# liuQuan98/EYOC

Measured on AMD Instinct MI355X. Metric: registered pairs/sec (30k-voxel KITTI pairs), higher is better.
Workload: dtype f32 (split16 products: fp32 storage/accumulation, 3 fp16 MFMAs on hi/lo-split operands per product); 1 GPU; 64 synthetic 30 cm KITTI-shaped pairs per step per GPU (mean 29894 voxels/cloud, ResUNetBN2C random-init, 5000-point NN, RANSAC 4000000 hypotheses/pair, planted inlier ratio 0.3, spconv math split16); parallelism=pairs sharded over 1 GPU(s), steps_in_flight=2

## Files before the change

### eyoc_amd/_lib.py

```python
from __future__ import annotations

import ctypes as C
import os
import threading

_HERE = os.path.dirname(os.path.abspath(__file__))
LIB_PATH = os.environ.get("EYOC_HIP_LIB") or os.path.join(_HERE, "lib", "libeyoc_hip.so")

MAX_LEVELS = 4
MAP_S1, MAP_DOWN, MAP_UP = 0, 1, 2


class MapsInfo(C.Structure):
    _fields_ = [("n_levels", C.c_int32), ("rows", C.c_int32 * MAX_LEVELS),
                ("pairs_s1", C.c_int64 * MAX_LEVELS), ("pairs_down", C.c_int64 * MAX_LEVELS),
                ("pairs_up", C.c_int64 * MAX_LEVELS), ("pairs_conv1", C.c_int64)]


class ModelDesc(C.Structure):
    _fields_ = [("in_channels", C.c_int32), ("out_channels", C.c_int32), ("conv1_kernel_size", C.c_int32),
                ("normalize_feature", C.c_int32), ("channels", C.c_int32 * 5), ("tr_channels", C.c_int32 * 5),
                ("bn_eps", C.c_float), ("expanded", C.c_int32)]


class LayerParams(C.Structure):
    _fields_ = [("name", C.c_char_p), ("kernel", C.POINTER(C.c_float)), ("K", C.c_int32), ("cin", C.c_int32),
                ("cout", C.c_int32), ("bias", C.POINTER(C.c_float)), ("bn_weight", C.POINTER(C.c_float)),
                ("bn_bias", C.POINTER(C.c_float)), ("bn_mean", C.POINTER(C.c_float)),
                ("bn_var", C.POINTER(C.c_float))]


class RansacParams(C.Structure):
    _fields_ = [("max_distance", C.c_float), ("edge_similarity", C.c_float), ("max_iteration", C.c_int32),
                ("seed", C.c_uint32)]


class RansacResult(C.Structure):
    _fields_ = [("T", C.c_float * 16), ("inliers", C.c_int32), ("best_hypothesis", C.c_int32),
                ("survivors", C.c_int32), ("inlier_rmse", C.c_float)]


class Sc2pcrParams(C.Structure):
    _fields_ = [("inlier_threshold", C.c_float), ("d_thre", C.c_float), ("ratio", C.c_float),
                ("nms_radius", C.c_float), ("num_iterations", C.c_int32), ("max_points", C.c_int32),
                ("k1", C.c_int32), ("k2", C.c_int32)]


class Sc2pcrLayout(C.Structure):
    _fields_ = ([(k, C.c_int32) for k in ("n", "words", "n_seed", "k1", "k2", "n_part", "col_chunk", "reserved")] +
                [("csr_cap", C.c_int64), ("total", C.c_uint64)] +
                [("off_" + k, C.c_uint64) for k in ("ctl", "v", "y", "score", "seeds", "hard", "tight", "knn", "Ts", "dom", "rank",
                                                    "ptr_h", "col_h", "val_h", "cnt", "blk_dense", "seed_h")])


class IcpParams(C.Structure):
    _fields_ = [("max_distance", C.c_double), ("relative_fitness", C.c_double), ("relative_rmse", C.c_double),
                ("max_iteration", C.c_int32), ("flags", C.c_int32)]


class IcpResult(C.Structure):
    _fields_ = [("T", C.c_double * 16), ("fitness", C.c_double), ("inlier_rmse", C.c_double), ("correspondences", C.c_int32),
                ("iterations", C.c_int32), ("status", C.c_int32), ("reserved", C.c_int32)]


_vp, _i, _sz = C.c_void_p, C.c_int, C.c_size_t
PROTOTYPES = {
    "eyoc_version": (_i, []),
    "eyoc_last_error": (C.c_char_p, []),
    "eyoc_create": (_i, [_i, C.POINTER(_vp)]),
    "eyoc_destroy": (_i, [_vp]),
    "eyoc_maps_workspace_bytes": (_sz, [_i]),
    "eyoc_maps_build": (_i, [_vp, _vp, _i, _vp, _sz, _vp, C.POINTER(_vp)]),
    "eyoc_maps_build_ordered": (_i, [_vp, _vp, _i, _vp, _sz, _vp, _i, C.POINTER(_vp)]),
    "eyoc_maps_free": (_i, [_vp]),
    "eyoc_maps_last_fault_batches": (_i, [_vp, _vp, _vp]),
    "eyoc_maps_internal_order": (_i, [_vp, _i]),
    "eyoc_maps_lazy_tables": (_i, [_vp, _i]),
    "eyoc_maps_fused_levels": (_i, [_vp, _i]),
    "eyoc_spconv_select_down_kernel": (_i, [_vp, _i]),
    "eyoc_maps_order_window_shift": (_i, [_vp, _i]),
    "eyoc_maps_row_order": (_vp, [_vp]),
    "eyoc_maps_copy_row_order": (_i, [_vp, _vp, _vp]),
    "eyoc_maps_rows": (_i, [_vp, _i]),
    "eyoc_maps_coords": (_vp, [_vp, _i]),
    "eyoc_maps_table": (_vp, [_vp, _i, _i]),
    "eyoc_maps_copy_coords": (_i, [_vp, _i, _vp, _vp]),
    "eyoc_maps_copy_table": (_i, [_vp, _i, _i, _vp, _vp]),
    "eyoc_maps_copy_up_order": (_i, [_vp, _i, _vp, _vp]),
    "eyoc_maps_order_min_rows": (_i, [_vp, _i]),
    "eyoc_maps_info": (_i, [_vp, _vp, _i, _vp, C.POINTER(MapsInfo)]),
    "eyoc_voxelize_workspace_bytes": (_sz, [_i]),
    "eyoc_voxelize": (_i, [_vp, _vp, _i, _i, C.c_float, _i, _vp, _vp, C.POINTER(C.c_int), _vp, _sz, _vp]),
    "eyoc_voxelize_batched_workspace_bytes": (_sz, [_i, _i]),
    "eyoc_voxelize_batched": (_i, [_vp, _vp, _i, C.POINTER(C.c_int64), _i, _i, C.c_float, _i, _vp, _vp, _vp,
                                   C.POINTER(C.c_int64), _vp, _sz, _vp]),
    "eyoc_voxelize_batched_isolating_workspace_bytes": (_sz, [_i, _i]),
    "eyoc_voxelize_batched_isolating": (_i, [_vp, _vp, _i, C.POINTER(C.c_int64), _i, _i, C.c_float, _i, _vp, _vp, _vp,
                                             C.POINTER(C.c_int64), _vp, _sz, _vp, _vp]),
    "eyoc_batch_drop_workspace_bytes": (_sz, [_i]),
    "eyoc_batch_drop": (_i, [_vp, _vp, _vp, _i, _i, _vp, _vp, _vp, _vp, C.POINTER(C.c_int), _vp, _vp, _sz, _vp]),
    "eyoc_remap_rows": (_i, [_vp, _vp, _i, _vp, _i, _vp, _vp]),
    "eyoc_gather_rows": (_i, [_vp, _vp, _i, _i, _vp, _i, _vp, C.c_float, _vp, _vp]),
    "eyoc_dotmax": (_i, [_vp, _vp, _vp, _i, C.POINTER(C.c_int32), C.POINTER(C.c_int32), _i, _vp, _vp, _vp]),
    "eyoc_knn2": (_i, [_vp, _vp, _vp, _i, C.POINTER(C.c_int32), C.POINTER(C.c_int32), _i, _vp, _vp, _vp, _vp]),
    "eyoc_lowe_topk": (_i, [_vp, _vp, _vp, _i, _i, _vp, _vp, _vp]),
    "eyoc_pair_filter": (_i, [_vp, _i, _vp, _vp, _vp, _vp, _i, _vp, C.c_float, _vp, _vp, _vp]),
    "eyoc_pair_filter_similarity": (_i, [_vp, _vp, _vp, _vp, _vp, _i, _vp, _i, _i, C.c_float, C.c_float, C.c_double, _vp, _vp,
                                         _vp]),
    "eyoc_spconv_packed_floats": (_sz, [_i, _i, _i]),
    "eyoc_spconv_pack_weights": (_i, [_vp, _vp, _i, _i, _i, _vp]),
    "eyoc_spconv_select_kernel": (_i, [_vp, _i]),
    "eyoc_spconv_pack_weights_transposed": (_i, [_vp, _i, _i, _i, _i, _vp]),
    "eyoc_spconv_grad_weight_workspace_bytes": (_sz, [_i, _i, _i, _i]),
    "eyoc_spconv_grad_weight": (_i, [_vp, _vp, _i, _i, _vp, _i, _i, _vp, _i, _i, _vp, _vp, _sz, _vp]),
    "eyoc_spconv_pack_weights_split16": (_i, [_vp, _vp, _i, _i, _i, _vp, _vp]),
    "eyoc_spconv_ex": (_i, [_vp, _vp, _i, _i, _i, _vp, _i, _i, _vp, _i, _vp, _vp, _i, _i, _vp, _i, _i, _i, _vp, _vp]),
    "eyoc_spconv_select_split16_kernel": (_i, [_vp, _i]),
    "eyoc_spconv_select_st_kernel": (_i, [_vp, _i]),
    "eyoc_spconv_st_split_below": (_i, [_vp, _i]),
    "eyoc_spconv_st_group_rows": (_i, [_vp, _i]),
    "eyoc_spconv_st_ksplit": (_i, [_vp, _i]),
    "eyoc_spconv_local_rulebook_bytes": (_sz, [_i]),
    "eyoc_spconv_build_local_rulebook": (_i, [_vp, _vp, _i, _i, _vp, _vp, _vp]),
    "eyoc_spconv_staged": (_i, [_vp, _vp, _vp, _i, _i, _vp, _i, _i, _vp, _i, _vp, _vp, _i, _i, _vp, _i, _i, _vp, _vp]),
    "eyoc_split16_encode": (_i, [_vp, _vp, _i, _i, _i, _vp, _i, _vp]),
    "eyoc_split16_decode": (_i, [_vp, _vp, _i, _i, _i, _vp, _i, _vp]),
    "eyoc_model_set_math": (_i, [_vp, _i]),
    "eyoc_model_last_math": (_i, [_vp]),
    "eyoc_model_range_check": (_i, [_vp, _vp, C.POINTER(C.c_float)]),
    "eyoc_model_range_snapshot": (_i, [_vp, _vp, _vp]),
    "eyoc_model_set_progress_event": (_i, [_vp, _i, _vp]),
    "eyoc_model_set_probe": (_i, [_vp, _i]),
    "eyoc_spconv": (_i, [_vp, _vp, _i, _i, _vp, _i, _i, _vp, _i, _vp, _vp, _i, _i, _vp, _i, _vp]),
    "eyoc_spconv_sum": (_i, [_vp, _vp, _i, _i, _vp, _i, _i, _vp, _i, _vp, _i, _vp]),
    "eyoc_model_blob_floats": (_sz, [C.POINTER(ModelDesc)]),
    "eyoc_model_pack_host": (_i, [C.POINTER(ModelDesc), C.POINTER(LayerParams), _i, _vp, _sz]),
    "eyoc_model_create": (_i, [_vp, C.POINTER(ModelDesc), C.POINTER(LayerParams), _i, _vp, _sz, C.POINTER(_vp)]),
    "eyoc_model_destroy": (_i, [_vp]),
    "eyoc_model_fuse_tail": (_i, [_vp, _i]),
    "eyoc_model_workspace_bytes": (_sz, [_vp, _vp]),
    "eyoc_model_forward": (_i, [_vp, _vp, _vp, _vp, _vp, _vp, _sz, _vp]),
    "eyoc_model_num_layers": (_i, [_vp]),
    "eyoc_model_layer_work": (_i, [_vp, _vp, _vp, _vp, C.POINTER(C.c_char_p), C.POINTER(C.c_int64),
                                   C.POINTER(C.c_double), C.POINTER(C.c_double), C.POINTER(C.c_double)]),
    "eyoc_model_set_timing": (_i, [_vp, _i]),
    "eyoc_model_layer_ms": (_i, [_vp, C.POINTER(C.c_float)]),
    "eyoc_model_timing_slot": (_i, [_vp, _i]),
    "eyoc_bn_workspace_bytes": (_sz, [_i, _i]),
    "eyoc_bn_train_forward": (_i, [_vp, _vp, _i, _i, _i, _vp, _vp, C.c_float, _i, _vp, _i, _vp, _vp, _sz, _vp]),
    "eyoc_bn_train_forward_running": (_i, [_vp, _vp, _i, _i, _i, _vp, _vp, C.c_float, _i, _vp, _i, _vp, _vp, _vp, C.c_float, _vp, _sz, _vp]),
    "eyoc_bn_train_backward": (_i, [_vp, _vp, _i, _vp, _i, _vp, _i, _i, _i, _vp, _vp, C.c_float, _vp, _i, _vp, _vp, _vp, _sz, _vp]),
    "eyoc_maps_gather_window": (_i, [_vp, _vp, _i, _vp, _i, _vp, _vp]),
    "eyoc_maps_gather_window_internal": (_i, [_vp, _vp, _i, _vp, _i, _vp, _vp]),
    "eyoc_knn_prefilter": (_i, [_vp, _i]),
    "eyoc_spconv_select_up_kernel": (_i, [_vp, _i]),
    "eyoc_spconv_upc_min_rows": (_i, [_vp, _i]),
    "eyoc_spconv_upc_tile_rows": (_i, [_i, _i]),
    "eyoc_spconv_upc_bytes": (_sz, [_i]),
    "eyoc_spconv_upc_build": (_i, [_vp, _vp, _i, _vp, _vp, _vp]),
    "eyoc_spconv_upc": (_i, [_vp, _vp, _vp, _i, _i, _vp, _i, _i, _vp, _i, _vp, _i, _vp, _i, _i, _vp, _vp]),
    "eyoc_spconv_select_conv1_kernel": (_i, [_vp, _i]),
    "eyoc_knn1": (_i, [_vp, _vp, _vp, _i, C.POINTER(C.c_int32), C.POINTER(C.c_int32), _i, _i, _vp, _vp, _vp]),
    "eyoc_pdist": (_i, [_vp, _vp, _i, _vp, _i, _i, _i, _vp, _vp]),
    "eyoc_kabsch_batched": (_i, [_vp, _vp, _vp, _vp, _i, _i, _vp, _vp]),
    "eyoc_irls_quad": (_i, [_vp, _vp, _vp, _vp, _i, _i, _vp, _vp]),
    "eyoc_ransac": (_i, [_vp, _vp, _vp, _vp, _i, C.POINTER(RansacParams), _vp, _vp]),
    "eyoc_maps_select_orders": (_i, [_vp, _i, _i]),
    "eyoc_ransac_select_pruning": (_i, [_vp, _i]),
    "eyoc_registration_accept_degenerate": (_i, [_vp, _i]),
    "eyoc_ransac_transform_store": (_i, [_vp, _i]),
    "eyoc_ransac_workspace_bytes": (_sz, [_vp, _i, _i, _i, _sz]),
    "eyoc_ransac_batched_ws": (_i, [_vp, _vp, _vp, _vp, C.POINTER(C.c_int32), C.POINTER(C.c_int32), _i,
                                    C.POINTER(RansacParams), _vp, _vp, _sz, _vp]),
    "eyoc_ransac_batched": (_i, [_vp, _vp, _vp, _vp, C.POINTER(C.c_int32), C.POINTER(C.c_int32), _i,
                                 C.POINTER(RansacParams), _vp, _vp]),
    "eyoc_sc2pcr_workspace_bytes": (_sz, [_i, C.POINTER(Sc2pcrParams)]),
    "eyoc_sc2pcr": (_i, [_vp, _vp, _vp, _i, C.POINTER(Sc2pcrParams), _vp, _vp, _vp, _sz, _vp]),
    "eyoc_sc2pcr_batched_workspace_bytes": (_sz, [_i, C.POINTER(Sc2pcrParams)]),
    "eyoc_sc2pcr_batched_workspace_bytes_n": (_sz, [_i, _i, C.POINTER(Sc2pcrParams)]),
    "eyoc_sc2pcr_set_shortlist_cap": (_i, [_vp, _i]),
    "eyoc_sc2pcr_set_dense_threshold": (_i, [_vp, _i]),
    "eyoc_sc2pcr_select_kernels": (_i, [_vp, _i]),
    "eyoc_sc2pcr_workspace_layout": (_i, [_i, C.POINTER(Sc2pcrParams), C.POINTER(Sc2pcrLayout)]),
    "eyoc_sc2pcr_batched": (_i, [_vp, _vp, _vp, C.POINTER(C.c_int32), _i, C.POINTER(Sc2pcrParams), _vp, _vp, _i, _vp, _sz,
                                 _vp]),
    "eyoc_icp_workspace_bytes": (_sz, [_i, _i, _i]),
    "eyoc_icp_batched": (_i, [_vp, _vp, _vp, C.POINTER(C.c_int32), C.POINTER(C.c_int32), _i, _vp, C.POINTER(IcpParams), _vp, _vp,
                              _vp, _sz, _vp]),
    "eyoc_icp_correspondences": (_i, [_vp, _vp, _vp, C.POINTER(C.c_int32), C.POINTER(C.c_int32), _i, _vp, C.c_double, _vp, _vp,
                                      _vp, _vp, _sz, _vp]),
}


ERR_INVALID, ERR_HIP, ERR_WORKSPACE, ERR_DUPLICATE, ERR_RANGE = -1, -2, -3, -4, -5
# ... 136 lines not shown
```

### eyoc_amd/csrc/common.h

```cpp
#pragma once
#include <hip/hip_runtime.h>

#include <cstdarg>
#include <cstdint>
#include <cstdio>
#include <cstring>
#include <string>
#include <vector>

#include "../../include/eyoc_hip.h"

namespace eyoc {

void set_error(const char* fmt, ...);

#define EYOC_CHECK_HIP(expr)                                                               \
  do {                                                                                     \
    hipError_t _e = (expr);                                                                \
    if (_e != hipSuccess) {                                                                \
      eyoc::set_error("%s failed: %s (%s:%d)", #expr, hipGetErrorString(_e), __FILE__,    \
                      __LINE__);                                                           \
      return EYOC_ERR_HIP;                                                                 \
    }                                                                                      \
  } while (0)
// ... 87 lines not shown
  unsigned long long* keys;
  int* vals;
  unsigned int mask;
};

__host__ __device__ inline unsigned long long pack_key(int b, int x, int y, int z) {
  return ((unsigned long long)(unsigned)b << 54) |
         ((unsigned long long)((unsigned)(x + COORD_BIAS) & 0x3FFFFu) << 36) |
         ((unsigned long long)((unsigned)(y + COORD_BIAS) & 0x3FFFFu) << 18) |
         ((unsigned long long)((unsigned)(z + COORD_BIAS) & 0x3FFFFu));
}

__host__ __device__ inline unsigned int hash_key(unsigned long long k) {
  k ^= k >> 33;
  k *= 0xff51afd7ed558ccdull;
  k ^= k >> 33;
  k *= 0xc4ceb9fe1a85ec53ull;
  k ^= k >> 33;
  return (unsigned int)k;
}

__device__ inline int hash_lookup(const HashTable& t, unsigned long long key) {
  unsigned int s = hash_key(key) & t.mask;
  for (unsigned int probes = 0; probes <= t.mask; ++probes) {
    unsigned long long k = t.keys[s];
    if (k == key) return t.vals[s];
    if (k == KEY_EMPTY) return -1;
    s = (s + 1) & t.mask;
  }
  return -1;
}

}

struct eyoc_maps {
  int n_levels = 0;
  int rows[EYOC_MAX_LEVELS] = {0, 0, 0, 0};
  int32_t* coords[EYOC_MAX_LEVELS] = {nullptr, nullptr, nullptr, nullptr};
  eyoc::HashTable table[EYOC_MAX_LEVELS];
  int32_t* nbr_s1[EYOC_MAX_LEVELS] = {nullptr, nullptr, nullptr, nullptr};
  int32_t* nbr_down[EYOC_MAX_LEVELS] = {nullptr, nullptr, nullptr, nullptr};
  int32_t* nbr_up[EYOC_MAX_LEVELS] = {nullptr, nullptr, nullptr, nullptr};
  int32_t* parent[EYOC_MAX_LEVELS] = {nullptr, nullptr, nullptr, nullptr};
  int32_t* children[EYOC_MAX_LEVELS] = {nullptr, nullptr, nullptr, nullptr};
  int32_t* perm_up[EYOC_MAX_LEVELS] = {nullptr, nullptr, nullptr, nullptr};
  int32_t* perm_s1[EYOC_MAX_LEVELS] = {nullptr, nullptr, nullptr, nullptr};
  int32_t* perm_down[EYOC_MAX_LEVELS] = {nullptr, nullptr, nullptr, nullptr};
  int32_t* row_perm = nullptr;
  unsigned char* local_s1[EYOC_MAX_LEVELS] = {nullptr, nullptr, nullptr, nullptr};
  unsigned char* local_up[EYOC_MAX_LEVELS] = {nullptr, nullptr, nullptr, nullptr};
  unsigned char* local_s1w[EYOC_MAX_LEVELS] = {nullptr, nullptr, nullptr, nullptr};
  unsigned char* local_down[EYOC_MAX_LEVELS] = {nullptr, nullptr, nullptr, nullptr};
  unsigned char* local_upc[EYOC_MAX_LEVELS] = {nullptr, nullptr, nullptr, nullptr};
  bool table0_built = false;
  bool s1_ready[EYOC_MAX_LEVELS] = {true, true, true, true};
  bool up_ready[EYOC_MAX_LEVELS] = {true, true, true, true};
  int32_t* up8[EYOC_MAX_LEVELS] = {nullptr, nullptr, nullptr, nullptr};
  hipEvent_t s1_ev[EYOC_MAX_LEVELS] = {nullptr, nullptr, nullptr, nullptr};
  hipEvent_t up_ev[EYOC_MAX_LEVELS] = {nullptr, nullptr, nullptr, nullptr};
  hipEvent_t table0_ev = nullptr;
  eyoc_maps() = default;
  eyoc_maps(const eyoc_maps&) = delete;
  eyoc_maps& operator=(const eyoc_maps&) = delete;
  ~eyoc_maps();
};

namespace eyoc {
int maps_build_table0(eyoc_maps* maps, hipStream_t st);
int maps_ensure_table(eyoc_maps* maps, int kind, int level, hipStream_t st);
size_t sort_rows64_tmp_bytes(int n);
int sort_rows_by_key64(void* tmp, size_t tmp_bytes, const unsigned long long* keys_in, unsigned long long* keys_out, const int* vals_in,
                       int* vals_out, int n, int bits, hipStream_t st);
size_t sort_rows_tmp_bytes(int n, int bits);
int sort_rows_by_key(void* tmp, size_t tmp_bytes, const unsigned int* keys_in, unsigned int* keys_out, const int* vals_in,
                     int* vals_out, int n, int bits, hipStream_t st);
}
```

### eyoc_amd/csrc/coordmap.hip

```cpp
#include <cstdlib>

#include "spconv.h"
#include "derive.h"
#include "scan.h"

using namespace eyoc;

namespace {

__device__ inline void coarse_coord(const int32_t* c, int ts2, int& b, int& x, int& y, int& z) {
  const int m = ~(ts2 - 1);
  b = c[0]; x = c[1] & m; y = c[2] & m; z = c[3] & m;
}

__global__ void k_insert(const int32_t* __restrict__ coords, int n, int ts2, HashTable t, int* __restrict__ slot_out,
                         int* __restrict__ err, unsigned int* __restrict__ range_mask = nullptr) {
  int i = blockIdx.x * blockDim.x + threadIdx.x;
  if (i >= n) return;
  int b, x, y, z;
  coarse_coord(coords + 4 * (size_t)i, ts2, b, x, y, z);
  constexpr int LIM = COORD_BIAS - 16;
  if (b < 0 || b >= 1024 || x < -LIM || x >= LIM || y < -LIM || y >= LIM || z < -LIM || z >= LIM) {
    if (err) atomicAdd(&err[0], 1);
    if (range_mask && b >= 0 && b < 1024) atomicOr(&range_mask[b >> 5], 1u << (b & 31));
// ... 556 lines not shown
  for (; i < n; i += stride) c += t[i] >= 0;
#pragma unroll
  for (int d = 32; d >= 1; d >>= 1) c += __shfl_down(c, d, 64);
  if ((threadIdx.x & 63) == 0 && c) atomicAdd(out, (unsigned long long)c);
}

__global__ void k_count_region(const int32_t* __restrict__ coords, int n, HashTable t, int ks,
                               unsigned long long* __restrict__ out) {
  int o = blockIdx.x * blockDim.x + threadIdx.x;
  unsigned int c = 0;
  if (o < n) {
    const int4 p = reinterpret_cast<const int4*>(coords)[o];
    const int r = ks / 2;
    for (int dz = -r; dz <= r; ++dz)
      for (int dy = -r; dy <= r; ++dy)
        for (int dx = -r; dx <= r; ++dx) c += hash_lookup(t, pack_key(p.x, p.y + dx, p.z + dy, p.w + dz)) >= 0;
  }
#pragma unroll
  for (int d = 32; d >= 1; d >>= 1) c += __shfl_down(c, d, 64);
  if ((threadIdx.x & 63) == 0 && c) atomicAdd(out, (unsigned long long)c);
}

constexpr int UP_KEY_BITS = KEY_PATTERN_BITS + KEY_WINDOW_BITS;
constexpr int ZORDER_MIN_ROWS = 8192;

unsigned int table_capacity(int n) {
  unsigned int cap = 1024;
  while (cap < 2u * (unsigned)n) cap <<= 1;
  return cap;
}

const int32_t* table_ptr(const eyoc_maps* maps, int kind, int level) {
  if (!maps || level < 0 || level >= maps->n_levels) return nullptr;
  switch (kind) {
    case EYOC_MAP_S1: return maps->nbr_s1[level];
    case EYOC_MAP_DOWN: return level + 1 < maps->n_levels ? maps->nbr_down[level] : nullptr;
    case EYOC_MAP_UP: return level + 1 < maps->n_levels ? maps->nbr_up[level] : nullptr;
    default: return nullptr;
  }
}

hipEvent_t* fill_event(eyoc_maps* m, int kind, int level) {
  if (!m || level < 0 || level + 1 >= m->n_levels) return nullptr;
  if (kind == EYOC_MAP_S1) return &m->s1_ev[level];
  if (kind == EYOC_MAP_UP) return &m->up_ev[level];
  return nullptr;
}

void keep_fault_masks(eyoc_ctx* ctx, const int* h, int code) {
  if (code == EYOC_ERR_DUPLICATE) memcpy(ctx->fault_dup, h, 32 * sizeof(uint32_t));
  if (code == EYOC_ERR_RANGE) memcpy(ctx->fault_range, h + 32, 32 * sizeof(uint32_t));
}

}

extern "C" {

size_t eyoc_maps_workspace_bytes(int n_rows) {
  if (n_rows < 0) return 0;
  const size_t n = (size_t)n_rows;
  const size_t cap = table_capacity(n_rows);
  size_t b = 0;
  b += EYOC_MAX_LEVELS * (align_up(cap * 8) + align_up(cap * 4));
  b += EYOC_MAX_LEVELS * align_up(n * 16);
  b += 10 * align_up(n * 27 * 4);
  b += 3 * align_up(n * 8 * 4);
  b += 3 * align_up(n * 4) + align_up((n / SCAN_TILE + 2) * 4);
  b += 3 * (align_up(n * 4) + align_up(n * 32));
  b += 4 * align_up(4 * n * 4) + align_up(sort_rows_tmp_bytes(4 * n_rows, UP_KEY_BITS + 4));
  b += align_up(n * 8) * 2 + align_up(n * 4) * 2 + align_up(sort_rows64_tmp_bytes(n_rows));
  b += 2 * align_up(local_rulebook_bytes(n_rows)) + EYOC_MAX_LEVELS * (align_up(local_rulebook_bytes(1)) + 256);
  b += 2 * align_up(local_rulebook_up_bytes(n_rows)) + EYOC_MAX_LEVELS * (align_up(local_rulebook_up_bytes(1)) + 256);
  b += 2 * (align_up(upc_kept_bytes(n_rows)) + align_up(upc_scratch_bytes(n_rows))) + EYOC_MAX_LEVELS * (align_up(upc_kept_bytes(1)) + align_up(upc_scratch_bytes(1)) + 512);
  b += 4 * (align_up(local_rulebook128_bytes(n_rows)) + 256);
  b += 4096;
  return b + 96 * 256;
}

int eyoc_maps_build(eyoc_ctx* ctx, const int32_t* coords_dev, int n, void* ws, size_t ws_bytes, void* stream,
                    eyoc_maps** out) {
  return eyoc_maps_build_ordered(ctx, coords_dev, n, ws, ws_bytes, stream, 0, out);
}

int eyoc_maps_build_ordered(eyoc_ctx* ctx, const int32_t* coords_dev, int n, void* ws, size_t ws_bytes, void* stream,
                            int order, eyoc_maps** out) {
  if (ctx) {
    memset(ctx->fault_dup, 0, sizeof(ctx->fault_dup));
    memset(ctx->fault_range, 0, sizeof(ctx->fault_range));
  }
  EYOC_REQUIRE(ctx && out && ws, EYOC_ERR_INVALID, "eyoc_maps_build: NULL argument");
  EYOC_REQUIRE(order >= -1 && order <= 1, EYOC_ERR_INVALID, "eyoc_maps_build_ordered: order %d", order);
  EYOC_REQUIRE(n > 0 && coords_dev, EYOC_ERR_INVALID, "eyoc_maps_build: empty coordinate set (n=%d)", n);
  EYOC_REQUIRE(((uintptr_t)ws & 255) == 0, EYOC_ERR_INVALID, "eyoc_maps_build: workspace must be 256-byte aligned");
  EYOC_REQUIRE(ws_bytes >= eyoc_maps_workspace_bytes(n), EYOC_ERR_WORKSPACE,
               "eyoc_maps_build: workspace %zu < required %zu bytes", ws_bytes, eyoc_maps_workspace_bytes(n));
  hipStream_t st = (hipStream_t)stream;
  Carver cv(ws, ws_bytes);
  eyoc_maps* m = new eyoc_maps();
  m->n_levels = EYOC_MAX_LEVELS;
  int* counters = cv.take<int>(128);
  unsigned int* fault_masks = (unsigned int*)(counters + 64);
  int* slot = cv.take<int>(n);
  int* flag = cv.take<int>(n);
  int* partial = cv.take<int>(n / SCAN_TILE + 2);
  int* host = (int*)ctx->pinned;
#define FAIL_HIP(expr)                                                                       \
  do {                                                                                       \
    hipError_t _e = (expr);                                                                  \
    if (_e != hipSuccess) {                                                                  \
      set_error("%s failed: %s (%s:%d)", #expr, hipGetErrorString(_e), __FILE__, __LINE__);  \
      delete m;                                                                              \
      return EYOC_ERR_HIP;                                                                   \
    }                                                                                        \
  } while (0)

  FAIL_HIP(hipMemsetAsync(counters, 0, 128 * sizeof(int), st));
  m->rows[0] = n;
  m->coords[0] = cv.take<int32_t>((size_t)n * 4);
  const eyoc_ctx::Knobs& kn = ctx->knobs;
  const int order_mode = kn.maps_internal_order >= 0 ? kn.maps_internal_order : order;
  const bool zorder = order_mode > 0 || (order_mode < 0 && n >= ZORDER_MIN_ROWS);
  int pre_rows[EYOC_MAX_LEVELS] = {n, 0, 0, 0};
  if (zorder) {
    unsigned long long* zk_in = cv.take<unsigned long long>(n);
    unsigned long long* zk_out = cv.take<unsigned long long>(n);
    int* zr_in = cv.take<int>(n);
    m->row_perm = cv.take<int32_t>(n);
    const size_t zb = sort_rows64_tmp_bytes(n);
    void* ztmp = cv.take<char>(zb);
    int kbits = ctx->zorder_kbits, bbits = ctx->zorder_bbits;
    for (int attempt = 0; attempt < 2; ++attempt) {
      if (attempt) FAIL_HIP(hipMemsetAsync(counters + 16, 0, (EYOC_MAX_LEVELS + 4) * sizeof(int), st));
      hipLaunchKernelGGL(k_morton_key, dim3(cdiv(n, 256)), dim3(256), 0, st, coords_dev, n, kbits, zk_in, zr_in);
      if (int rc = sort_rows_by_key64(ztmp, zb, zk_in, zk_out, zr_in, m->row_perm, n, 3 * (kbits + 1) + bbits, st)) { delete m; return rc; }
      hipLaunchKernelGGL(k_gather_coords, dim3(cdiv(n, 256)), dim3(256), 0, st, coords_dev, m->row_perm, n, m->coords[0]);
      hipLaunchKernelGGL(k_count_levels, dim3(cdiv(n, 256) < 1024 ? cdiv(n, 256) : 1024), dim3(256), 0, st, m->coords[0], n, kbits, bbits,
                         counters + 16, fault_masks);
      FAIL_HIP(hipMemcpyAsync(host + 16, counters + 16, (128 - 16) * sizeof(int), hipMemcpyDeviceToHost, st));
      FAIL_HIP(hipStreamSynchronize(st));
      if (host[16] == 0) break;
      kbits = 17; bbits = 10;
    }
    {
      int kb = 1, bb = 1;
      while (kb < 17 && (1 << kb) <= host[16 + EYOC_MAX_LEVELS + 2]) ++kb;
      while (bb < 10 && (1 << bb) <= host[16 + EYOC_MAX_LEVELS + 3]) ++bb;
      ctx->zorder_kbits = kb + 1 < 17 ? kb + 1 : 17;
      ctx->zorder_bbits = bb + 1 < 10 ? bb + 1 : 10;
    }
    if (host[16 + EYOC_MAX_LEVELS] != 0) {
      set_error("eyoc_maps_build: %d coordinate rows outside the supported key range (|c| < 2^17 - 16, 0 <= batch < 1024)",
                host[16 + EYOC_MAX_LEVELS]);
      keep_fault_masks(ctx, host + 64, EYOC_ERR_RANGE);
      delete m;
      return EYOC_ERR_RANGE;
    }
    if (host[16 + EYOC_MAX_LEVELS + 1] != 0) {
      set_error("eyoc_maps_build: %d duplicate coordinate rows (a sparse tensor needs unique coordinates)", host[16 + EYOC_MAX_LEVELS + 1]);
      keep_fault_masks(ctx, host + 64, EYOC_ERR_DUPLICATE);
      delete m;
      return EYOC_ERR_DUPLICATE;
    }
    for (int l = 1; l < EYOC_MAX_LEVELS; ++l) pre_rows[l] = host[16 + l];
  } else {
    FAIL_HIP(hipMemcpyAsync(m->coords[0], coords_dev, (size_t)n * 16, hipMemcpyDeviceToDevice, st));
  }
  {
    const unsigned int cap = table_capacity(n);
    m->table[0].keys = cv.take<unsigned long long>(cap);
    m->table[0].vals = cv.take<int>(cap);
    m->table[0].mask = cap - 1;
    m->table0_built = false;
  }
  unsigned int top_cap = 0;
// ... 7 lines not shown
    FAIL_HIP(hipMemsetAsync(m->children[0], 0xFF, (size_t)((char*)(tt.keys + top_cap) - (char*)m->children[0]), st));
    FAIL_HIP(hipMemsetAsync(tt.vals, 0x7F, (size_t)top_cap * 4, st));
  }
  const bool fused_levels = zorder && kn.maps_fused_levels;
  if (fused_levels) {
    LevelOut lo;
    for (int l = 1; l < EYOC_MAX_LEVELS; ++l) {
      m->rows[l] = pre_rows[l];
      m->coords[l] = cv.take<int32_t>((size_t)m->rows[l] * 4);
      m->parent[l - 1] = cv.take<int32_t>((size_t)m->rows[l - 1]);
      lo.coords[l - 1] = m->coords[l]; lo.parent[l - 1] = m->parent[l - 1]; lo.children[l - 1] = m->children[l - 1];
    }
    const int tiles = cdiv(n, LV_TILE);
    int* part = flag;
    hipLaunchKernelGGL(k_levels_count, dim3(tiles), dim3(LV_BLOCK), 0, st, m->coords[0], n, part, counters);
    hipLaunchKernelGGL(k_levels_fill, dim3(tiles), dim3(LV_BLOCK), 0, st, m->coords[0], n, part, lo, counters + 3);
    const int lt = EYOC_MAX_LEVELS - 1;
    hipLaunchKernelGGL(k_insert, dim3(cdiv(m->rows[lt], 256)), dim3(256), 0, st, m->coords[lt], m->rows[lt], 1 << lt, m->table[lt], (int*)nullptr, counters);
  }
  for (int l = 1; l < EYOC_MAX_LEVELS && !fused_levels; ++l) {
    const int n_src = m->rows[l - 1];
    const int32_t* src = m->coords[l - 1];
    const int ts2 = 1 << l;
    const int nb = cdiv(n_src, SCAN_TILE);
    const bool sorted_level = zorder;
    HashTable& t = m->table[l];
    if (sorted_level) {
      hipLaunchKernelGGL(k_flag_sorted, dim3(cdiv(n_src, 256)), dim3(256), 0, st, src, n_src, ts2, flag,
                         l == 1 ? counters : (int*)nullptr, l == 1 ? counters + 1 : (int*)nullptr);
    } else {
      const unsigned int cap = table_capacity(n_src);
      t.keys = cv.take<unsigned long long>(cap);
      t.vals = cv.take<int>(cap);
      t.mask = cap - 1;
      FAIL_HIP(hipMemsetAsync(t.keys, 0xFF, (size_t)cap * 8, st));
      FAIL_HIP(hipMemsetAsync(t.vals, 0x7F, (size_t)cap * 4, st));
      hipLaunchKernelGGL(k_insert, dim3(cdiv(n_src, 256)), dim3(256), 0, st, src, n_src, ts2, t, slot, counters,
                         l == 1 ? fault_masks + 32 : (unsigned int*)nullptr);
      hipLaunchKernelGGL(k_flag, dim3(cdiv(n_src, 256)), dim3(256), 0, st, slot, t.vals, n_src, flag, (int*)nullptr);
    }
    hipLaunchKernelGGL(k_scan_partials, dim3(nb), dim3(SCAN_BLOCK), 0, st, flag, n_src, partial);
    hipLaunchKernelGGL(k_scan_top, dim3(1), dim3(SCAN_BLOCK), 0, st, partial, nb, counters + 2 + l);
    if (zorder) {
      m->rows[l] = pre_rows[l];
    } else {
    if (l == 1) {
      FAIL_HIP(hipMemcpyAsync(host + 128, counters, 128 * sizeof(int), hipMemcpyDeviceToHost, st));
      FAIL_HIP(hipStreamSynchronize(st));
      host[0] = host[128 + 2 + l]; host[1] = host[128]; host[2] = host[128 + 1];
    } else {
      FAIL_HIP(hipMemcpyAsync(host, counters + 2 + l, sizeof(int), hipMemcpyDeviceToHost, st));
      FAIL_HIP(hipStreamSynchronize(st));
    }
    if (l == 1 && host[1] != 0) {
      set_error("eyoc_maps_build: %d coordinate rows outside the supported key range (|c| < 2^17 - 16, 0 <= batch < 1024)", host[1]);
      keep_fault_masks(ctx, host + 128 + 64, EYOC_ERR_RANGE);
      delete m;
      return EYOC_ERR_RANGE;
    }
    if (l == 1 && sorted_level && host[2] != 0) {
      set_error("eyoc_maps_build: %d duplicate coordinate rows (a sparse tensor needs unique coordinates)", host[2]);
      keep_fault_masks(ctx, host + 128 + 64, EYOC_ERR_DUPLICATE);
      delete m;
      return EYOC_ERR_DUPLICATE;
    }
    m->rows[l] = host[0];
    }
    m->coords[l] = cv.take<int32_t>((size_t)m->rows[l] * 4);
    m->parent[l - 1] = cv.take<int32_t>((size_t)n_src);
    if (!zorder) {
      m->children[l - 1] = cv.take<int32_t>((size_t)m->rows[l] * 8);
      FAIL_HIP(hipMemsetAsync(m->children[l - 1], 0xFF, (size_t)m->rows[l] * 32, st));
    }
    if (sorted_level) {
      hipLaunchKernelGGL(k_compact_sorted, dim3(nb), dim3(SCAN_BLOCK), 0, st, flag, partial, src, n_src, ts2, l - 1,
                         m->coords[l], m->parent[l - 1], m->children[l - 1]);
      if (l + 1 == EYOC_MAX_LEVELS) {
        hipLaunchKernelGGL(k_insert, dim3(cdiv(m->rows[l], 256)), dim3(256), 0, st, m->coords[l], m->rows[l], ts2, t, (int*)nullptr, counters);
      }
      continue;
    }
    hipLaunchKernelGGL(k_compact<false>, dim3(nb), dim3(SCAN_BLOCK), 0, st, flag, partial, slot, src, n_src, ts2,
                       m->coords[l], t.vals, (int32_t*)nullptr);
    hipLaunchKernelGGL(k_children, dim3(cdiv(n_src, 256)), dim3(256), 0, st, slot, t.vals, src, n_src, l - 1,
                       m->parent[l - 1], m->children[l - 1], l == 1 ? counters + 1 : (int*)nullptr,
                       l == 1 ? fault_masks : (unsigned int*)nullptr);
    if (l == 1) {
      FAIL_HIP(hipMemcpyAsync(host + 128, counters, 128 * sizeof(int), hipMemcpyDeviceToHost, st));
      FAIL_HIP(hipStreamSynchronize(st));
      host[0] = host[128 + 1];
      if (host[0] != 0) {
        set_error("eyoc_maps_build: %d duplicate coordinate rows (a sparse tensor needs unique coordinates)", host[0]);
        keep_fault_masks(ctx, host + 128 + 64, EYOC_ERR_DUPLICATE);
        delete m;
        return EYOC_ERR_DUPLICATE;
      }
    }
  }
  const bool use_upc = kn.up_kernel == 2 && n >= kn.upc_min_rows;
  const bool use_up = kn.up_kernel == 1 || (kn.up_kernel == 2 && !use_upc);
  const bool lazy = zorder && use_upc && kn.maps_lazy_tables != 0;
  for (int l = 0; l < EYOC_MAX_LEVELS; ++l) {
    m->nbr_s1[l] = cv.take<int32_t>((size_t)27 * m->rows[l]);
    if (l + 1 < EYOC_MAX_LEVELS) {
      m->nbr_down[l] = cv.take<int32_t>((size_t)27 * m->rows[l + 1]);
      m->nbr_up[l] = cv.take<int32_t>((size_t)27 * m->rows[l]);
// ... 27 lines not shown
  unsigned int* key_in = cv.take<unsigned int>(total);
  unsigned int* key_out = cv.take<unsigned int>(total);
  int* row_in = cv.take<int>(total);
  int32_t* perm_all = cv.take<int32_t>(total);
  const size_t sort_bytes = sort_rows_tmp_bytes((int)total, TAG_SHIFT + TAG_BITS);
  void* sort_tmp = cv.take<char>(sort_bytes);
  for (int l = EYOC_MAX_LEVELS - 2; l >= 0; --l) {
    const int nl = m->rows[l], nc = m->rows[l + 1];
    const int su = seg_up[l];
    if (lazy) {
      if (l > 0)
        hipLaunchKernelGGL((k_derive_fine<true, 2>), dim3(cdiv(nl, 256)), dim3(256), 0, st, m->coords[l], nl, l, m->parent[l], m->children[l],
                           m->nbr_s1[l + 1], nc, m->nbr_s1[l], m->up8[l], (unsigned int*)nullptr, (int*)nullptr, 0u, wshift);
    } else {
      hipLaunchKernelGGL((k_derive_fine<true, 1>), dim3(cdiv(nl, 256)), dim3(256), 0, st, m->coords[l], nl, l, m->parent[l],
                         m->children[l], m->nbr_s1[l + 1], nc, m->nbr_s1[l], m->nbr_up[l],
                         su >= 0 ? key_in + seg_base[su] : (unsigned int*)nullptr, su >= 0 ? row_in + seg_base[su] : (int*)nullptr,
                         (unsigned int)(su >= 0 ? su : 0) << TAG_SHIFT, wshift);
    }
    hipLaunchKernelGGL(k_derive_down, dim3(cdiv(nc, 256)), dim3(256), 0, st, nc, m->children[l], m->nbr_s1[l + 1],
                       m->nbr_down[l]);
  }
  for (int l = 0; l + 1 < EYOC_MAX_LEVELS; ++l) {
    const int sd = seg_dn[l];
    if (sd < 0) continue;
    hipLaunchKernelGGL(k_children_key, dim3(cdiv(m->rows[l + 1], 256)), dim3(256), 0, st, m->children[l], m->rows[l + 1],
                       key_in + seg_base[sd], row_in + seg_base[sd], (unsigned int)sd << TAG_SHIFT, wshift);
  }
  for (int l = 0; l < EYOC_MAX_LEVELS; ++l) {
    const int ss = seg_s1[l];
    if (ss < 0) continue;
    const int bits = l == 0 ? 2 : 4;
    hipLaunchKernelGGL(k_pattern_key, dim3(cdiv(m->rows[l], 256)), dim3(256), 0, st, m->nbr_s1[l], m->rows[l], bits,
                       key_in + seg_base[ss], row_in + seg_base[ss], (unsigned int)ss << TAG_SHIFT, wshift);
  }
  if (total > 0) {
    if (int rc = sort_rows_by_key(sort_tmp, sort_bytes, key_in, key_out, row_in, perm_all, (int)total, TAG_SHIFT + TAG_BITS, st)) {
      delete m;
      return rc;
    }
    for (int l = 0; l < EYOC_MAX_LEVELS; ++l) {
      if (seg_up[l] >= 0) m->perm_up[l] = perm_all + seg_base[seg_up[l]];
      if (seg_s1[l] >= 0) m->perm_s1[l] = perm_all + seg_base[seg_s1[l]];
      if (seg_dn[l] >= 0) m->perm_down[l] = perm_all + seg_base[seg_dn[l]];
    }
  }
  if (zorder) {
    for (int l = 0; l < EYOC_MAX_LEVELS; ++l) {
      m->local_s1[l] = cv.take<unsigned char>(local_rulebook_bytes(m->rows[l]));
      if (lazy && l == 0) {
        DeriveSrc src;
        src.coords = m->coords[0]; src.parent = m->parent[0]; src.children = m->children[0]; src.s1c = m->nbr_s1[1];
        src.nc = m->rows[1]; src.sh = 0; src.up8 = m->up8[0];
        if (int rc = build_local_rulebook_derived(src, m->rows[0], m->local_s1[0], counters + 8, st, kn.st_group)) { delete m; return rc; }
      } else if (int rc = build_local_rulebook(m->nbr_s1[l], 27, m->rows[l], m->local_s1[l], counters + 8, st, kn.st_group)) { delete m; return rc; }
      if (l + 1 < EYOC_MAX_LEVELS && use_up) {
        m->local_up[l] = cv.take<unsigned char>(local_rulebook_up_bytes(m->rows[l]));
        if (int rc = build_local_rulebook_up(m->nbr_up[l], 27, m->rows[l], m->local_up[l], counters + 9, st)) { delete m; return rc; }
      }
      if (l + 1 < EYOC_MAX_LEVELS && use_upc) {
        m->local_upc[l] = cv.take<unsigned char>(upc_kept_bytes(m->rows[l]));
        unsigned char* scratch = cv.take<unsigned char>(upc_scratch_bytes(m->rows[l]));
        if (m->local_upc[l]) {
          if (int rc = build_upc(lazy ? m->up8[l] : m->nbr_up[l], m->coords[l], 1 << l, m->rows[l], m->local_upc[l], scratch, st, lazy)) { delete m; return rc; }
        } else if (int rc = maps_ensure_table(m, EYOC_MAP_UP, l, st)) { delete m; return rc; }
      }
    }
    const bool use_down = kn.down_kernel == 1 && n >= kn.upc_min_rows;
    for (int l = EYOC_MAX_LEVELS - 1; l < EYOC_MAX_LEVELS && use_down && kn.s1_wide; ++l) {
      m->local_s1w[l] = cv.take<unsigned char>(local_rulebook128_bytes(m->rows[l]));
      if (m->local_s1w[l])
        if (int rc = build_local_rulebook128(m->nbr_s1[l], 27, m->rows[l], m->local_s1w[l], counters + 13, st, kn.st_group)) { delete m; return rc; }
    }
    for (int l = 0; l + 1 < EYOC_MAX_LEVELS && use_down; ++l) {
      m->local_down[l] = cv.take<unsigned char>(local_rulebook128_bytes(m->rows[l + 1]));
      if (m->local_down[l])
        if (int rc = build_local_rulebook128(m->nbr_down[l], 27, m->rows[l + 1], m->local_down[l], counters + 10 + l, st, kn.st_group)) { delete m; return rc; }
    }
    for (int l = 0; l < EYOC_MAX_LEVELS; ++l) {
      host[16 + l] = 0;
      if (m->local_upc[l]) FAIL_HIP(hipMemcpyAsync(host + 16 + l, upc_overflow_ptr(m->local_upc[l]), sizeof(int), hipMemcpyDeviceToHost, st));
    }
    FAIL_HIP(hipMemcpyAsync(host, counters + 8, 8 * sizeof(int), hipMemcpyDeviceToHost, st));
    FAIL_HIP(hipMemcpyAsync(host + 32, counters, 8 * sizeof(int), hipMemcpyDeviceToHost, st));
    FAIL_HIP(hipStreamSynchronize(st));
    if (host[32] != 0) {
      set_error("eyoc_maps_build: %d coordinate rows outside the supported key range (|c| < 2^17 - 16, 0 <= batch < 1024)", host[32]);
      keep_fault_masks(ctx, host + 64, EYOC_ERR_RANGE);
      delete m;
      return EYOC_ERR_RANGE;
    }
    if (host[33] != 0) {
      set_error("eyoc_maps_build: %d duplicate coordinate rows (a sparse tensor needs unique coordinates)", host[33]);
      keep_fault_masks(ctx, host + 64, EYOC_ERR_DUPLICATE);
      delete m;
      return EYOC_ERR_DUPLICATE;
    }
    for (int l = 1; l < EYOC_MAX_LEVELS; ++l)
      if (host[32 + 2 + l] != m->rows[l]) {
        set_error("eyoc_maps_build: internal error - level %d has %d rows by its scan, %d by the up-front count", l, host[32 + 2 + l], m->rows[l]);
        delete m;
        return EYOC_ERR_INVALID;
      }
    if (host[0] != 0) {
      for (int l = 0; l < EYOC_MAX_LEVELS; ++l) m->local_s1[l] = nullptr;
      if (int rc = maps_ensure_table(m, EYOC_MAP_S1, 0, st)) { delete m; return rc; }
    }
    if (host[1] != 0)
      for (int l = 0; l < EYOC_MAX_LEVELS; ++l) m->local_up[l] = nullptr;
    for (int l = 0; l + 1 < EYOC_MAX_LEVELS; ++l)
      if (host[2 + l] != 0) m->local_down[l] = nullptr;
    if (host[5] != 0)
      for (int l = 0; l < EYOC_MAX_LEVELS; ++l) m->local_s1w[l] = nullptr;
    for (int l = 0; l < EYOC_MAX_LEVELS; ++l)
      if (host[16 + l] != 0) {
        m->local_upc[l] = nullptr;
        if (int rc = maps_ensure_table(m, EYOC_MAP_UP, l, st)) { delete m; return rc; }
      }
  }
  FAIL_HIP(hipGetLastError());
#undef FAIL_HIP
  if (!cv.ok()) {
    set_error("eyoc_maps_build: internal workspace accounting error (%zu > %zu)", cv.off, cv.cap);
    delete m;
    return EYOC_ERR_WORKSPACE;
  }
  *out = m;
  return EYOC_OK;
}

size_t eyoc_voxelize_workspace_bytes(int n_points) {
  if (n_points < 0) return 0;
  const size_t n = (size_t)n_points, cap = table_capacity(n_points);
  return align_up(cap * 8) + align_up(cap * 4) + align_up(n * 16) + 3 * align_up(n * 4) +
         align_up((n / SCAN_TILE + 2) * 4) + 4096 + 16 * 256;
}

size_t eyoc_voxelize_batched_workspace_bytes(int n_points_total, int n_clouds) {
  if (n_points_total < 0 || n_clouds < 1) return 0;
  return eyoc_voxelize_workspace_bytes(n_points_total) + align_up((size_t)(n_clouds + 1) * 8) + align_up((size_t)(n_clouds + 1) * 4);
}

size_t eyoc_voxelize_batched_isolating_workspace_bytes(int n_points_total, int n_clouds) {
  if (n_points_total < 0 || n_clouds < 1) return 0;
  return eyoc_voxelize_batched_workspace_bytes(n_points_total, n_clouds) + align_up((size_t)n_clouds * 8 + 8);
}

}

namespace {

int voxelize_run(eyoc_ctx* ctx, const char* who, const float* xyz_dev, int n, int stride, const int64_t* pt_off_host,
                 int n_clouds, float voxel_size, int batch_base, int32_t* sel_dev, int32_t* coords_dev, float* xyz_out_dev,
                 int64_t* vox_off_host, void* ws, size_t ws_bytes, hipStream_t st, int32_t* faults_host = nullptr) {
  Carver cv(ws, ws_bytes);
  const bool iso = faults_host != nullptr;
  const int fo = 64 + ((n_clouds + 2) & ~1);
  int* counters = cv.take<int>(iso ? fo + 2 * n_clouds : 64 + n_clouds + 1);
  int* faults = counters + fo;
  int64_t* pt_off = cv.take<int64_t>(n_clouds + 1);
  int32_t* raw = cv.take<int32_t>((size_t)n * 4);
  int* slot = cv.take<int>(n);
  int* flag = cv.take<int>(n);
  int* partial = cv.take<int>(n / SCAN_TILE + 2);
  HashTable t;
  const unsigned int cap = table_capacity(n);
  t.keys = cv.take<unsigned long long>(cap);
  t.vals = cv.take<int>(cap);
  t.mask = cap - 1;
  EYOC_REQUIRE(cv.ok(), EYOC_ERR_WORKSPACE, "%s: internal workspace accounting error (%zu > %zu)", who, cv.off, cv.cap);
  const size_t up_bytes = n_clouds > 1 ? align_up((size_t)(n_clouds + 1) * 8) : 0;
  const int back = iso ? fo + 2 * n_clouds : n_clouds > 1 ? 64 + n_clouds + 1 : 4;
  EYOC_REQUIRE(up_bytes + (size_t)back * 4 <= ctx->pinned_bytes, EYOC_ERR_INVALID, "%s: %d clouds exceed the pinned staging", who,
               n_clouds);
  int64_t* up = (int64_t*)ctx->pinned;
  int* host = (int*)((char*)ctx->pinned + up_bytes);
  if (n_clouds > 1) {
    memcpy(up, pt_off_host, (size_t)(n_clouds + 1) * 8);
    EYOC_CHECK_HIP(hipMemcpyAsync(pt_off, up, (size_t)(n_clouds + 1) * 8, hipMemcpyHostToDevice, st));
  }
  EYOC_CHECK_HIP(hipMemsetAsync(counters, 0, 64 * sizeof(int), st));
  if (iso) EYOC_CHECK_HIP(hipMemsetAsync(faults, 0, (size_t)n_clouds * 2 * sizeof(int), st));
// ... 346 lines not shown
```

### eyoc_amd/csrc/model.hip

```cpp
#include <algorithm>
#include <cmath>
#include <cstdlib>

#include "spconv.h"

using namespace eyoc;

namespace {

enum MapSel { M_CONV1, M_S1, M_DOWN, M_UP, M_IDENT, M_AFFINE };

struct LayerPlan {
  std::string name;
  std::string norm;
  int K, cin, cout;
  MapSel map;
  int level;
  int out_level;
  int in_buf, in_col, out_buf, out_col, res_buf;
  int relu, l2norm, has_bias;
  size_t w_off = 0, b_off = 0;
  size_t w16_off = 0, s_off = 0;
};

// ... 333 lines not shown
  if (m->math == 0) return 0;
  for (const LayerPlan& p : m->layers)
    if (p.map == M_S1 && p.cin >= 128 && p.cout >= 64 && p.cout <= 256 &&
        (long long)cdiv(maps->rows[p.level], ST_TILE) * (p.cout / 32) <= KS_MAX_SLOTS)
      return KS_PART_BYTES;
  return 0;
}

size_t eyoc_model_workspace_bytes(const eyoc_model* m, const eyoc_maps* maps) {
  if (!m || !maps) return 0;
  size_t b = 0;
  for (int i = B_X1; i < B_OUT; ++i) b += align_up((size_t)maps->rows[m->bufs[i].level] * m->bufs[i].width * sizeof(float));
  b += align_up(ks_part_bytes(m, maps));
  return b + 256;
}

int eyoc_model_num_layers(const eyoc_model* m) { return m ? (int)m->layers.size() : 0; }

int eyoc_model_set_math(eyoc_model* m, int mode) {
  EYOC_REQUIRE(m && mode >= -1 && mode <= 1, EYOC_ERR_INVALID, "eyoc_model_set_math: mode %d not in {-1, 0, 1}", mode);
  const int prev = m->math;
  m->math = mode;
  return prev + 1 ? prev + 2 : 1;
}

int eyoc_model_last_math(const eyoc_model* m) { return m ? m->last_math : -1; }

int eyoc_model_set_timing(eyoc_model* m, int on) {
  EYOC_REQUIRE(m, EYOC_ERR_INVALID, "eyoc_model_set_timing: NULL model");
  m->timing = on ? 1 : 0;
  m->events_valid[0] = m->events_valid[1] = 0;
  if (on && m->events.empty()) {
    m->events.resize(2 * (m->layers.size() + 1));
    for (auto& e : m->events) EYOC_CHECK_HIP(hipEventCreate(&e));
  }
  return EYOC_OK;
}

int eyoc_model_timing_slot(eyoc_model* m, int slot) {
  EYOC_REQUIRE(m && (slot == 0 || slot == 1), EYOC_ERR_INVALID, "eyoc_model_timing_slot: slot %d", slot);
  m->slot = slot;
  return EYOC_OK;
}

int eyoc_model_layer_ms(eyoc_model* m, float* ms) {
  EYOC_REQUIRE(m && ms, EYOC_ERR_INVALID, "eyoc_model_layer_ms: NULL argument");
  EYOC_REQUIRE(m->timing && m->events_valid[m->slot], EYOC_ERR_INVALID, "eyoc_model_layer_ms: no timed forward recorded in slot %d", m->slot);
  const hipEvent_t* ev = m->events.data() + (size_t)m->slot * (m->layers.size() + 1);
  EYOC_CHECK_HIP(hipEventSynchronize(ev[m->layers.size()]));
  for (size_t i = 0; i < m->layers.size(); ++i) EYOC_CHECK_HIP(hipEventElapsedTime(&ms[i], ev[i], ev[i + 1]));
  return EYOC_OK;
}

int eyoc_model_forward(eyoc_ctx* ctx, const eyoc_model* mc, const eyoc_maps* maps, const float* feats_dev, float* out_dev,
                       void* ws, size_t ws_bytes, void* stream) {
  EYOC_REQUIRE(ctx && mc && maps && feats_dev && out_dev && ws, EYOC_ERR_INVALID, "eyoc_model_forward: NULL argument");
  EYOC_REQUIRE(ws_bytes >= eyoc_model_workspace_bytes(mc, maps), EYOC_ERR_WORKSPACE,
               "eyoc_model_forward: workspace %zu < required %zu bytes", ws_bytes, eyoc_model_workspace_bytes(mc, maps));
  EYOC_REQUIRE(((uintptr_t)ws & 255) == 0, EYOC_ERR_INVALID, "eyoc_model_forward: workspace must be 256-byte aligned");
  eyoc_model* m = const_cast<eyoc_model*>(mc);
  hipStream_t st = (hipStream_t)stream;
  float* buf[B_COUNT];
  Carver cv(ws, ws_bytes);
  buf[B_IN] = const_cast<float*>(feats_dev);
  buf[B_OUT] = out_dev;
  for (int i = B_X1; i < B_OUT; ++i) buf[i] = cv.take<float>((size_t)maps->rows[m->bufs[i].level] * m->bufs[i].width);
  const size_t ks_bytes = ks_part_bytes(m, maps);
  float* ks_part = ks_bytes ? cv.take<float>(ks_bytes / 4) : nullptr;
  const int want = m->math;
  const bool split_ok = ctx->knobs.spconv_kernel != 0 && !(m->desc.normalize_feature && m->desc.out_channels > 64) &&
                        m->desc.channels[1] % 32 == 0;
  const bool split = split_ok && (want == 1 || (want < 0 && maps->rows[0] >= 8192));
  EYOC_REQUIRE(want != 1 || split, EYOC_ERR_INVALID,
               "eyoc_model_forward: split16 arithmetic is not available for this model / kernel selection");
  m->last_math = split ? 1 : 0;
  EYOC_CHECK_HIP(hipMemsetAsync(m->range, 0, 4, st));
  EYOC_CHECK_HIP(hipMemsetAsync(m->range + 4, 0, 8, st));
  hipEvent_t* ev = m->timing ? m->events.data() + (size_t)m->slot * (m->layers.size() + 1) : nullptr;
  if (m->timing) EYOC_CHECK_HIP(hipEventRecord(ev[0], st));
  bool progress_recorded = m->progress_event == nullptr;
  for (size_t li = 0; li < m->layers.size(); ++li) {
    const LayerPlan& p = m->layers[li];
    const int n_out = maps->rows[p.out_level];
    int rc;
    if (!progress_recorded && (int)li >= m->progress_layer) {
      EYOC_CHECK_HIP(hipEventRecord(m->progress_event, st));
      progress_recorded = true;
    }
    if (p.map == M_AFFINE) {
      rc = launch_affine(buf[p.in_buf] + p.in_col, m->bufs[p.in_buf].width, n_out, p.cout, m->blob + p.w_off, m->blob + p.b_off,
                         buf[p.out_buf] + p.out_col, m->bufs[p.out_buf].width, split, split ? m->range : nullptr, st);
    } else if (p.map == M_CONV1) {
      Conv1Args a;
      a.coords = maps->coords[0]; a.n = n_out; a.table = maps->table[0]; a.ks = m->desc.conv1_kernel_size;
      a.in = buf[p.in_buf]; a.cin = p.cin; a.w = m->blob + p.w_off; a.bias = m->blob + p.b_off; a.cout = p.cout;
      a.out = buf[p.out_buf] + p.out_col; a.ld_out = m->bufs[p.out_buf].width;
      a.out_split = split ? 1 : 0;
      a.ctx = ctx;
      a.range = split ? m->range : nullptr;
      a.wscale = m->blob + p.s_off;
      a.in_perm = maps->row_perm;
      if (a.in_perm) {
        int best = -1;
        size_t best_sz = 0;
        for (int i = B_X1; i < B_OUT; ++i) {
          const size_t sz = (size_t)maps->rows[m->bufs[i].level] * m->bufs[i].width;
          if (i != p.out_buf && sz > best_sz) { best = i; best_sz = sz; }
        }
// ... 11 lines not shown
    } else if (split && ctx->knobs.fuse_tail != 0 && li + 2 == m->layers.size() && p.map == M_IDENT && p.K == 1 && p.res_buf < 0 &&
               m->layers[li + 1].map == M_IDENT && m->layers[li + 1].K == 1 && m->layers[li + 1].in_buf == p.out_buf &&
               m->layers[li + 1].res_buf < 0 && !m->layers[li + 1].relu && m->layers[li + 1].out_buf == B_OUT && p.out_col == 0 &&
               tail_fusable(p.cin, p.cout, m->layers[li + 1].cout)) {
      const LayerPlan& q = m->layers[li + 1];
      rc = launch_tail_fused(buf[p.in_buf] + p.in_col, m->bufs[p.in_buf].width, n_out, m->blob + p.w16_off, m->blob + p.s_off,
                             m->blob + p.b_off, p.relu, m->blob + q.w16_off, m->blob + q.s_off, m->blob + q.b_off, q.l2norm,
                             buf[q.out_buf] + q.out_col, m->bufs[q.out_buf].width, maps->row_perm, m->range, st);
      if (rc) return rc;
      if (m->timing) {
        EYOC_CHECK_HIP(hipEventRecord(ev[li + 1], st));
        EYOC_CHECK_HIP(hipEventRecord(ev[li + 2], st));
      }
      ++li;
      continue;
    } else {
      SpconvArgs a;
      a.nbr = p.map == M_S1 ? maps->nbr_s1[p.level] : p.map == M_DOWN ? maps->nbr_down[p.level]
              : p.map == M_UP ? maps->nbr_up[p.level] : nullptr;
      a.K = p.K; a.n_out = n_out;
      a.n_in = maps->rows[m->bufs[p.in_buf].level];
      a.in = buf[p.in_buf] + p.in_col; a.ld_in = m->bufs[p.in_buf].width; a.cin = p.cin;
      a.w = m->blob + p.w_off; a.cout = p.cout; a.bias = m->blob + p.b_off;
      a.res = p.res_buf >= 0 ? buf[p.res_buf] : nullptr; a.ld_res = p.res_buf >= 0 ? m->bufs[p.res_buf].width : 0;
      a.relu = p.relu; a.l2norm = p.l2norm;
      a.out = buf[p.out_buf] + p.out_col; a.ld_out = m->bufs[p.out_buf].width;
      a.ctx = ctx;
      if (split) {
        a.math = 1;
        a.w = m->blob + p.w16_off;
        a.out_scale = m->blob + p.s_off;
        a.out_split = p.out_buf != B_OUT;
        a.range = m->range;
        if (p.map == M_S1 && p.cin >= 32 && p.cin % 32 == 0) { a.local = maps->local_s1[p.level]; a.ks_part = ks_part; }
        if (p.map == M_S1 && p.cin % 32 == 0 && p.cout % 128 == 0 && ctx->knobs.s1_wide) a.local128 = maps->local_s1w[p.level];
        if (p.map == M_DOWN && p.cin % 32 == 0 && p.cout % 64 == 0) a.local_down = maps->local_down[p.level];
        if (p.map == M_UP && p.cin % 32 == 0 && p.cout % 64 == 0) a.local_up = maps->local_up[p.level];
        if (p.map == M_UP && p.cin % 32 == 0 && p.cout % 64 == 0) a.local_upc = maps->local_upc[p.level];
      }
      if (p.out_buf == B_OUT) a.out_perm = maps->row_perm;
      if ((p.map == M_S1 || p.map == M_UP) && spconv_record_path(a) == 0)
        if ((rc = maps_ensure_table(const_cast<eyoc_maps*>(maps), p.map == M_S1 ? EYOC_MAP_S1 : EYOC_MAP_UP, p.level, st))) return rc;
      a.perm = p.map == M_UP ? maps->perm_up[p.level] : p.map == M_S1 ? maps->perm_s1[p.level]
               : p.map == M_DOWN ? maps->perm_down[p.level] : nullptr;
      if (split && ctx->knobs.fuse_tail == 2 && li + 3 == m->layers.size() && p.map == M_S1 && p.cout == 64) {
        const LayerPlan &q1 = m->layers[li + 1], &q2 = m->layers[li + 2];
        if (q1.map == M_IDENT && q1.K == 1 && q1.res_buf < 0 && q2.map == M_IDENT && q2.K == 1 && q2.in_buf == q1.out_buf && q2.res_buf < 0 &&
            !q2.relu && q2.out_buf == B_OUT && q1.out_col == 0 && tail_fusable(q1.cin, q1.cout, q2.cout) && q1.in_buf == p.out_buf &&
            q1.in_col == p.out_col && q1.cin == p.cout + 32 && spconv_record_path(a) == 1 && spconv_st_can_fuse_tail(a)) {
          a.tail.skip = buf[q1.in_buf] + q1.in_col + p.cout; a.tail.ld_skip = m->bufs[q1.in_buf].width;
          a.tail.w1 = m->blob + q1.w16_off; a.tail.s1 = m->blob + q1.s_off; a.tail.b1 = m->blob + q1.b_off; a.tail.relu1 = q1.relu;
          a.tail.w2 = m->blob + q2.w16_off; a.tail.s2 = m->blob + q2.s_off; a.tail.b2 = m->blob + q2.b_off; a.tail.l2norm = q2.l2norm;
          a.tail.out = buf[q2.out_buf] + q2.out_col; a.tail.ld_out = m->bufs[q2.out_buf].width; a.tail.out_perm = maps->row_perm;
          rc = launch_spconv(a, st);
          if (rc) return rc;
          if (m->timing)
            for (int e = 1; e <= 3; ++e) EYOC_CHECK_HIP(hipEventRecord(ev[li + e], st));
          li += 2;
          continue;
        }
      }
      rc = launch_spconv(a, st);
    }
    if (rc) return rc;
    if (m->timing) EYOC_CHECK_HIP(hipEventRecord(ev[li + 1], st));
  }
  if (!progress_recorded) EYOC_CHECK_HIP(hipEventRecord(m->progress_event, st));
  if (m->timing) m->events_valid[m->slot] = 1;
  return EYOC_OK;
}

int eyoc_model_set_progress_event(eyoc_model* m, int layer, void* hip_event) {
  EYOC_REQUIRE(m, EYOC_ERR_INVALID, "eyoc_model_set_progress_event: NULL model");
  const int n = (int)m->layers.size();
  if (layer < 0) layer += n;
  EYOC_REQUIRE(!hip_event || (layer >= 0 && layer <= n), EYOC_ERR_INVALID, "eyoc_model_set_progress_event: layer %d of %d", layer, n);
  m->progress_event = (hipEvent_t)hip_event;
  m->progress_layer = layer;
  return EYOC_OK;
}

int eyoc_model_layer_work(eyoc_ctx* ctx, const eyoc_model* m, const eyoc_maps* maps, void* stream, const char** names,
                          int64_t* pairs, double* flops, double* gather_bytes, double* compulsory_bytes) {
  EYOC_REQUIRE(ctx && m && maps, EYOC_ERR_INVALID, "eyoc_model_layer_work: NULL argument");
  eyoc_maps_info_t info;
  int rc = eyoc_maps_info(ctx, maps, m->desc.conv1_kernel_size, stream, &info);
  if (rc) return rc;
  for (size_t li = 0; li < m->layers.size(); ++li) {
    const LayerPlan& p = m->layers[li];
    const double n_out = maps->rows[p.out_level];
    double n_in = n_out, pr = 0;
    switch (p.map) {
      case M_CONV1: pr = (double)info.pairs_conv1; break;
      case M_S1: pr = (double)info.pairs_s1[p.level]; break;
      case M_DOWN: pr = (double)info.pairs_down[p.level]; n_in = maps->rows[p.level]; break;
      case M_UP: pr = (double)info.pairs_up[p.level]; n_in = maps->rows[p.level + 1]; break;
      case M_IDENT: pr = n_out; break;
      case M_AFFINE: break;
    }
    if (p.map == M_AFFINE) {
      if (names) names[li] = p.name.c_str();
      if (pairs) pairs[li] = 0;
      if (flops) flops[li] = 2.0 * n_out * p.cout;
      if (gather_bytes) gather_bytes[li] = 8.0 * n_out * p.cout;
      if (compulsory_bytes) compulsory_bytes[li] = 8.0 * n_out * p.cout;
      continue;
    }
    const double wbytes = 4.0 * p.K * p.cin * p.cout;
    if (names) names[li] = p.name.c_str();
    if (pairs) pairs[li] = (int64_t)pr;
    if (flops) flops[li] = 2.0 * pr * p.cin * p.cout;
    if (gather_bytes) gather_bytes[li] = pr * (4.0 * p.cin + 8.0) + 4.0 * n_out * p.cout + wbytes;
    if (compulsory_bytes) compulsory_bytes[li] = 4.0 * (n_in * p.cin + n_out * p.cout) + 8.0 * pr + wbytes;
  }
  return EYOC_OK;
}

}
```

### eyoc_amd/csrc/spconv.h

```cpp
#pragma once
#include "common.h"

namespace eyoc {

inline int spconv_ct(int cout) { return cout >= 128 ? 128 : cout; }
inline int spconv_cc(int cin, int ) { return cin % 64 == 0 ? 64 : 32; }

struct TailFuse {
  const float* skip = nullptr;
  int ld_skip = 0;
  const float *w1 = nullptr, *s1 = nullptr, *b1 = nullptr, *w2 = nullptr, *s2 = nullptr, *b2 = nullptr;
  int relu1 = 0, l2norm = 0;
  float* out = nullptr;
  int ld_out = 0;
  const int32_t* out_perm = nullptr;
};

struct SpconvArgs {
  const int32_t* nbr;
  int K, n_out;
  int n_in = 0;
  const float* in;
  int ld_in, cin;
  const float* w;
  int cout;
  const float* bias;
  const float* res;
  int ld_res;
  int relu;
  int l2norm;
  float* out;
  int ld_out;
  int math = 0;
  int out_split = 0;
  const int32_t* out_perm = nullptr;
  const unsigned char* local = nullptr;
  const unsigned char* local128 = nullptr;
  const unsigned char* local_down = nullptr;
  const unsigned char* local_up = nullptr;
  const unsigned char* local_upc = nullptr;
  const float* out_scale = nullptr;
  const int32_t* perm = nullptr;
  int small_rows = 0;
  unsigned int* range = nullptr;
  eyoc_ctx* ctx = nullptr;
  float* ks_part = nullptr;
  int allow_offset_split = 0, offset_split = 1;
  float* offset_part = nullptr;
  int cg_local = 0;
  TailFuse tail;
};
constexpr int KS_MAX_SLOTS = 1024;
constexpr size_t KS_PART_BYTES = (size_t)KS_MAX_SLOTS * 256 * 32 * 4;

typedef _Float16 half8_t __attribute__((ext_vector_type(8)));
typedef _Float16 half4_t __attribute__((ext_vector_type(4)));

__device__ inline void split16_encode4(const float4 v, uint2& hi, uint2& lo) {
  half4_t h, l;
  h[0] = (_Float16)v.x; h[1] = (_Float16)v.y; h[2] = (_Float16)v.z; h[3] = (_Float16)v.w;
  l[0] = (_Float16)(v.x - (float)h[0]); l[1] = (_Float16)(v.y - (float)h[1]);
  l[2] = (_Float16)(v.z - (float)h[2]); l[3] = (_Float16)(v.w - (float)h[3]);
  hi = __builtin_bit_cast(uint2, h);
  lo = __builtin_bit_cast(uint2, l);
}
__device__ inline float4 split16_decode4(const uint2 hi, const uint2 lo) {
  const half4_t h = __builtin_bit_cast(half4_t, hi), l = __builtin_bit_cast(half4_t, lo);
  return make_float4((float)h[0] + (float)l[0], (float)h[1] + (float)l[1], (float)h[2] + (float)l[2], (float)h[3] + (float)l[3]);
}
__host__ __device__ inline int split16_off4(int c) { return (c >> 5) * 128 + (c & 31) * 2; }
constexpr int SPLIT16_LO = 64;
__device__ inline void split16_store4(float* row, int c, const float4 v) {
  uint2 hi, lo;
  split16_encode4(v, hi, lo);
  char* p = reinterpret_cast<char*>(row) + split16_off4(c);
  *reinterpret_cast<uint2*>(p) = hi;
  *reinterpret_cast<uint2*>(p + SPLIT16_LO) = lo;
}
__device__ inline float4 split16_load4(const float* row, int c) {
  const char* p = reinterpret_cast<const char*>(row) + split16_off4(c);
  return split16_decode4(*reinterpret_cast<const uint2*>(p), *reinterpret_cast<const uint2*>(p + SPLIT16_LO));
}

constexpr float SPLIT16_LIMIT = 6.0e4f;
__device__ inline float split16_merge(float a, float b) {
  const unsigned int x = __float_as_uint(a) & 0x7FFFFFFFu, y = __float_as_uint(b) & 0x7FFFFFFFu;
  return __uint_as_float(x > y ? x : y);
}
__device__ inline bool split16_over(float mx) { return (__float_as_uint(mx) & 0x7FFFFFFFu) >= __float_as_uint(SPLIT16_LIMIT); }
__device__ inline void split16_track(float& mx, const float4 v) {
  mx = split16_merge(split16_merge(split16_merge(mx, v.x), split16_merge(v.y, v.z)), v.w);
}
__device__ inline void split16_report(unsigned int* range, float mx) {
  if (!range) return;
  if (split16_over(mx)) { atomicOr(range, 1u); atomicOr(range + 3, 1u); }
  if (__builtin_nontemporal_load(range + 2)) atomicMax(range + 1, __float_as_uint(mx) & 0x7FFFFFFFu);
}
__device__ inline bool split16_poisoned(const unsigned int* range) { return range && __builtin_nontemporal_load(range) != 0u; }

__device__ __forceinline__ void lds_barrier() { asm volatile("s_waitcnt lgkmcnt(0)\n\ts_barrier" ::: "memory"); }

template <int HS>
__device__ inline int canonical_slot_id(const int* hk, const unsigned short* hpos, int s) {
  const int kv = hk[s];
  int start = s, len = 1;
  while (len < HS && hk[(start - 1) & (HS - 1)] >= 0) { start = (start - 1) & (HS - 1); ++len; }
  int rank = 0;
  for (int q = start; q != s; q = (q + 1) & (HS - 1)) rank += hk[q] < kv;
  for (int q = (s + 1) & (HS - 1); hk[q] >= 0 && q != start; q = (q + 1) & (HS - 1)) rank += hk[q] < kv;
  return hpos[(start + rank) & (HS - 1)];
}

int launch_spconv(const SpconvArgs& a, hipStream_t st);
int launch_permute_rows(const float* in, const int32_t* perm, int n, int c, float* out, hipStream_t st);
int launch_spconv_st(const SpconvArgs& a, const unsigned char* local_dev, hipStream_t st);
int launch_spconv_up(const SpconvArgs& a, const unsigned char* local_dev, hipStream_t st);
size_t local_rulebook_up_bytes(int n_out);
bool spconv_st_can_fuse_tail(const SpconvArgs& a);
int spconv_record_path(const SpconvArgs& a);
int build_local_rulebook_up(const int32_t* nbr_dev, int K, int n_out, unsigned char* out_dev, int* overflow_dev, hipStream_t st);
size_t upc_kept_bytes(int n_out);
size_t upc_scratch_bytes(int n_out);
int build_upc(const int32_t* nbr_dev, const int32_t* coords_dev, int stride, int n_out, unsigned char* ws, unsigned char* scratch, hipStream_t st, bool compact = false);
const int* upc_overflow_ptr(const unsigned char* ws);
int upc_set_tile_rows(int odd_axes, int rows);
int launch_spconv_upc(const SpconvArgs& a, const unsigned char* ws, hipStream_t st);
int st_variants();
size_t local_rulebook_bytes(int n_out);
int build_local_rulebook(const int32_t* nbr_dev, int K, int n_out, unsigned char* out_dev, int* overflow_dev, hipStream_t st, int group = 1);
struct DeriveSrc {
  const int32_t* coords = nullptr;
  const int32_t* parent = nullptr;
  const int32_t* children = nullptr;
  const int32_t* s1c = nullptr;
  int nc = 0, sh = 0;
  int32_t* up8 = nullptr;
};
size_t local_rulebook128_bytes(int n_out);
int build_local_rulebook128(const int32_t* nbr_dev, int K, int n_out, unsigned char* out_dev, int* overflow_dev, hipStream_t st, int group = 1);
int launch_spconv_st128(const SpconvArgs& a, const unsigned char* local_dev, hipStream_t st);
int build_local_rulebook_derived(const DeriveSrc& src, int n_out, unsigned char* out_dev, int* overflow_dev, hipStream_t st, int group = 1);
int launch_spconv_rs(const SpconvArgs& a, hipStream_t st);
bool tail_fusable(int cin1, int cmid, int cout);
int launch_tail_fused(const float* in, int ld_in, int n, const float* w1, const float* s1, const float* b1, int relu1, const float* w2,
                      const float* s2, const float* b2, int l2norm, float* out, int ld_out, const int32_t* out_perm, unsigned int* range,
                      hipStream_t st);
bool spconv_rs_fits(const SpconvArgs& a);
int launch_spconv_wave(const SpconvArgs& a, hipStream_t st);

struct Conv1Args {
  const int32_t* coords;
  int n;
  HashTable table;
  int ks;
  const float* in;
  int cin;
  const float* w;
  const float* bias;
  int cout;
  const float* wscale = nullptr;
  float* out;
  int ld_out;
  int out_split = 0;
  unsigned int* range = nullptr;
  const int32_t* in_perm = nullptr;
  const int32_t* parent;
  const int32_t* children;
  const int32_t* s1c;
  int nc;
  const unsigned char* local1 = nullptr;
  const eyoc_ctx* ctx = nullptr;
};
constexpr int ST_TILE = 256, ST_UMAX = 639, ST_UCAP = 1280, ST_NPASS = 2, ST_LOC_OFF = 16 + ST_UCAP * 4, ST_INV_OFF = 33152, ST_LR_BYTES = 33408;
int launch_conv1(const Conv1Args& a, hipStream_t st);
bool conv1_walks_octree(const Conv1Args& a);

}
```

### eyoc_amd/csrc/spconv_st.hip

```cpp
#include <atomic>
#include <cstdlib>

#include "spconv.h"
#include "derive.h"

using namespace eyoc;

namespace {

typedef float f32x4 __attribute__((ext_vector_type(4)));
typedef unsigned int u32x4 __attribute__((ext_vector_type(4)));

constexpr int NW = 4;
constexpr int TILE = NW * 64;
constexpr int XROWS = 640;
constexpr int UMAX = XROWS - 1;
constexpr int NPASS = 2;
constexpr int UCAP = 1280;
constexpr int X_BYTES = XROWS * 128;
constexpr int LO_REGION = XROWS * 64;
constexpr int NIT = XROWS / (16 * NW);
__host__ __device__ constexpr int slot_addr(int l) { return l * 64 + ((l >> 2) & 3) * 16; }

constexpr int MASK_OFF = 16 + UCAP * 4 + NPASS * 27 * 64 * 8;
constexpr int MASK_PASS_BYTES = 56;
constexpr int RM_OFF = MASK_OFF + NPASS * MASK_PASS_BYTES;
constexpr int INV_OFF = RM_OFF + TILE;
constexpr int LR_BYTES = INV_OFF + TILE;
static_assert(INV_OFF == ST_INV_OFF, "spconv.h mirrors this layout");
static_assert(TILE == ST_TILE && UMAX == ST_UMAX && UCAP == ST_UCAP && NPASS == ST_NPASS && LR_BYTES == ST_LR_BYTES, "spconv.h mirrors this layout");
static_assert(LR_BYTES % 128 == 0, "records start on cache lines");
#ifndef EYOC_LR_HSLOTS_LOG2
#define EYOC_LR_HSLOTS_LOG2 11
#endif
constexpr int HSLOTS_LOG2 = EYOC_LR_HSLOTS_LOG2, HSLOTS_T = 1 << HSLOTS_LOG2;

template <bool DERIVE, int NWB>
__global__ __launch_bounds__(NWB * 64) void k_local_rulebook(const int32_t* __restrict__ nbr, int K, int n_out, unsigned char* __restrict__ out,
                                                             int* __restrict__ overflow, int group, DeriveSrc d) {
  constexpr int TR = NWB * 64;
  constexpr int HS = HSLOTS_T, HSHIFT = 32 - HSLOTS_LOG2;
  __shared__ int hk[HS];
  __shared__ unsigned short hid[HS];
  __shared__ unsigned short srow[27][TR];
  __shared__ __attribute__((aligned(16))) unsigned long long key[TR];
  __shared__ int wave_cnt[NWB];
  __shared__ int too_many;
  const int lane = threadIdx.x & 63, wave = threadIdx.x >> 6;
  const int tile = blockIdx.x;
  const int row = tile * TR + (int)threadIdx.x;
  for (int i = threadIdx.x; i < HS; i += TR) hk[i] = -1;
  if (threadIdx.x == 0) too_many = 0;
  __syncthreads();
  unsigned short slot[27];
  int idxs[27];
  if constexpr (DERIVE) {
#pragma unroll
    for (int k = 0; k < 27; ++k) idxs[k] = -1;
    if (row < n_out) {
      const int4 c = reinterpret_cast<const int4*>(d.coords)[row];
      const int b[3] = {(c.y >> d.sh) & 1, (c.z >> d.sh) & 1, (c.w >> d.sh) & 1};
      int blk[8];
      derive_blocks(b, d.parent[row], d.s1c, d.nc, blk);
      derive_window(b, blk, d.children, idxs);
      if (d.up8) {
        int bl[8];
        derive_up_blocks(b, blk, bl);
        const int cls = b[0] | (b[1] << 1) | (b[2] << 2);
#pragma unroll
        for (int m = 0; m < 8; ++m) d.up8[(size_t)m * n_out + row] = (m & ~cls) == 0 ? bl[m] : -1;
      }
    }
  } else {
#pragma unroll
    for (int k = 0; k < 27; ++k) idxs[k] = (k < K && row < n_out) ? nbr[(size_t)k * n_out + row] : -1;
  }
#pragma unroll
  for (int k = 0; k < 27; ++k) {
    const int idx = idxs[k];
    unsigned int s = 0xFFFFu;
    if (idx >= 0) {
      s = ((unsigned)idx * 2654435761u) >> HSHIFT;
      int probes = 0;
      while (true) {
        const int prev = atomicCAS(&hk[s], -1, idx);
        if (prev == -1 || prev == idx) break;
        s = (s + 1) & (HS - 1);
        if (++probes >= HS) { too_many = 1; s = 0xFFFFu; break; }
      }
    }
    slot[k] = (unsigned short)s;
  }
  {
    unsigned int mask = 0;
#pragma unroll
    for (int k = 0; k < 27; ++k) {
      srow[k][threadIdx.x] = slot[k];
      if (slot[k] != 0xFFFFu) mask |= 1u << k;
    }
    const unsigned int zp = (mask >> 18) & 0x1FFu, zm = mask & 0x1FFu, z0 = (mask >> 9) & 0x1FFu;
    const unsigned int yp = mask & 0x70381C0u ? 1u : 0u;
    const unsigned int ym = mask & 0x01C0E07u ? 1u : 0u;
    const unsigned int xp = mask & 0x4924924u ? 1u : 0u;
    const unsigned int xm = mask & 0x1249249u ? 1u : 0u;
    unsigned int cb = (zp ? 32u : 0u) | (zm ? 16u : 0u) | (yp << 3) | (ym << 2) | (xp << 1) | xm;
    cb ^= cb >> 1; cb ^= cb >> 2; cb ^= cb >> 4;
    const unsigned long long coarse = cb;
    const unsigned long long pattern = ((unsigned long long)zp << 18) | ((unsigned long long)zm << 9) | z0;
    key[threadIdx.x] = group ? (coarse << 35) | (pattern << 8) | threadIdx.x : (unsigned long long)threadIdx.x;
  }
  __syncthreads();
  if (too_many) {
    if (threadIdx.x == 0) {
      reinterpret_cast<int*>(out + (size_t)tile * LR_BYTES)[0] = -1;
      atomicAdd(overflow, 1);
    }
    return;
  }
  constexpr int PER_WAVE = HS / NWB;
  int cnt = 0;
  for (int i0 = 0; i0 < PER_WAVE; i0 += 64) cnt += __popcll(__ballot(hk[wave * PER_WAVE + i0 + lane] >= 0));
  if (lane == 0) wave_cnt[wave] = cnt;
  __syncthreads();
  int base = 0, total = 0;
  for (int w = 0; w < NWB; ++w) { if (w < wave) base += wave_cnt[w]; total += wave_cnt[w]; }
  unsigned char* lr = out + (size_t)tile * LR_BYTES;
  int* U = reinterpret_cast<int*>(lr + 16);
  if (total <= UMAX) {
    for (int i0 = 0; i0 < PER_WAVE; i0 += 64) {
      const int s = wave * PER_WAVE + i0 + lane;
      const int key = hk[s];
      const unsigned long long m = __ballot(key >= 0);
      const int id = base + __popcll(m & ((1ull << lane) - 1ull));
      if (key >= 0) {
        hid[s] = (unsigned short)id;
        U[id] = key;
      }
      base += __popcll(m);
    }
  } else {
    for (int i0 = 0; i0 < PER_WAVE; i0 += 64) {
      const int s = wave * PER_WAVE + i0 + lane;
      const unsigned long long m = __ballot(hk[s] >= 0);
      if (hk[s] >= 0) hid[s] = (unsigned short)(base + __popcll(m & ((1ull << lane) - 1ull)));
      base += __popcll(m);
    }
    __syncthreads();
    unsigned short ids[PER_WAVE / 64];
#pragma unroll
    for (int q = 0; q < PER_WAVE / 64; ++q) {
      const int s = wave * PER_WAVE + q * 64 + lane;
      ids[q] = hk[s] >= 0 ? (unsigned short)canonical_slot_id<HS>(hk, hid, s) : (unsigned short)0;
    }
    __syncthreads();
#pragma unroll
    for (int q = 0; q < PER_WAVE / 64; ++q) {
      const int s = wave * PER_WAVE + q * 64 + lane;
      const int key = hk[s];
      if (key >= 0) {
        hid[s] = ids[q];
        if (ids[q] < NPASS * UMAX) U[ids[q]] = key;
      }
    }
  }
  if (threadIdx.x == 0) {
    reinterpret_cast<int*>(lr)[0] = total <= NPASS * UMAX ? total : -1;
    if (total > NPASS * UMAX) atomicAdd(overflow, 1);
  }
  __syncthreads();
  if (group) {
    const unsigned long long mine = key[threadIdx.x];
    int rank = 0;
    const ulonglong2* kp = reinterpret_cast<const ulonglong2*>(key);
#pragma unroll 8
    for (int i = 0; i < TR / 2; ++i) {
      const ulonglong2 kk = kp[i];
      rank += (kk.x < mine) + (kk.y < mine);
    }
    __syncthreads();
    key[rank] = mine;
    __syncthreads();
  }
  unsigned short* loc = reinterpret_cast<unsigned short*>(lr + 16 + UCAP * 4);
  unsigned char* msk = lr + MASK_OFF;
  __shared__ unsigned char nib[NPASS][27][4];
  const int r = (int)threadIdx.x, w = r >> 6, c = (r >> 4) & 3, j = r & 15;
  const int src = (int)(key[group ? (c * NWB + ((c & 1) ? NWB - 1 - w : w)) * 16 + j : r] & 255u);
  lr[RM_OFF + (w * 16 + j) * 4 + c] = (unsigned char)src;
  lr[INV_OFF + src] = (unsigned char)r;
#pragma unroll
  for (int k = 0; k < 27; ++k) {
    const unsigned int hs = srow[k][src];
    const int id = hs != 0xFFFFu ? (int)hid[hs] : -1;
#pragma unroll
    for (int p = 0; p < NPASS; ++p) {
      if (p > 0 && total <= p * UMAX) continue;
      const int l = (id >= p * UMAX && id < (p + 1) * UMAX) ? id - p * UMAX : UMAX;
      loc[(((size_t)(p * 27 + k) * 64) + w * 16 + j) * 4 + c] = (unsigned short)slot_addr(l);
      const unsigned long long b = __ballot(l != UMAX);
      if (lane == 0)
        nib[p][k][w] = (unsigned char)(((b & 0xFFFFull) != 0) | (((b >> 16) & 0xFFFFull) != 0) << 1 | (((b >> 32) & 0xFFFFull) != 0) << 2 |
                                       (((b >> 48) & 0xFFFFull) != 0) << 3);
    }
  }
  __syncthreads();
  if (threadIdx.x < NPASS * 28) {
    const int p = (int)threadIdx.x / 28, k = (int)threadIdx.x % 28;
    unsigned short m = 0;
    if (k < 27 && !(p > 0 && total <= p * UMAX)) {
      m = (unsigned short)(nib[p][k][0] | nib[p][k][1] << 4);
      if (NWB == 4) m |= (unsigned short)(nib[p][k][2] << 8 | nib[p][k][3] << 12);
    }
    reinterpret_cast<unsigned short*>(msk)[p * 28 + k] = m;
  }
}

template <int NTW, int CC, int NH>
__global__ __launch_bounds__(NW * 64, 2) void spconv_st_kernel(SpconvArgs a, const unsigned char* __restrict__ local, int n_tiles) {
  constexpr int CTW = NTW * 16, NC = 4;
  constexpr int CTG = CTW * NH;
  constexpr int WD = (NTW * NH <= 2) ? 2 : 1;
  extern __shared__ __attribute__((aligned(16))) unsigned char xs[];
  const int lane = threadIdx.x & 63;
  const int wave = __builtin_amdgcn_readfirstlane((int)(threadIdx.x >> 6));
  const int g = lane >> 4, j = lane & 15;
  const int n_cg = a.cout / CTG;
  const int xcd = (int)blockIdx.x & 7, per = 8 / n_cg;
  const int cg = xcd % n_cg, tile = ((int)blockIdx.x >> 3) * per + xcd / n_cg;
  if (tile >= n_tiles) return;
  const int w0 = NH == 1 ? wave : 2 * (wave >> 1);
  const int ct0 = cg * CTG + (NH == 2 ? (wave & 1) * CTW : 0);
  const int CT = a.cout >= 128 ? 128 : a.cout;
  const int n_slices = a.cout / CT, slice = ct0 / CT, nt0 = (ct0 - slice * CT) / 16;
  constexpr int JQ = CC / 16;
  const int ncc = a.cin / CC;
  const int nqb = a.cin / 32;
  constexpr int K = 27;

  const unsigned char* lr = local + (size_t)tile * LR_BYTES;
  const int n_u = __builtin_amdgcn_readfirstlane(reinterpret_cast<const int*>(lr)[0]);
// ... 153 lines not shown
      if (a.out_split) split16_store4(a.out + (size_t)o * a.ld_out, ch, v);
      else *reinterpret_cast<float4*>(a.out + (size_t)o * a.ld_out + ch) = v;
    }
  }
  if (a.out_split) split16_report(a.range, mx);
}


#ifdef EYOC_ST_TRACE
constexpr int TRACE_WGS = 16384, TRACE_N = 16;
__device__ unsigned long long g_st_trace[TRACE_WGS * TRACE_N];
#define ST_STAMP(i) do { if (threadIdx.x == 0 && blockIdx.x < TRACE_WGS) g_st_trace[blockIdx.x * TRACE_N + (i)] = __builtin_amdgcn_s_memrealtime(); } while (0)
#else
#define ST_STAMP(i) do {} while (0)
#endif
typedef float f32x16 __attribute__((ext_vector_type(16)));
typedef unsigned int u32x8 __attribute__((ext_vector_type(8)));

#include "spconv_st_loop.inc"
#if defined(EYOC_ST_ABLATIONS) || defined(EYOC_ST_TRACE)
#include "spconv_st_loop_abl.inc"
#endif

template <int CC, int NH, int SKIP, int NWV = NW, int TR = TILE, int TAILF = 0>
__global__ __launch_bounds__(NWV * 64, NWV / 2) void spconv_st_asm_kernel(SpconvArgs a, const unsigned char* __restrict__ local, int n_tiles, int ksplit, int phase) {
  constexpr int NTW = 2, CTW = NTW * 16, NC = 4;
  constexpr bool T128 = TR == 128;
  static_assert(TAILF == 0 || (NH == 2 && TR == TILE && NWV == NW && SKIP == 1), "the fused tail rides on the 256-row NH = 2 kernel");
  constexpr int CTG = T128 ? (NH == 2 ? 4 * CTW : 2 * CTW) : CTW * NH * (NWV / NW);
  constexpr int NITV = XROWS / (16 * NWV);
  static_assert(NWV == NW || (NWV == 2 * NW && NH == 1), "8 waves: 64 rows x 32 channels each");
  static_assert(TR == TILE || (T128 && NWV == NW), "128-row tiles: four waves");
  __shared__ __attribute__((aligned(128))) unsigned char xs[X_BYTES + (SKIP >= 15 && SKIP <= 17 ? 8192 : 0)];
  const int lane = threadIdx.x & 63;
  const int wave = __builtin_amdgcn_readfirstlane((int)(threadIdx.x >> 6));
  const int g = lane >> 4, j = lane & 15;
  const int n_cg = a.cout / CTG;
  const int xcd = (int)blockIdx.x & 7, per = 8 / n_cg;
  const int cg = a.cg_local ? ((int)blockIdx.x >> 3) % n_cg : xcd % n_cg;
  const int tile = a.cg_local ? (((int)blockIdx.x >> 3) / n_cg) * 8 + xcd : ((int)blockIdx.x >> 3) * per + xcd / n_cg;
  if (tile >= n_tiles) return;
  const int w0 = T128 ? (NH == 2 ? 0 : (wave >> 1)) : NH == 1 ? (wave & 3) : 2 * (wave >> 1);
  const int ct0 = cg * CTG + (T128 && NH == 2 ? wave * CTW : T128 || NH == 2 ? (wave & 1) * CTW : (wave >> 2) * CTW);
  const int CT = a.cout >= 128 ? 128 : a.cout;
  const int n_slices = a.cout / CT, slice = ct0 / CT, nt0 = (ct0 - slice * CT) / 16;
  constexpr int JQ = CC / 16;
  const int ncc = a.cin / CC;
  const int nqb = a.cin / 32;
  constexpr int K = 27;

  ST_STAMP(0);
  const unsigned char* lr = local + (size_t)tile * LR_BYTES;
  const int* __restrict__ U = reinterpret_cast<const int*>(lr + 16);
  if (threadIdx.x < 8)
    *reinterpret_cast<float4*>(xs + (threadIdx.x >> 2) * LO_REGION + UMAX * 64 + (threadIdx.x & 3) * 16) = make_float4(0.f, 0.f, 0.f, 0.f);

  const unsigned long long wbits = (unsigned long long)(size_t)a.w;
  u32x4 wr;
  wr[0] = (unsigned)__builtin_amdgcn_readfirstlane((int)(unsigned)wbits);
  wr[1] = (unsigned)__builtin_amdgcn_readfirstlane((int)((unsigned)(wbits >> 32) & 0xFFFFu));
  wr[2] = (unsigned)__builtin_amdgcn_readfirstlane(K * a.cin * a.cout * 4);
  wr[3] = 0x00020000u;
  const int tile4 = CC * CT / 4;
  const unsigned int kstride = (unsigned)(n_slices * ncc * tile4 * 16);
  const unsigned int w1off = JQ * 1024;
  if ((unsigned)(size_t)(__attribute__((address_space(3))) unsigned char*)xs != 0u) __builtin_trap();

  f32x16 A0, A1, A2, A3;
#pragma unroll
  for (int i = 0; i < 16; ++i) { A0[i] = 0.f; A1[i] = 0.f; A2[i] = 0.f; A3[i] = 0.f; }

  int n_up = 0;
  int Ureg[NITV];
  auto load_rows = [&](int pass) {
#pragma unroll
    for (int it = 0; it < NITV; ++it) Ureg[it] = U[pass * UMAX + (it * NWV + wave) * 16 + (lane >> 2)];
  };
  auto stage = [&](int pass, int qb) {
    if constexpr (SKIP == 6) return;
#pragma unroll
    for (int it = 0; it < NITV; ++it) {
      const int l0 = (it * NWV + wave) * 16;
      if (l0 < n_up) {
        const int l = l0 + (lane >> 2);
        const float* src = a.in + (size_t)Ureg[it] * a.ld_in + qb * 32 + (((lane & 3) ^ ((l >> 2) & 3)) << 2);
        if (l < n_up) {
          __builtin_amdgcn_global_load_lds(src, (__attribute__((address_space(3))) void*)(xs + l0 * 64), 16, 0, 0);
          __builtin_amdgcn_global_load_lds(src + 16, (__attribute__((address_space(3))) void*)(xs + LO_REGION + l0 * 64), 16, 0, 0);
        }
      }
    }
  };

  if (!phase) load_rows(0);
  int warm = 0;
  if (!phase && threadIdx.x < 27 * 64 * 8 / 128) warm = *reinterpret_cast<const int*>(lr + 16 + UCAP * 4 + threadIdx.x * 128);
  const int n_u = __builtin_amdgcn_readfirstlane(reinterpret_cast<const int*>(lr)[0]);
  const int n_pass = n_u > UMAX ? 2 : 1;
  const int ks = __builtin_amdgcn_readfirstlane((int)blockIdx.y);
  const int i0 = ks * (n_pass * nqb) / ksplit, i1 = phase ? 0 : (ks + 1) * (n_pass * nqb) / ksplit;
  bool first = true;
  for (int pass = 0; pass < n_pass; ++pass) {
    const int q_lo = max(i0 - pass * nqb, 0), q_hi = min(i1 - pass * nqb, nqb);
    if (q_lo >= q_hi) continue;
    n_up = min(n_u - pass * UMAX, UMAX);
    if (pass > 0) load_rows(pass);
    const unsigned int* mp = reinterpret_cast<const unsigned int*>(lr + MASK_OFF + pass * MASK_PASS_BYTES);
    u32x8 M0, M1;
#pragma unroll
    for (int i = 0; i < 8; ++i) {
      M0[i] = (unsigned)__builtin_amdgcn_readfirstlane((int)mp[i]) >> (w0 * 4);
      M1[i] = i < 6 ? (unsigned)__builtin_amdgcn_readfirstlane((int)mp[8 + i]) >> (w0 * 4) : 0u;
    }
    const unsigned char* lb = lr + 16 + UCAP * 4 + ((size_t)pass * 27 * 64 + w0 * 16) * 8;
#ifdef EYOC_ST_QBREV
    for (int qbr = q_lo; qbr < q_hi; ++qbr) {
      const int qb = q_hi - 1 - (qbr - q_lo);
#else
    for (int qb = q_lo; qb < q_hi; ++qb) {
#endif
      if (!first) __syncthreads();
#ifdef EYOC_ST_DELAY_PRE
      if (first) { asm volatile("s_waitcnt vmcnt(0)" ::: "memory"); for (int z_ = 0; z_ < EYOC_ST_DELAY_PRE; ++z_) __builtin_amdgcn_s_sleep(127); }
#endif
      first = false;
      stage(pass, qb);
      const int cc = (qb * 32) / CC, qp = ((qb * 32) % CC) / 32;
      const unsigned int ws0 = (unsigned)__builtin_amdgcn_readfirstlane(((slice * ncc + cc) * tile4 + (nt0 * JQ + 2 * qp) * 64) * 16);
      unsigned int so;
#ifdef EYOC_ST_DELAY
      if (pass == 0 && qb == q_lo) { asm volatile("s_waitcnt vmcnt(0)" ::: "memory"); for (int z_ = 0; z_ < EYOC_ST_DELAY; ++z_) __builtin_amdgcn_s_sleep(127); }
#endif
#ifdef EYOC_ST_TRACE
      unsigned long long tb = 0, tb1 = 0, tb2 = 0;
      const int blk_i = pass * nqb + qb;
      if (blk_i < 2) ST_STAMP(2 + 3 * blk_i);
      if (blk_i == 0) ST_STAMP(1);
#endif
#define EYOC_ST_OPERANDS                                                                                                            \
  [wr] "s"(wr), [ws0] "s"(ws0), [ks] "s"(kstride), [lb] "s"(lb), [w1] "s"(w1off), "{s[36:43]}"(M0), "{s[44:51]}"(M1)
#define EYOC_ST_ASM_NH2(TEXT)                                                                                                       \
  asm volatile(TEXT : "+{v[64:79]}"(A0), "+{v[80:95]}"(A1), "+{v[96:111]}"(A2), "+{v[112:127]}"(A3), [so] "=&s"(so)                   \
               : EYOC_ST_OPERANDS : "memory", "scc", EYOC_ST_LOOP_CLOBBERS)
#ifdef EYOC_ST_TRACE
      if constexpr (NH == 2 && SKIP == 1) {
        asm volatile(EYOC_ST_LOOP_NH2_TRACE : "+{v[64:79]}"(A0), "+{v[80:95]}"(A1), "+{v[96:111]}"(A2), "+{v[112:127]}"(A3), [so] "=&s"(so), [tb] "=&s"(tb), [tb1] "=&s"(tb1), [tb2] "=&s"(tb2)
                     : EYOC_ST_OPERANDS : "memory", "scc", EYOC_ST_LOOP_CLOBBERS);
        if (blk_i < 2) {
          if (threadIdx.x == 0 && blockIdx.x < TRACE_WGS) {
            g_st_trace[blockIdx.x * TRACE_N + 3 + 3 * blk_i] = tb;
            g_st_trace[blockIdx.x * TRACE_N + 10 + 2 * blk_i] = tb1;
            g_st_trace[blockIdx.x * TRACE_N + 11 + 2 * blk_i] = tb2;
          }
          ST_STAMP(4 + 3 * blk_i);
        }
      } else
#endif
      if constexpr (NH == 2 && (SKIP == 1 || SKIP == 6 || SKIP == 7 || SKIP == 15)) EYOC_ST_ASM_NH2(EYOC_ST_LOOP_NH2);
      else if constexpr (NH == 2 && SKIP == 0) EYOC_ST_ASM_NH2(EYOC_ST_LOOP_NH2_NOSKIP);
#ifdef EYOC_ST_ABLATIONS
      else if constexpr (NH == 2 && SKIP == 2) EYOC_ST_ASM_NH2(EYOC_ST_LOOP_NH2_LAZY);
      else if constexpr (NH == 2 && SKIP == 3) EYOC_ST_ASM_NH2(EYOC_ST_LOOP_NH2_NOW);
      else if constexpr (NH == 2 && SKIP == 4) EYOC_ST_ASM_NH2(EYOC_ST_LOOP_NH2_NOX);
      else if constexpr (NH == 2 && SKIP == 5) EYOC_ST_ASM_NH2(EYOC_ST_LOOP_NH2_NOV);
      else if constexpr (NH == 2 && SKIP == 8) EYOC_ST_ASM_NH2(EYOC_ST_LOOP_NH2_NOM);
// ... 34 lines not shown
                     : EYOC_ST_OPERANDS : "memory", "scc", EYOC_ST_LOOP_CLOBBERS);
#undef EYOC_ST_ASM_NH2
#undef EYOC_ST_OPERANDS
    }
  }

  asm volatile("" :: "v"(warm));
  if constexpr (NH == 1 && NWV == NW && !T128) {
    if (ksplit > 1) {
      constexpr int NR4 = 8;
      float4* P = reinterpret_cast<float4*>(a.ks_part) + (size_t)((tile * n_cg + cg) * ksplit) * NR4 * 256;
      if (phase == 0) {
        float4* mine = P + (size_t)ks * NR4 * 256 + threadIdx.x;
#pragma unroll
        for (int r = 0; r < NR4; ++r) {
          const f32x16& A = r < 4 ? A0 : A1;
          mine[r * 256] = make_float4(A[(r & 3) * 4], A[(r & 3) * 4 + 1], A[(r & 3) * 4 + 2], A[(r & 3) * 4 + 3]);
        }
        return;
      }
#pragma unroll
      for (int i = 0; i < 16; ++i) { A0[i] = 0.f; A1[i] = 0.f; }
      for (int k = 0; k < ksplit; ++k) {
        const float4* src = P + (size_t)k * NR4 * 256 + threadIdx.x;
#pragma unroll
        for (int r = 0; r < NR4; ++r) {
          const float4 v = src[r * 256];
          f32x16& A = r < 4 ? A0 : A1;
          A[(r & 3) * 4] += v.x; A[(r & 3) * 4 + 1] += v.y; A[(r & 3) * 4 + 2] += v.z; A[(r & 3) * 4 + 3] += v.w;
        }
      }
    }
  }
  const float os = a.out_scale ? *a.out_scale : 1.0f;
  const int ch = ct0 + 8 * g;
  float4 b4[NTW];
#pragma unroll
  for (int t = 0; t < NTW; ++t)
    b4[t] = a.bias ? *reinterpret_cast<const float4*>(a.bias + ch + 4 * t) : make_float4(0.f, 0.f, 0.f, 0.f);
  float mx = 0.f;
  constexpr int NG = NH * NC;
  int orow[NG];
#pragma unroll
  for (int h = 0; h < NH; ++h) {
    const unsigned int rm = *reinterpret_cast<const unsigned int*>(lr + RM_OFF + ((w0 + h) * 16 + j) * 4);
#pragma unroll
    for (int c = 0; c < NC; ++c) orow[h * NC + c] = tile * TR + (int)((rm >> (8 * c)) & 255u);
  }
  uint4 rh[NG], rl[NG];
  if (a.res) {
#pragma unroll
    for (int hc = 0; hc < NG; ++hc) {
      const int o = orow[hc];
      if (o < a.n_out) {
        const char* rp = reinterpret_cast<const char*>(a.res + (size_t)o * a.ld_res) + split16_off4(ch);
        rh[hc] = *reinterpret_cast<const uint4*>(rp);
        rl[hc] = *reinterpret_cast<const uint4*>(rp + SPLIT16_LO);
      }
    }
  }
  float4 v[NG][NTW];
#pragma unroll
  for (int hc = 0; hc < NG; ++hc) {
    const int o = orow[hc];
#pragma unroll
    for (int t = 0; t < NTW; ++t) {
      const int ai = (hc * NTW + t) * 4;
      const f32x16& A = ai < 16 ? A0 : ai < 32 ? A1 : ai < 48 ? A2 : A3;
      v[hc][t] = make_float4(A[ai % 16 + 0] * os + b4[t].x, A[ai % 16 + 1] * os + b4[t].y, A[ai % 16 + 2] * os + b4[t].z,
                             A[ai % 16 + 3] * os + b4[t].w);
    }
    if (a.res && o < a.n_out) {
      const float4 q0 = split16_decode4(make_uint2(rh[hc].x, rh[hc].y), make_uint2(rl[hc].x, rl[hc].y));
      const float4 q1 = split16_decode4(make_uint2(rh[hc].z, rh[hc].w), make_uint2(rl[hc].z, rl[hc].w));
      v[hc][0].x += q0.x; v[hc][0].y += q0.y; v[hc][0].z += q0.z; v[hc][0].w += q0.w;
      v[hc][1].x += q1.x; v[hc][1].y += q1.y; v[hc][1].z += q1.z; v[hc][1].w += q1.w;
    }
#pragma unroll
    for (int t = 0; t < NTW; ++t) {
      if (a.relu) { v[hc][t].x = fmaxf(v[hc][t].x, 0.f); v[hc][t].y = fmaxf(v[hc][t].y, 0.f); v[hc][t].z = fmaxf(v[hc][t].z, 0.f); v[hc][t].w = fmaxf(v[hc][t].w, 0.f); }
      if (o < a.n_out) split16_track(mx, v[hc][t]);
    }
  }
  if constexpr (TAILF != 0) {
    const TailFuse& tf = a.tail;
    const bool odd = (wave & 1) != 0;
    uint4 Xh[NG], Xl[NG];
#pragma unroll
    for (int hc = 0; hc < NG; ++hc) {
      uint2 h0, l0, h1, l1;
      split16_encode4(v[hc][0], h0, l0);
      split16_encode4(v[hc][1], h1, l1);
      Xh[hc] = make_uint4(h0.x, h0.y, h1.x, h1.y);
      Xl[hc] = make_uint4(l0.x, l0.y, l1.x, l1.y);
    }
    auto sel4 = [](bool c, const uint4 x, const uint4 y) { return make_uint4(c ? x.x : y.x, c ? x.y : y.y, c ? x.z : y.z, c ? x.w : y.w); };
    constexpr int NK = NG / 2;
    int myrow[NK];
    uint4 Oh[NK], Ol[NK], Sh[NK], Sl[NK];
#pragma unroll
    for (int k = 0; k < NK; ++k) {
      myrow[k] = odd ? orow[NK + k] : orow[k];
      Oh[k] = sel4(odd, Xh[NK + k], Xh[k]);
      Ol[k] = sel4(odd, Xl[NK + k], Xl[k]);
      const int o = myrow[k] < a.n_out ? myrow[k] : a.n_out - 1;
      const char* sp = reinterpret_cast<const char*>(tf.skip + (size_t)o * tf.ld_skip) + g * 16;
      Sh[k] = *reinterpret_cast<const uint4*>(sp);
      Sl[k] = *reinterpret_cast<const uint4*>(sp + SPLIT16_LO);
    }
    auto load_w1 = [&](int cc, half8_t (&W)[4][2]) {
#pragma unroll
      for (int nt = 0; nt < 4; ++nt)
#pragma unroll
        for (int p = 0; p < 2; ++p)
          W[nt][p] = *reinterpret_cast<const half8_t*>(reinterpret_cast<const char*>(tf.w1) + ((cc * 4 + nt) * 2 + p) * 1024 + lane * 16);
    };
    half8_t Wc[2][4][2];
    load_w1(0, Wc[0]);
    half8_t W2[2][2][2];
    auto load_w2 = [&]() {
#pragma unroll
      for (int nt = 0; nt < 2; ++nt)
#pragma unroll
        for (int kb = 0; kb < 2; ++kb)
#pragma unroll
          for (int p = 0; p < 2; ++p) {
            const char* f = reinterpret_cast<const char*>(tf.w2) + (nt * 4 + 2 * kb + p) * 1024 + (((g >> 1) * 16 + j) * 16) + 8 * (g & 1);
            const uint2 lo = *reinterpret_cast<const uint2*>(f), hi = *reinterpret_cast<const uint2*>(f + 512);
            W2[nt][kb][p] = __builtin_bit_cast(half8_t, make_uint4(lo.x, lo.y, hi.x, hi.y));
          }
    };
    const float os1 = *tf.s1, os2 = *tf.s2;
    float4 b1[4], b2[2];
#pragma unroll
    for (int t = 0; t < 4; ++t) b1[t] = *reinterpret_cast<const float4*>(tf.b1 + 16 * t + 4 * g);
#pragma unroll
    for (int t = 0; t < 2; ++t) b2[t] = *reinterpret_cast<const float4*>(tf.b2 + 16 * t + 4 * g);
    lds_barrier();
    unsigned char* xw = xs + (size_t)(wave * NK) * 2048 + lane * 16;
#pragma unroll
    for (int k = 0; k < NK; ++k) {
      *reinterpret_cast<uint4*>(xw + k * 2048) = sel4(odd, Xh[k], Xh[NK + k]);
      *reinterpret_cast<uint4*>(xw + k * 2048 + 1024) = sel4(odd, Xl[k], Xl[NK + k]);
    }
    lds_barrier();
    const unsigned char* xr = xs + (size_t)((wave ^ 1) * NK) * 2048 + lane * 16;
    uint4 Ph[NK], Pl[NK];
#pragma unroll
    for (int k = 0; k < NK; ++k) {
      Ph[k] = *reinterpret_cast<const uint4*>(xr + k * 2048);
      Pl[k] = *reinterpret_cast<const uint4*>(xr + k * 2048 + 1024);
    }
    f32x4 acc1[NK][4];
#pragma unroll
    for (int k = 0; k < NK; ++k)
#pragma unroll
      for (int t = 0; t < 4; ++t) acc1[k][t] = f32x4{0.f, 0.f, 0.f, 0.f};
#pragma unroll
    for (int cc = 0; cc < 3; ++cc) {
      if (cc < 2) load_w1(cc + 1, Wc[(cc + 1) & 1]);
      else load_w2();
#pragma unroll
      for (int k = 0; k < NK; ++k) {
        const bool mine = cc == (odd ? 1 : 0);
        const uint4 xh = cc == 2 ? Sh[k] : sel4(mine, Oh[k], Ph[k]), xl = cc == 2 ? Sl[k] : sel4(mine, Ol[k], Pl[k]);
        const half8_t X0 = __builtin_bit_cast(half8_t, xh), X1 = __builtin_bit_cast(half8_t, xl);
#pragma unroll
        for (int term = 0; term < 3; ++term)
#pragma unroll
          for (int t = 0; t < 4; ++t)
            acc1[k][t] = __builtin_amdgcn_mfma_f32_16x16x32_f16(Wc[cc & 1][t][term == 2 ? 1 : 0], term == 1 ? X1 : X0, acc1[k][t], 0, 0, 0);
      }
    }
    const bool poisoned = split16_poisoned(a.range) || split16_over(mx);
    const float qnan = __builtin_nanf("");
    float mx2 = 0.f;
#pragma unroll
    for (int k = 0; k < NK; ++k) {
      half8_t Y[2][2];
      float cmx = 0.f;
#pragma unroll
      for (int t = 0; t < 4; ++t) {
        float4 u = make_float4(acc1[k][t][0] * os1 + b1[t].x, acc1[k][t][1] * os1 + b1[t].y, acc1[k][t][2] * os1 + b1[t].z, acc1[k][t][3] * os1 + b1[t].w);
        if (tf.relu1) { u.x = fmaxf(u.x, 0.f); u.y = fmaxf(u.y, 0.f); u.z = fmaxf(u.z, 0.f); u.w = fmaxf(u.w, 0.f); }
        split16_track(cmx, u);
        uint2 h, l;
        split16_encode4(u, h, l);
        const half4_t h4 = __builtin_bit_cast(half4_t, h), l4 = __builtin_bit_cast(half4_t, l);
#pragma unroll
        for (int r = 0; r < 4; ++r) { Y[t >> 1][0][4 * (t & 1) + r] = h4[r]; Y[t >> 1][1][4 * (t & 1) + r] = l4[r]; }
      }
      f32x4 o2[2];
#pragma unroll
      for (int t = 0; t < 2; ++t) o2[t] = f32x4{0.f, 0.f, 0.f, 0.f};
#pragma unroll
      for (int kb = 0; kb < 2; ++kb)
#pragma unroll
        for (int term = 0; term < 3; ++term)
#pragma unroll
          for (int t = 0; t < 2; ++t)
            o2[t] = __builtin_amdgcn_mfma_f32_16x16x32_f16(W2[t][kb][term == 2 ? 1 : 0], Y[kb][term == 1 ? 1 : 0], o2[t], 0, 0, 0);
      float4 w[2];
      float ss = 0.f;
#pragma unroll
      for (int t = 0; t < 2; ++t) {
        w[t] = make_float4(o2[t][0] * os2 + b2[t].x, o2[t][1] * os2 + b2[t].y, o2[t][2] * os2 + b2[t].z, o2[t][3] * os2 + b2[t].w);
        ss += w[t].x * w[t].x + w[t].y * w[t].y + w[t].z * w[t].z + w[t].w * w[t].w;
      }
      if (tf.l2norm) {
        ss += __shfl_xor(ss, 16, 64);
        ss += __shfl_xor(ss, 32, 64);
        const float inv = 1.0f / sqrtf(ss);
#pragma unroll
        for (int t = 0; t < 2; ++t) { w[t].x *= inv; w[t].y *= inv; w[t].z *= inv; w[t].w *= inv; }
      }
      if (myrow[k] < a.n_out) mx2 = split16_merge(mx2, cmx);
      cmx = split16_merge(cmx, __shfl_xor(cmx, 16, 64));
      cmx = split16_merge(cmx, __shfl_xor(cmx, 32, 64));
      const bool bad = poisoned || split16_over(cmx);
      if (myrow[k] < a.n_out) {
        const size_t oo = tf.out_perm ? (size_t)tf.out_perm[myrow[k]] : (size_t)myrow[k];
#pragma unroll
        for (int t = 0; t < 2; ++t)
          *reinterpret_cast<float4*>(tf.out + oo * tf.ld_out + 16 * t + 4 * g) = bad ? make_float4(qnan, qnan, qnan, qnan) : w[t];
      }
    }
    if (a.range) {
      if (split16_over(mx)) { atomicOr(a.range + 4, 1u); atomicOr(a.range + 3, 1u); }
      if (split16_over(mx2)) { atomicOr(a.range + 5, 1u); atomicOr(a.range + 3, 1u); }
      if (__builtin_nontemporal_load(a.range + 2)) atomicMax(a.range + 1, __float_as_uint(split16_merge(mx, mx2)) & 0x7FFFFFFFu);
    }
    return;
  }
#pragma unroll
  for (int hc = 0; hc < NG; ++hc) {
    const int o = orow[hc];
    if (o >= a.n_out) continue;
    if (SKIP == 7 && os != 12345.f) continue;
    if (a.out_split) {
      uint2 h0, l0, h1, l1;
      split16_encode4(v[hc][0], h0, l0);
      split16_encode4(v[hc][1], h1, l1);
      char* op = reinterpret_cast<char*>(a.out + (size_t)o * a.ld_out) + split16_off4(ch);
      *reinterpret_cast<uint4*>(op) = make_uint4(h0.x, h0.y, h1.x, h1.y);
      *reinterpret_cast<uint4*>(op + SPLIT16_LO) = make_uint4(l0.x, l0.y, l1.x, l1.y);
    } else {
      float* op = a.out + (size_t)o * a.ld_out + ch;
      *reinterpret_cast<float4*>(op) = v[hc][0];
      *reinterpret_cast<float4*>(op + 4) = v[hc][1];
    }
  }
  if (a.out_split) split16_report(a.range, mx);
#ifdef EYOC_ST_TRACE
  asm volatile("s_waitcnt vmcnt(0)" ::: "memory");
  ST_STAMP(8);
  if (threadIdx.x == 0 && blockIdx.x < TRACE_WGS) {
    unsigned int hw;
    asm volatile("s_getreg_b32 %0, hwreg(HW_REG_HW_ID)" : "=s"(hw));
    unsigned int xcc;
    asm volatile("s_getreg_b32 %0, hwreg(HW_REG_XCC_ID)" : "=s"(xcc));
    g_st_trace[blockIdx.x * TRACE_N + 9] = ((unsigned long long)xcc << 32) | hw;
  }
#endif
}

}

#ifdef EYOC_ST_TRACE
extern "C" int eyoc_debug_st_trace(unsigned long long* host, size_t n) {
  if (n > (size_t)TRACE_WGS * TRACE_N) n = (size_t)TRACE_WGS * TRACE_N;
  if (hipMemcpyFromSymbol(host, HIP_SYMBOL(g_st_trace), n * 8) != hipSuccess) return -1;
  unsigned long long* z = (unsigned long long*)calloc(n, 8);
  (void)hipMemcpyToSymbol(HIP_SYMBOL(g_st_trace), z, n * 8);
  free(z);
  return 0;
}
#endif

namespace eyoc {

size_t local_rulebook_bytes(int n_out) { return (size_t)cdiv(n_out, TILE) * LR_BYTES; }

int build_local_rulebook(const int32_t* nbr_dev, int K, int n_out, unsigned char* out_dev, int* overflow_dev, hipStream_t st, int group) {
  if (n_out <= 0) return EYOC_OK;
  hipLaunchKernelGGL((k_local_rulebook<false, 4>), dim3(cdiv(n_out, TILE)), dim3(256), 0, st, nbr_dev, K, n_out, out_dev, overflow_dev, group, DeriveSrc());
  EYOC_CHECK_HIP(hipGetLastError());
  return EYOC_OK;
}

int build_local_rulebook_derived(const DeriveSrc& src, int n_out, unsigned char* out_dev, int* overflow_dev, hipStream_t st, int group) {
  if (n_out <= 0) return EYOC_OK;
  EYOC_REQUIRE(src.coords && src.parent && src.children && src.s1c && src.nc > 0, EYOC_ERR_INVALID, "build_local_rulebook_derived: incomplete octree");
  hipLaunchKernelGGL((k_local_rulebook<true, 4>), dim3(cdiv(n_out, TILE)), dim3(256), 0, st, (const int32_t*)nullptr, 27, n_out, out_dev, overflow_dev, group, src);
  EYOC_CHECK_HIP(hipGetLastError());
  return EYOC_OK;
}

#ifdef EYOC_ST_ABLATIONS
constexpr int ST_VARIANTS = 28;
#else
constexpr int ST_VARIANTS = 7;
#endif
int st_variants() { return ST_VARIANTS; }

bool spconv_st_can_fuse_tail(const SpconvArgs& a) {
  if (a.math != 1 || !a.local || a.l2norm || a.K != 27 || a.cout != 64 || a.cin % 32 != 0 || !a.out_split || a.out_perm) return false;
  const eyoc_ctx::Knobs& kn = knobs_of(a.ctx);
  const int v = kn.st_variant;
  if (!(v == 1 || v == 4 || v == 5 || v == 6)) return false;
  const int n_tiles = cdiv(a.n_out, TILE);
  return !((long long)n_tiles * (a.cout / 64) < kn.st_split_below);
}

__global__ __launch_bounds__(256) void k_tail_poison(unsigned int* __restrict__ range, float* __restrict__ out, int n, int ld, int c) {
  const unsigned int stored = __builtin_nontemporal_load(range + 4), inter = __builtin_nontemporal_load(range + 5);
  if (blockIdx.x == 0 && threadIdx.x == 0 && (stored | inter)) atomicOr(range, 1u);
  if (stored == 0u) return;
  const float qnan = __builtin_nanf("");
  for (long long i = (long long)blockIdx.x * 256 + threadIdx.x; i < (long long)n * c; i += (long long)gridDim.x * 256)
    out[(i / c) * ld + i % c] = qnan;
}

int launch_spconv_st(const SpconvArgs& a_in, const unsigned char* local_dev, hipStream_t st) {
  const SpconvArgs& a = a_in;
  EYOC_REQUIRE(a.math == 1 && local_dev && !a.l2norm && a.K == 27 && !a.perm, EYOC_ERR_INVALID, "spconv_st: unsupported layer");
  const int n_tiles = cdiv(a.n_out, TILE);
  const eyoc_ctx::Knobs& kn = knobs_of(a.ctx);
  const int split_below = kn.st_split_below;
  const int variant0 = kn.st_variant;
  const bool small = variant0 != 0 && a.cout >= 64 && a.cout <= 256 && (long long)n_tiles * (a.cout / 64) < split_below;
  const int ctg = a.cout >= 64 && !small ? 64 : 32;
  const bool wide = spconv_cc(a.cin, a.cout) == 64;
  const int n_cg = a.cout / ctg;
  EYOC_REQUIRE(a.cout % ctg == 0 && n_cg >= 1 && n_cg <= 8 && 8 % n_cg == 0 && a.cin % 32 == 0, EYOC_ERR_INVALID,
               "spconv_st: %d -> %d channels", a.cin, a.cout);
  SpconvArgs a_loc = a_in;
  a_loc.cg_local = (kn.st_cg_local && n_cg > 1 && variant0 != 0 && (size_t)27 * a.cin * a.cout * 4 <= (size_t)2 << 20) ? 1 : 0;
  const SpconvArgs& a2 = a_loc;
  dim3 grid((unsigned)(a_loc.cg_local ? cdiv(n_tiles, 8) * 8 * n_cg : cdiv(n_tiles, 8 / n_cg) * 8)), block(NW * 64);
  const int variant = kn.st_variant;
  int ksplit = 1;
  if (variant == 1 && ctg == 32 && a.ks_part && kn.st_ksplit && a.cin >= 128) {
    const int wgs = (int)grid.x, nqb = a.cin / 32;
    ksplit = KS_MAX_SLOTS / (wgs > 0 ? wgs : 1);
    if (ksplit > nqb) ksplit = nqb;
    if (ksplit < 4 || (long long)n_tiles * n_cg > KS_MAX_SLOTS) ksplit = 1;
// ... 63 lines not shown
  const dim3 grid((unsigned)(cdiv(n_tiles, 8 / n_cg) * 8)), block(NW * 64);
  if (wide_wg) {
    if (spconv_cc(a.cin, a.cout) == 64) hipLaunchKernelGGL((spconv_st_asm_kernel<64, 2, 1, NW, 128>), grid, block, 0, st, a, local_dev, n_tiles, 1, 0);
    else hipLaunchKernelGGL((spconv_st_asm_kernel<32, 2, 1, NW, 128>), grid, block, 0, st, a, local_dev, n_tiles, 1, 0);
    EYOC_CHECK_HIP(hipGetLastError());
    return EYOC_OK;
  }
  const int nh1 = knobs_of(a.ctx).st_variant;
  const bool deep = nh1 != 4;
#ifdef EYOC_ST_ABLATIONS
  const int v_ = knobs_of(a.ctx).st_variant;
#define EYOC_ST128_ABL(SK_)                                                                                                         \
  do {                                                                                                                              \
    if (spconv_cc(a.cin, a.cout) == 64) hipLaunchKernelGGL((spconv_st_asm_kernel<64, 1, SK_, NW, 128>), grid, block, 0, st, a, local_dev, n_tiles, 1, 0); \
    else hipLaunchKernelGGL((spconv_st_asm_kernel<32, 1, SK_, NW, 128>), grid, block, 0, st, a, local_dev, n_tiles, 1, 0);          \
    EYOC_CHECK_HIP(hipGetLastError());                                                                                              \
    return EYOC_OK;                                                                                                                 \
  } while (0)
  if (v_ == 16) EYOC_ST128_ABL(6);
  if (v_ == 17) EYOC_ST128_ABL(7);
  if (v_ == 23) EYOC_ST128_ABL(13);
  if (v_ == 18) EYOC_ST128_ABL(8);
  if (v_ == 19) EYOC_ST128_ABL(9);
  if (v_ == 20) EYOC_ST128_ABL(10);
  if (v_ == 21) EYOC_ST128_ABL(11);
#undef EYOC_ST128_ABL
#endif
  if (nh1 == 5 || nh1 == 6) {
    if (spconv_cc(a.cin, a.cout) == 64) {
      if (nh1 == 5) hipLaunchKernelGGL((spconv_st_asm_kernel<64, 1, 19, NW, 128>), grid, block, 0, st, a, local_dev, n_tiles, 1, 0);
      else hipLaunchKernelGGL((spconv_st_asm_kernel<64, 1, 20, NW, 128>), grid, block, 0, st, a, local_dev, n_tiles, 1, 0);
    } else {
      if (nh1 == 5) hipLaunchKernelGGL((spconv_st_asm_kernel<32, 1, 19, NW, 128>), grid, block, 0, st, a, local_dev, n_tiles, 1, 0);
      else hipLaunchKernelGGL((spconv_st_asm_kernel<32, 1, 20, NW, 128>), grid, block, 0, st, a, local_dev, n_tiles, 1, 0);
    }
    EYOC_CHECK_HIP(hipGetLastError());
    return EYOC_OK;
  }
  if (spconv_cc(a.cin, a.cout) == 64) {
    if (deep) hipLaunchKernelGGL((spconv_st_asm_kernel<64, 1, 18, NW, 128>), grid, block, 0, st, a, local_dev, n_tiles, 1, 0);
    else hipLaunchKernelGGL((spconv_st_asm_kernel<64, 1, 1, NW, 128>), grid, block, 0, st, a, local_dev, n_tiles, 1, 0);
  } else {
    if (deep) hipLaunchKernelGGL((spconv_st_asm_kernel<32, 1, 18, NW, 128>), grid, block, 0, st, a, local_dev, n_tiles, 1, 0);
    else hipLaunchKernelGGL((spconv_st_asm_kernel<32, 1, 1, NW, 128>), grid, block, 0, st, a, local_dev, n_tiles, 1, 0);
  }
  EYOC_CHECK_HIP(hipGetLastError());
  return EYOC_OK;
}

size_t local_rulebook128_bytes(int n_out) { return (size_t)cdiv(n_out, 128) * LR_BYTES; }

int build_local_rulebook128(const int32_t* nbr_dev, int K, int n_out, unsigned char* out_dev, int* overflow_dev, hipStream_t st, int group) {
  if (n_out <= 0) return EYOC_OK;
  hipLaunchKernelGGL((k_local_rulebook<false, 2>), dim3(cdiv(n_out, 128)), dim3(128), 0, st, nbr_dev, K, n_out, out_dev, overflow_dev, group, DeriveSrc());
  EYOC_CHECK_HIP(hipGetLastError());
  return EYOC_OK;
}

}
```

### eyoc_amd/harness.py

```python
from __future__ import annotations

import contextlib
import copy
import json
import logging
from dataclasses import dataclass, field
from typing import NamedTuple

import numpy as np
import torch

from . import _lib, icp
from . import registration as reg
from .eval import gather_rows, knn1_segmented
from .isolate import batch_drop, remap_rows
from .metrics import registration_errors
from .sparse_tensor import CoordinateManager, SparseTensor
from .synthetic import batch_coords, plant_correspondences, subsample_indices
from .voxelize import sparse_quantize_batch


@dataclass
class RegistrationConfig:
    model: str = "ResUNetBN2C"
    model_n_out: int = 32
    conv1_kernel_size: int = 5
    normalize_feature: bool = True
    bn_momentum: float = 0.05
    voxel_size: float = 0.3
    n_points: int = 5000
    use_RANSAC: bool = True
    ransac_max_iteration: int = 4000000
    rte_thresh: float = 2.0
    rre_thresh: float = 5.0
    sc2pcr: dict = field(default_factory=lambda: dict(
        inlier_threshold=0.6, num_node=8000, use_mutual=False, d_thre=0.1, num_iterations=20, ratio=0.2,
        nms_radius=0.6, max_points=8000, k1=30, k2=20))
    fp32_retry_per_step: bool = False
    isolate_failures: bool = False
    icp_refine: bool = False
    icp_max_correspondence_distance: float | None = None
    icp_max_iteration: int = 30


RETRIED_FP32 = 1 << 4
DROPPED_DUPLICATE = 1 << 0
DROPPED_RANGE = 1 << 1
DROPPED_EMPTY = 1 << 2
DROPPED_NONFINITE = 1 << 3
DROPPED = DROPPED_DUPLICATE | DROPPED_RANGE | DROPPED_EMPTY | DROPPED_NONFINITE
MAX_REBUILDS = 2


def pairs_of_clouds(clouds, offsets, P):
    n_clouds = len(offsets) - 1
    if n_clouds != 2 * P:
        raise ValueError(f"{n_clouds} clouds for {P} pairs")
    clouds = np.asarray(list(clouds), np.int64)
    if clouds.size and (clouds.min() < 0 or clouds.max() >= n_clouds):
        raise ValueError(f"cloud {int(clouds.max() if clouds.max() >= n_clouds else clouds.min())} is not one of the batch's {n_clouds}")
    return clouds // 2


def fault_bits(dup, rng, offsets, P):
    bits = np.zeros(P, np.int64)
    np.bitwise_or.at(bits, pairs_of_clouds(dup, offsets, P), DROPPED_DUPLICATE)
    np.bitwise_or.at(bits, pairs_of_clouds(rng, offsets, P), DROPPED_RANGE)
    return bits


def live_segments(dropped, n_points):
    return np.concatenate([[0], np.cumsum(np.where(np.asarray(dropped) == 0, int(n_points), 0))]).astype(np.int64)


def build_with_isolation(batch, build, fault_batches):
    first = None
    for attempt in range(MAX_REBUILDS + 1):
        try:
            return build(batch), batch
        except _lib.EyocError as e:
            if e.code not in (_lib.ERR_DUPLICATE, _lib.ERR_RANGE):
                raise
            first = first or _lib.EyocError(str(e), e.code)
            if attempt == MAX_REBUILDS:
                raise first
            dup, rng = fault_batches()
            bits = fault_bits(dup, rng, batch.offsets, batch.P)
            if not bits[batch.dropped == 0].any():
                raise first
            batch = batch.without_pairs(bits)


# ... 186 lines not shown

    def wait(self):
        self.done.synchronize()
        self.keep = None
        overflow = bool(int(self.words[0]) != 0)
        self.status = np.zeros(self.host.shape[0], np.int64) if self.dropped is None else np.array(self.dropped, np.int64)
        if overflow and self.retry is not None:
            pipe, batch, seed, maps, slot = self.retry
            again = pipe._retry_fp32(batch, seed, maps, slot, pipelined=True)
            self.host.copy_(again.result.cpu())
            if self.icp is not None:
                self.icp.copy_(again.icp.cpu())
            self.status |= RETRIED_FP32
        self.retry = None
        return self.host, overflow


_CALLERS_STREAM = contextlib.nullcontext()


class RegistrationPipeline:
    def __init__(self, model, config: RegistrationConfig | None = None):
        self.model = model
        self.cfg = config or RegistrationConfig()
        self.matcher = None if self.cfg.use_RANSAC else reg.Matcher(**self.cfg.sc2pcr)
        self.timing = False
        self.slot = 0
        self._ev = None
        self.fp32_retries = 0
        self.dropped_pairs = 0
        self.featured = self.matched = self.last_nn_idx = None
        self.registered_batch = None
        self.last_icp = None
        self._icp_dev = None
        self.side_priority = 0
        self._side = self._tail = None
        self._pinned, self._pinned_w, self._stage = {}, {}, {}
        self._range_words = None
        self._ransac_budget = None

    def _mark(self, step, i):
        if step.timers is not None:
            step.timers[i].record()

    def stage_ms(self, slot=None):
        e = self._ev[self.slot if slot is None else slot]
        e[3].synchronize()
        return {"feat": e[0].elapsed_time(e[1]), "match": e[1].elapsed_time(e[2]), "reg": e[2].elapsed_time(e[3])}

    @torch.no_grad()
    def features(self, batch: DeviceBatch, maps=None) -> SparseTensor:
        return self._features(batch, maps)[0]

    def _features(self, batch, maps):
        check, self.model.range_check = self.model.range_check, False
        try:
            if maps is None and not self.cfg.isolate_failures:
                return self.model(SparseTensor(batch.feats, coordinates=batch.coords)), batch
            if maps is None:
                cm, batch = self._build_maps(batch)
            else:
                cm, ready, reduced = maps
                torch.cuda.current_stream().wait_event(ready)
                if self.cfg.isolate_failures and reduced is not batch:
                    batch = reduced
                    batch.record_stream(torch.cuda.current_stream())
            return self.model(SparseTensor(batch.feats, coordinate_manager=cm)), batch
        finally:
            self.model.range_check = check

    def _build_maps(self, batch):
        def build(b):
            cm = CoordinateManager(b.coords)
            cm.maps(-1)
            return cm
        if not self.cfg.isolate_failures:
            return build(batch), batch
        return build_with_isolation(batch, build, lambda: _lib.fault_batches(batch.coords.device))

    @contextlib.contextmanager
    def _accept_degenerate(self, device):
        if not self.cfg.isolate_failures:
            yield
            return
        prev = _lib.knob("eyoc_registration_accept_degenerate", 1, device=device)
        try:
            yield
        finally:
            _lib.knob("eyoc_registration_accept_degenerate", prev, device=device)

    def _step(self, batch, seed, maps, slot, timed, tail=None, read_back=False):
        if timed and self._ev is None:
            self._ev = [[torch.cuda.Event(enable_timing=True) for _ in range(4)] for _ in range(2)]
        step = _Step(slot, self._ev[slot] if timed else None)
        main = torch.cuda.current_stream()
        self._mark(step, 0)
        F, step.batch = self._features(batch, maps)
        step.F = F.F
        self._mark(step, 1)
        if read_back:
            step.words = self._pinned_words(slot)
            if tail is not None:
                self.model.range_snapshot(step.words)
        step.featured = torch.cuda.Event()
        step.featured.record(main)
        if tail is not None:
            tail.wait_event(step.featured)
        with _CALLERS_STREAM if tail is None else torch.cuda.stream(tail):
            if tail is not None and self.cfg.isolate_failures and step.batch.dropped.any():
                step.batch.record_stream(tail)
            step.result = (self._match_and_register if self.cfg.use_RANSAC else self._match_and_register_sc2)(step, seed)
            self._mark(step, 3)
            if read_back:
                step.host = self._pinned_set(slot, step.result)
                step.host.copy_(step.result, non_blocking=True)
                if self.cfg.icp_refine:
                    step.icp_host = self._pinned_set(slot, step.icp)
                    step.icp_host.copy_(step.icp, non_blocking=True)
                if tail is None:
                    self.model.range_snapshot(step.words)
                step.done = torch.cuda.Event()
                step.done.record(main if tail is None else tail)
        return step

    def _publish(self, step, count_dropped=True):
        self.featured, self.matched, self.last_nn_idx, self._icp_dev = step.featured, step.matched, step.nn_idx, step.icp
        if self.cfg.isolate_failures:
            self.registered_batch = step.batch
            if count_dropped:
                self.dropped_pairs += int((step.batch.dropped != 0).sum())
        return step

    @torch.no_grad()
    def _retry_fp32(self, batch, seed, maps, slot, pipelined):
        self.fp32_retries += 1
        if pipelined:
            try:
                self.model.check_range()
            except _lib.EyocError as e:
                if e.code != _lib.ERR_RANGE:
                    raise
        math, self.model.spconv_math = self.model.spconv_math, "fp32"
        try:
            return self._step(batch, seed, maps, slot, self.timing and not pipelined)
        finally:
            self.model.spconv_math = math

    @torch.no_grad()
    def prepare_maps(self, batch: DeviceBatch, after=None) -> MapsHandle:
        if self._side is None:
# ... 184 lines not shown
```

### eyoc_amd/model.py

```python
from __future__ import annotations

import ctypes as C
import itertools
import logging

import numpy as np
import torch
import torch.nn as nn

from . import _lib
from .sparse_tensor import SparseTensor

_TENSOR_VERSION = torch.Tensor._version.__get__
_TENSOR_PTR = torch.Tensor.data_ptr


class _Conv(nn.Module):

    def __init__(self, K, cin, cout, bias=False):
        super().__init__()
        shape = (cin, cout) if K == 1 else (K, cin, cout)
        self.kernel = nn.Parameter(torch.randn(shape) * float(np.sqrt(2.0 / (K * cin))))
        self.bias = nn.Parameter(torch.zeros(1, cout)) if bias else None
        self.K, self.cin, self.cout = K, cin, cout
# ... 140 lines not shown

    def repack(self):
        return self.pack(self._packed_device)

    def pack_host(self) -> torch.Tensor:
        lib = _lib.load()
        blob = torch.zeros(self.blob_floats(), dtype=torch.float32)
        d = self._desc()
        layers, nl, keep = self._layer_params()
        _lib.check(lib.eyoc_model_pack_host(C.byref(d), layers, nl, C.c_void_p(blob.data_ptr()), blob.numel()), "eyoc_model_pack_host")
        del keep
        return blob

    def pack(self, device=None, blob: torch.Tensor | None = None, from_blob=False):
        lib = _lib.load()
        device = torch.device(device) if device is not None else self.final.kernel.device
        if device.type != "cuda":
            raise _lib.EyocError("the model runs on the GPU only: call model.to('cuda') first")
        self._invalidate()
        n = self.blob_floats()
        if blob is None:
            blob = torch.zeros(n + 64, dtype=torch.float32, device=device)
            off = ((-blob.data_ptr()) % 256) // 4
            blob = blob[off:off + n]
        d = self._desc()
        h = C.c_void_p()
        with torch.cuda.device(device):
            if from_blob:
                rc = lib.eyoc_model_create(_lib.ctx(device.index), C.byref(d), None, 0, _lib.ptr(blob), blob.numel(),
                                           C.byref(h))
            else:
                layers, nl, keep = self._layer_params()
                rc = lib.eyoc_model_create(_lib.ctx(device.index), C.byref(d), layers, nl, _lib.ptr(blob),
                                           blob.numel(), C.byref(h))
        _lib.check(rc, "eyoc_model_create")
        self._handle, self._blob, self._packed_device = h, blob, device
        self._packed_version = None if from_blob else self._weights_version()
        if self._timing:
            _lib.check(lib.eyoc_model_set_timing(h, 1), "eyoc_model_set_timing")
        if self._math != -1:
            lib.eyoc_model_set_math(h, self._math)
        if self._probe:
            _lib.check(lib.eyoc_model_set_probe(h, 1), "eyoc_model_set_probe")
        self._apply_progress()
        return blob

    @property
    def weight_blob(self):
        if self._handle is None:
            self.pack()
        return self._blob

    def forward(self, x: SparseTensor) -> SparseTensor:
        if not isinstance(x, SparseTensor):
            raise TypeError("expected an eyoc_amd.SparseTensor")
        if x.F.shape[1] != self.in_channels:
            raise ValueError(f"features have {x.F.shape[1]} channels, model expects {self.in_channels}")
        if self.training:
            from .train import forward_layers
            return forward_layers(self, x)
        dev = x.device
        if self._handle is None or self._packed_device != dev:
            self.pack(dev)
        elif self._packed_version is not None and self._packed_version != self._weights_version():
            self.pack(dev)
        lib = _lib.load()
        cm = x.coordinate_manager
        maps = cm.maps(-1)
        cm._reading()
        out = torch.empty((len(x), self.out_channels), dtype=torch.float32, device=dev)
        with torch.cuda.device(dev):
            ws = _lib.workspace(lib.eyoc_model_workspace_bytes(self._handle, maps), dev)

            def run():
                _lib.check(lib.eyoc_model_forward(_lib.ctx(dev.index), self._handle, maps, _lib.ptr(x.F), _lib.ptr(out),
                                                  _lib.ptr(ws), ws.numel(), _lib.stream_ptr()), "eyoc_model_forward")
            run()
            if self.range_check and lib.eyoc_model_last_math(self._handle) == 1:
                try:
                    self.check_range()
                except _lib.EyocError as e:
                    if e.code != _lib.ERR_RANGE or self._math != -1:
                        raise
                    logging.warning("eyoc_amd: split16 arithmetic overflowed (an activation reached 6e4); re-running "
                                    "this forward with fp32 MFMAs - set model.spconv_math = 'fp32' for this checkpoint")
                    lib.eyoc_model_set_math(self._handle, 0)
                    try:
                        run()
                    finally:
                        lib.eyoc_model_set_math(self._handle, -1)
        return SparseTensor(out, coordinate_map_key=x.coordinate_map_key, coordinate_manager=cm)

    def check_range(self):
        if self._handle is None:
            return None
        mx = C.c_float(-1.0)
        with torch.cuda.device(self._packed_device):
            rc = _lib.load().eyoc_model_range_check(self._handle, _lib.stream_ptr(), C.byref(mx))
        self.last_max_activation = float(mx.value) if mx.value >= 0 else None
        _lib.check(rc, "eyoc_model_range_check")
        return self.last_max_activation

    def progress_event(self, layer: int):
        if layer is None:
            self._progress = None
        else:
            ev = torch.cuda.Event()
            ev.record()
            self._progress = (ev, int(layer))
        self._apply_progress()
        return None if layer is None else self._progress[0]

    def _apply_progress(self):
        pr = getattr(self, "_progress", None)
        if self._handle is not None:
            _lib.check(_lib.load().eyoc_model_set_progress_event(self._handle, 0 if pr is None else pr[1], None if pr is None else C.c_void_p(pr[0].cuda_event)),
                       "eyoc_model_set_progress_event")

    def range_snapshot(self, words: torch.Tensor):
        assert words.is_pinned() and words.dtype == torch.int32 and words.numel() >= 4
        if self._handle is None:
            words.zero_()
            return
        with torch.cuda.device(self._packed_device):
            _lib.check(_lib.load().eyoc_model_range_snapshot(self._handle, words.data_ptr(), _lib.stream_ptr()), "eyoc_model_range_snapshot")

    def probe_activations(self, on=True):
        self._probe = bool(on)
        if self._handle is not None:
            _lib.check(_lib.load().eyoc_model_set_probe(self._handle, 1 if on else 0), "eyoc_model_set_probe")
# ... 117 lines not shown
```

### eyoc_amd/sparse_tensor.py

```python
from __future__ import annotations

import ctypes as C

import torch

from . import _lib


class _DeviceArray:

    def __init__(self, ptr: int, shape, owner):
        self.__cuda_array_interface__ = {"shape": tuple(shape), "typestr": "<i4", "data": (ptr, False), "version": 2}
        self._owner = owner


class CoordinateManager:

    def __init__(self, coordinates: torch.Tensor):
        if coordinates.dim() != 2 or coordinates.shape[1] != 4:
            raise ValueError(f"coordinates must be [N,4] (batch,x,y,z), got {tuple(coordinates.shape)}")
        if not coordinates.is_cuda:
            raise _lib.EyocError("SparseTensor coordinates must live on the GPU (no CPU path)")
        self.coordinates = coordinates.to(torch.int32).contiguous()
        self._maps = None
        self._ws = None
        self._maps_caller = None
        self._ws_caller = None
        self._readers = set()

    @property
    def device(self):
        return self.coordinates.device

    def _build(self, order: int):
        lib = _lib.load()
        n = self.coordinates.shape[0]
        with torch.cuda.device(self.device):
            ws = _lib.workspace(lib.eyoc_maps_workspace_bytes(n), self.device)
            h = C.c_void_p()
            _lib.check(lib.eyoc_maps_build_ordered(_lib.ctx(self.device.index), _lib.ptr(self.coordinates), n,
                                                   _lib.ptr(ws), ws.numel(), _lib.stream_ptr(), int(order),
                                                   C.byref(h)), "eyoc_maps_build")
        return h, ws

    def _reading(self):
        try:
            h = torch._C._cuda_getCurrentRawStream(self.device.index)
        except AttributeError:
            h = torch.cuda.current_stream(self.device).cuda_stream
        if h in self._readers:
            return
        s = torch.cuda.current_stream(self.device)
        for ws in (self._ws, self._ws_caller):
            if ws is not None:
                ws.record_stream(s)
        self._readers.add(h)

    def maps(self, order: int = 0):
        if self._maps is None:
            self._maps, self._ws = self._build(order)
        return self._maps

    def _caller_maps(self):
        if not _lib.load().eyoc_maps_row_order(self.maps()):
            return self._maps
        if self._maps_caller is None:
            self._maps_caller, self._ws_caller = self._build(0)
            self._readers.clear()
        return self._maps_caller

    def rows(self, level: int) -> int:
        return int(_lib.load().eyoc_maps_rows(self.maps(), level))

    def level_coordinates(self, level: int, internal: bool = False) -> torch.Tensor:
        m = self.maps() if internal else self._caller_maps()
        n = self.rows(level)
        out = torch.empty((n, 4), dtype=torch.int32, device=self.device)
        self._reading()
        with torch.cuda.device(self.device):
            _lib.check(_lib.load().eyoc_maps_copy_coords(m, level, _lib.ptr(out), _lib.stream_ptr()), "eyoc_maps_copy_coords")
        return out

    def table(self, kind: int, level: int, internal: bool = False) -> torch.Tensor:
        m = self.maps() if internal else self._caller_maps()
        n_out = {0: self.rows(level), 1: self.rows(level + 1), 2: self.rows(level)}[kind]
        out = torch.empty((27, n_out), dtype=torch.int32, device=self.device)
        self._reading()
        with torch.cuda.device(self.device):
            _lib.check(_lib.load().eyoc_maps_copy_table(m, kind, level, _lib.ptr(out), _lib.stream_ptr()), "eyoc_maps_copy_table")
        return out

    def table_view(self, kind: int, level: int, internal: bool = False) -> torch.Tensor:
        m = self.maps() if internal else self._caller_maps()
        n_out = {0: self.rows(level), 1: self.rows(level + 1), 2: self.rows(level)}[kind]
        ptr = _lib.load().eyoc_maps_table(m, kind, level)
        if not ptr or n_out == 0:
            return self.table(kind, level, internal)
        self._reading()
        return torch.as_tensor(_DeviceArray(int(ptr), (27, n_out), self), device=self.device)

    def row_order(self) -> torch.Tensor | None:
        lib = _lib.load()
        if not lib.eyoc_maps_row_order(self.maps()):
            return None
        out = torch.empty((self.rows(0),), dtype=torch.int32, device=self.device)
        self._reading()
        with torch.cuda.device(self.device):
            _lib.check(lib.eyoc_maps_copy_row_order(self.maps(), _lib.ptr(out), _lib.stream_ptr()), "eyoc_maps_copy_row_order")
        return out

    def up_order(self, level: int, internal: bool = False) -> torch.Tensor:
        m = self.maps() if internal else self._caller_maps()
        out = torch.empty((self.rows(level),), dtype=torch.int32, device=self.device)
        self._reading()
        with torch.cuda.device(self.device):
            _lib.check(_lib.load().eyoc_maps_copy_up_order(m, level, _lib.ptr(out), _lib.stream_ptr()), "eyoc_maps_copy_up_order")
        return out

    def info(self, conv1_kernel_size: int = 0) -> dict:
        info = _lib.MapsInfo()
        m = self.maps()
        self._reading()
        with torch.cuda.device(self.device):
            _lib.check(_lib.load().eyoc_maps_info(_lib.ctx(self.device.index), m, conv1_kernel_size,
                                                  _lib.stream_ptr(), C.byref(info)), "eyoc_maps_info")
        L = info.n_levels
        return {"rows": list(info.rows[:L]), "pairs_s1": list(info.pairs_s1[:L]),
                "pairs_down": list(info.pairs_down[:L - 1]), "pairs_up": list(info.pairs_up[:L - 1]),
                "pairs_conv1": int(info.pairs_conv1)}

    def __del__(self):
        try:
            for name in ("_maps", "_maps_caller"):
                if getattr(self, name, None) is not None:
                    _lib.load().eyoc_maps_free(getattr(self, name))
                    setattr(self, name, None)
        except Exception:
            pass


class SparseTensor:
    def __init__(self, features: torch.Tensor, coordinates: torch.Tensor | None = None, device=None,
                 coordinate_map_key=None, coordinate_manager: CoordinateManager | None = None, **_unused):
        if device is not None:
            features = features.to(device)
            if coordinates is not None:
                coordinates = coordinates.to(device)
        if coordinate_manager is None:
            if coordinates is None:
                raise ValueError("either coordinates or coordinate_manager is required")
            coordinate_manager = CoordinateManager(coordinates)
        if features.dim() != 2 or features.shape[0] != coordinate_manager.coordinates.shape[0]:
            raise ValueError("features must be [N,C] with one row per coordinate")
        if not features.is_cuda:
            raise _lib.EyocError("SparseTensor features must live on the GPU (no CPU path)")
        self._F = features.to(torch.float32).contiguous()
        self.coordinate_manager = coordinate_manager
        self.coordinate_map_key = coordinate_map_key if coordinate_map_key is not None else (1, 1, 1)

    @property
    def F(self):
        return self._F
# ... 25 lines not shown
```

### include/eyoc_hip.h

```cpp
#ifndef EYOC_HIP_H
#define EYOC_HIP_H

#include <stddef.h>
#include <stdint.h>

#ifdef __cplusplus
extern "C" {
#endif

typedef struct eyoc_ctx eyoc_ctx;
typedef struct eyoc_maps eyoc_maps;
typedef struct eyoc_model eyoc_model;

typedef enum {
  EYOC_OK = 0,
  EYOC_ERR_INVALID = -1,
  EYOC_ERR_HIP = -2,
  EYOC_ERR_WORKSPACE = -3,
  EYOC_ERR_DUPLICATE = -4,
  EYOC_ERR_RANGE = -5
} eyoc_status;

#define EYOC_MAX_LEVELS 4
#define EYOC_VERSION 111

int eyoc_version(void);
const char* eyoc_last_error(void);
int eyoc_create(int device, eyoc_ctx** out);
int eyoc_destroy(eyoc_ctx* ctx);

typedef enum { EYOC_MAP_S1 = 0, EYOC_MAP_DOWN = 1, EYOC_MAP_UP = 2 } eyoc_map_kind;

typedef struct {
  int32_t n_levels;
  int32_t rows[EYOC_MAX_LEVELS];
  int64_t pairs_s1[EYOC_MAX_LEVELS];
  int64_t pairs_down[EYOC_MAX_LEVELS];
  int64_t pairs_up[EYOC_MAX_LEVELS];
  int64_t pairs_conv1;
} eyoc_maps_info_t;

size_t eyoc_maps_workspace_bytes(int n_rows);
int eyoc_maps_build(eyoc_ctx* ctx, const int32_t* coords_dev, int n_rows, void* workspace_dev,
                    size_t workspace_bytes, void* stream, eyoc_maps** out);
int eyoc_maps_build_ordered(eyoc_ctx* ctx, const int32_t* coords_dev, int n_rows, void* workspace_dev,
                            size_t workspace_bytes, void* stream, int order, eyoc_maps** out);
int eyoc_maps_last_fault_batches(const eyoc_ctx* ctx, uint32_t* dup, uint32_t* range);
int eyoc_maps_free(eyoc_maps* maps);
int eyoc_maps_copy_up_order(const eyoc_maps* maps, int level, int32_t* out_dev, void* stream);
int eyoc_maps_order_min_rows(eyoc_ctx* ctx, int min_rows);
int eyoc_maps_order_window_shift(eyoc_ctx* ctx, int shift);
int eyoc_maps_select_orders(eyoc_ctx* ctx, int s1, int down);
int eyoc_maps_internal_order(eyoc_ctx* ctx, int mode);
int eyoc_maps_lazy_tables(eyoc_ctx* ctx, int on);
int eyoc_maps_fused_levels(eyoc_ctx* ctx, int on);
int eyoc_spconv_select_down_kernel(eyoc_ctx* ctx, int mode);
const int32_t* eyoc_maps_row_order(const eyoc_maps* maps);
int eyoc_maps_copy_row_order(const eyoc_maps* maps, int32_t* out_dev, void* stream);
int eyoc_maps_rows(const eyoc_maps* maps, int level);
const int32_t* eyoc_maps_coords(const eyoc_maps* maps, int level);
const int32_t* eyoc_maps_table(const eyoc_maps* maps, int kind, int level);
int eyoc_maps_copy_coords(const eyoc_maps* maps, int level, int32_t* out_dev, void* stream);
int eyoc_maps_copy_table(const eyoc_maps* maps, int kind, int level, int32_t* out_dev, void* stream);
int eyoc_maps_info(eyoc_ctx* ctx, const eyoc_maps* maps, int conv1_kernel_size, void* stream,
                   eyoc_maps_info_t* info);

size_t eyoc_voxelize_workspace_bytes(int n_points);
int eyoc_voxelize(eyoc_ctx* ctx, const float* xyz_dev, int n_points, int stride, float voxel_size, int batch_index,
                  int32_t* sel_dev, int32_t* coords_dev, int* n_out, void* workspace_dev, size_t workspace_bytes,
                  void* stream);

size_t eyoc_voxelize_batched_workspace_bytes(int n_points_total, int n_clouds);
int eyoc_voxelize_batched(eyoc_ctx* ctx, const float* xyz_dev, int stride, const int64_t* point_offsets, int n_clouds,
                          int n_points, float voxel_size, int batch_base, int32_t* sel_dev, int32_t* coords_dev,
                          float* xyz_out_dev, int64_t* voxel_offsets, void* workspace_dev, size_t workspace_bytes,
                          void* stream);
size_t eyoc_voxelize_batched_isolating_workspace_bytes(int n_points_total, int n_clouds);
int eyoc_voxelize_batched_isolating(eyoc_ctx* ctx, const float* xyz_dev, int stride, const int64_t* point_offsets, int n_clouds,
                                    int n_points, float voxel_size, int batch_base, int32_t* sel_dev, int32_t* coords_dev,
                                    float* xyz_out_dev, int64_t* voxel_offsets, void* workspace_dev, size_t workspace_bytes,
                                    void* stream, int32_t* cloud_faults);

size_t eyoc_batch_drop_workspace_bytes(int n_rows);
int eyoc_batch_drop(eyoc_ctx* ctx, const int32_t* coords_dev, const float* feats_dev, int n_rows, int c, const uint32_t* drop_mask,
                    int32_t* coords_out_dev, float* feats_out_dev, int32_t* row_map_dev, int* n_kept, int32_t* kept_per_batch,
                    void* workspace_dev, size_t workspace_bytes, void* stream);
int eyoc_remap_rows(eyoc_ctx* ctx, const int64_t* idx_dev, int m, const int32_t* row_map_dev, int n_rows, int64_t* out_dev,
                    void* stream);

size_t eyoc_spconv_packed_floats(int K, int cin, int cout);
int eyoc_spconv_pack_weights(const float* w_host , const float* scale_host ,
                             int K, int cin, int cout, float* packed_host);
int eyoc_spconv(eyoc_ctx* ctx, const int32_t* nbr_dev, int K, int n_out, const float* in_dev,
                int ld_in, int cin, const float* wpacked_dev, int cout, const float* bias_dev,
                const float* res_dev, int ld_res, int relu, float* out_dev, int ld_out, void* stream);
int eyoc_spconv_select_split16_kernel(eyoc_ctx* ctx, int mode);
int eyoc_spconv_select_up_kernel(eyoc_ctx* ctx, int on);
int eyoc_spconv_upc_min_rows(eyoc_ctx* ctx, int rows);
int eyoc_spconv_upc_tile_rows(int odd_axes, int rows);
// ... 10 lines not shown
size_t eyoc_spconv_local_rulebook_bytes(int n_out);
int eyoc_spconv_build_local_rulebook(eyoc_ctx* ctx, const int32_t* nbr_dev, int K, int n_out, void* out_dev,
                                     int32_t* overflow_dev, void* stream);
int eyoc_spconv_staged(eyoc_ctx* ctx, const int32_t* nbr_dev, const void* local_dev, int n_out, int n_in, const float* in_dev,
                       int ld_in, int cin, const float* wpacked_dev, int cout, const float* bias_dev, const float* res_dev,
                       int ld_res, int relu, float* out_dev, int ld_out, int out_split, const float* out_scale_dev, void* stream);
int eyoc_spconv_pack_weights_split16(const float* w_host, const float* scale_host, int K, int cin, int cout,
                                     float* packed_host, float* out_scale_host);
int eyoc_spconv_ex(eyoc_ctx* ctx, const int32_t* nbr_dev, int K, int n_out, int n_in, const float* in_dev, int ld_in, int cin,
                   const float* wpacked_dev, int cout, const float* bias_dev, const float* res_dev, int ld_res, int relu,
                   float* out_dev, int ld_out, int math, int out_split, const float* out_scale_dev, void* stream);
int eyoc_split16_encode(eyoc_ctx* ctx, const float* in_dev, int n, int c, int ld_in, float* out_dev, int ld_out, void* stream);
int eyoc_split16_decode(eyoc_ctx* ctx, const float* in_dev, int n, int c, int ld_in, float* out_dev, int ld_out, void* stream);
int eyoc_spconv_sum(eyoc_ctx* ctx, const int32_t* nbr_dev, int K, int n_out, const float* in_dev, int ld_in, int cin,
                    const float* wpacked_dev, int cout, float* out_dev, int ld_out, void* stream);
int eyoc_spconv_pack_weights_transposed(const float* w_host , int K, int cin, int cout, int mirror,
                                        float* packed_host);
size_t eyoc_spconv_grad_weight_workspace_bytes(int K, int n_out, int cin, int cout);
int eyoc_spconv_grad_weight(eyoc_ctx* ctx, const int32_t* nbr_dev, int K, int n_out, const float* in_dev, int ld_in, int cin,
                            const float* dout_dev, int ld_dout, int cout, float* dw_dev, void* workspace_dev,
                            size_t workspace_bytes, void* stream);
int eyoc_spconv_select_kernel(eyoc_ctx* ctx, int mode);

typedef struct {
  int32_t in_channels, out_channels, conv1_kernel_size, normalize_feature;
  int32_t channels[5];
  int32_t tr_channels[5];
  float bn_eps;
  int32_t expanded;
} eyoc_model_desc;

typedef struct {
  const char* name;
  const float* kernel;
  int32_t K, cin, cout;
  const float* bias;
  const float* bn_weight;
  const float* bn_bias;
  const float* bn_mean;
  const float* bn_var;
} eyoc_layer_params;

size_t eyoc_model_blob_floats(const eyoc_model_desc* desc);
int eyoc_model_pack_host(const eyoc_model_desc* desc, const eyoc_layer_params* layers, int n_layers,
                         float* blob_host, size_t blob_floats);
int eyoc_model_create(eyoc_ctx* ctx, const eyoc_model_desc* desc, const eyoc_layer_params* layers,
                      int n_layers, float* blob_dev, size_t blob_floats, eyoc_model** out);
int eyoc_model_destroy(eyoc_model* model);
int eyoc_model_fuse_tail(eyoc_ctx* ctx, int on);
size_t eyoc_model_workspace_bytes(const eyoc_model* model, const eyoc_maps* maps);
int eyoc_model_forward(eyoc_ctx* ctx, const eyoc_model* model, const eyoc_maps* maps,
                       const float* feats_dev, float* out_dev, void* workspace_dev,
                       size_t workspace_bytes, void* stream);
int eyoc_model_num_layers(const eyoc_model* model);
int eyoc_model_layer_work(eyoc_ctx* ctx, const eyoc_model* model, const eyoc_maps* maps, void* stream,
                          const char** names, int64_t* pairs, double* flops, double* gather_bytes,
                          double* compulsory_bytes);
int eyoc_model_set_math(eyoc_model* model, int mode);
int eyoc_model_last_math(const eyoc_model* model);
int eyoc_model_range_check(eyoc_model* model, void* stream, float* max_abs);
int eyoc_model_range_snapshot(eyoc_model* model, uint32_t* words_host, void* stream);
int eyoc_model_set_progress_event(eyoc_model* model, int layer, void* hip_event);
int eyoc_model_set_probe(eyoc_model* model, int on);
int eyoc_model_set_timing(eyoc_model* model, int on);
int eyoc_model_layer_ms(eyoc_model* model, float* ms );
int eyoc_model_timing_slot(eyoc_model* model, int slot);

int eyoc_knn_prefilter(eyoc_ctx* ctx, int mode);
int eyoc_knn1(eyoc_ctx* ctx, const float* A_dev, const float* B_dev, int c, const int32_t* seg_a,
              const int32_t* seg_b, int nseg, int dist_type, int64_t* idx_dev, float* dist_dev,
              void* stream);

int eyoc_gather_rows(eyoc_ctx* ctx, const float* F_dev, int ld, int c, const int64_t* sel_dev, int n,
                     const float* G_dev, float beta, float* out_dev, void* stream);

int eyoc_dotmax(eyoc_ctx* ctx, const float* A_dev, const float* B_dev, int c, const int32_t* seg_a,
                const int32_t* seg_b, int nseg, int64_t* idx_dev, float* weight_dev, void* stream);

int eyoc_knn2(eyoc_ctx* ctx, const float* A_dev, const float* B_dev, int c, const int32_t* seg_a,
              const int32_t* seg_b, int nseg, int64_t* idx_dev, float* d1_dev, float* d2_dev, void* stream);

int eyoc_lowe_topk(eyoc_ctx* ctx, const float* d1_dev, const float* d2_dev, int n, int k, int64_t* idx_out_dev,
                   float* w_out_dev, void* stream);
int eyoc_pair_filter(eyoc_ctx* ctx, int mode, const float* P0_dev, const float* P1_dev, const int64_t* idx0_dev,
                     const int64_t* idx1_dev, int m, const float* T_dev, float radius, int64_t* pairs_out_dev,
                     int32_t* n_out_dev, void* stream);

int eyoc_pair_filter_similarity(eyoc_ctx* ctx, const float* P0_dev, const float* P1_dev, const int64_t* idx0_dev,
                                const int64_t* idx1_dev, int m, const double* table_dev, int xlim, int ylim, float grid0,
                                float grid1, double thresh, int64_t* pairs_out_dev, int32_t* n_out_dev, void* stream);

int eyoc_pdist(eyoc_ctx* ctx, const float* A_dev, int n, const float* B_dev, int m, int c, int dist_type,
               float* out_dev, void* stream);

int eyoc_kabsch_batched(eyoc_ctx* ctx, const float* A_dev, const float* B_dev, const float* w_dev,
                        int bs, int n, float* T_dev, void* stream);
int eyoc_irls_quad(eyoc_ctx* ctx, const float* p0_dev, const float* p1_dev, const float* w_dev, int n,
                   int iters, float* T_dev, void* stream);

size_t eyoc_bn_workspace_bytes(int n, int c);
int eyoc_bn_train_forward(eyoc_ctx* ctx, const float* x_dev, int n, int c, int ld_x, const float* gamma_dev, const float* beta_dev,
                          float eps, int relu, float* y_dev, int ld_y, float* mean_var_dev, void* workspace_dev, size_t workspace_bytes,
                          void* stream);
int eyoc_bn_train_forward_running(eyoc_ctx* ctx, const float* x_dev, int n, int c, int ld_x, const float* gamma_dev, const float* beta_dev,
                                  float eps, int relu, float* y_dev, int ld_y, float* mean_var_dev, float* running_mean_dev,
                                  float* running_var_dev, float momentum, void* workspace_dev, size_t workspace_bytes, void* stream);
// ... 89 lines not shown
```

Baseline: 3337 pairs/s.

## Compute final-layer features only for rows sampled for matching

Adds a build path that takes the list of sampled rows (the 5000-point NN subset), marks them in a bitmask, and tags unneeded rows in the level-0 tile rulebook. A rows-only forward then has the final fused spconv and tail compute outputs only for the needed rows, skipping final-layer work for voxels never used downstream. The cost is extra scatter and bitmask work during map building, and output rows outside the needed set are left unwritten. It is only used in the pipeline when the spconv math is not fp32.

```diff
diff --git a/eyoc_amd/_lib.py b/eyoc_amd/_lib.py
--- a/eyoc_amd/_lib.py
+++ b/eyoc_amd/_lib.py
@@ -72,6 +72,9 @@
     "eyoc_maps_workspace_bytes": (_sz, [_i]),
     "eyoc_maps_build": (_i, [_vp, _vp, _i, _vp, _sz, _vp, C.POINTER(_vp)]),
     "eyoc_maps_build_ordered": (_i, [_vp, _vp, _i, _vp, _sz, _vp, _i, C.POINTER(_vp)]),
+    "eyoc_maps_build_needed": (_i, [_vp, _vp, _i, _vp, _sz, _vp, _i, _vp, C.c_int64, C.POINTER(_vp)]),
+    "eyoc_maps_has_needed_rows": (_i, [_vp]),
+    "eyoc_maps_copy_tile_records": (_i, [_vp, _i, _vp, _sz, _vp]),
     "eyoc_maps_free": (_i, [_vp]),
     "eyoc_maps_last_fault_batches": (_i, [_vp, _vp, _vp]),
     "eyoc_maps_internal_order": (_i, [_vp, _i]),
@@ -140,6 +143,7 @@
     "eyoc_model_fuse_tail": (_i, [_vp, _i]),
     "eyoc_model_workspace_bytes": (_sz, [_vp, _vp]),
     "eyoc_model_forward": (_i, [_vp, _vp, _vp, _vp, _vp, _vp, _sz, _vp]),
+    "eyoc_model_forward_rows": (_i, [_vp, _vp, _vp, _vp, _vp, _vp, _sz, _vp]),
     "eyoc_model_num_layers": (_i, [_vp]),
     "eyoc_model_layer_work": (_i, [_vp, _vp, _vp, _vp, C.POINTER(C.c_char_p), C.POINTER(C.c_int64),
                                    C.POINTER(C.c_double), C.POINTER(C.c_double), C.POINTER(C.c_double)]),
diff --git a/eyoc_amd/csrc/common.h b/eyoc_amd/csrc/common.h
--- a/eyoc_amd/csrc/common.h
+++ b/eyoc_amd/csrc/common.h
@@ -163,6 +163,7 @@
   unsigned char* local_s1w[EYOC_MAX_LEVELS] = {nullptr, nullptr, nullptr, nullptr};
   unsigned char* local_down[EYOC_MAX_LEVELS] = {nullptr, nullptr, nullptr, nullptr};
   unsigned char* local_upc[EYOC_MAX_LEVELS] = {nullptr, nullptr, nullptr, nullptr};
+  bool need_list = false, need_records = false;
   bool table0_built = false;
   bool s1_ready[EYOC_MAX_LEVELS] = {true, true, true, true};
   bool up_ready[EYOC_MAX_LEVELS] = {true, true, true, true};
diff --git a/eyoc_amd/csrc/coordmap.hip b/eyoc_amd/csrc/coordmap.hip
--- a/eyoc_amd/csrc/coordmap.hip
+++ b/eyoc_amd/csrc/coordmap.hip
@@ -632,6 +632,18 @@
   if (code == EYOC_ERR_RANGE) memcpy(ctx->fault_range, h + 32, 32 * sizeof(uint32_t));
 }
 
+__global__ __launch_bounds__(256) void k_need_scatter(const long long* __restrict__ rows, long long n_need, int n, unsigned int* __restrict__ bits,
+                                                      int* __restrict__ bad) {
+  for (long long i = (long long)blockIdx.x * 256 + threadIdx.x; i < n_need; i += (long long)gridDim.x * 256) {
+    const long long r = rows[i];
+    if (r < 0 || r >= n) atomicAdd(bad, 1);
+    else if (bits) atomicOr(bits + (r >> 5), 1u << (r & 31));
+  }
+}
+
+int maps_build_impl(eyoc_ctx* ctx, const int32_t* coords_dev, int n, void* ws, size_t ws_bytes, void* stream, int order, bool has_need,
+                    const int64_t* need_rows, int64_t n_need, eyoc_maps** out);
+
 }
 
 extern "C" {
@@ -654,6 +666,7 @@
   b += 2 * (align_up(upc_kept_bytes(n_rows)) + align_up(upc_scratch_bytes(n_rows))) + EYOC_MAX_LEVELS * (align_up(upc_kept_bytes(1)) + align_up(upc_scratch_bytes(1)) + 512);
   b += 4 * (align_up(local_rulebook128_bytes(n_rows)) + 256);
   b += 4096;
+  b += align_up(((n + 31) / 32) * 4) + 256;
   return b + 96 * 256;
 }
 
@@ -664,6 +677,33 @@
 
 int eyoc_maps_build_ordered(eyoc_ctx* ctx, const int32_t* coords_dev, int n, void* ws, size_t ws_bytes, void* stream,
                             int order, eyoc_maps** out) {
+  return maps_build_impl(ctx, coords_dev, n, ws, ws_bytes, stream, order, false, nullptr, 0, out);
+}
+
+int eyoc_maps_build_needed(eyoc_ctx* ctx, const int32_t* coords_dev, int n, void* ws, size_t ws_bytes, void* stream, int order,
+                           const int64_t* needed_rows_dev, int64_t n_needed, eyoc_maps** out) {
+  EYOC_REQUIRE(n_needed >= 0 && (n_needed == 0 || needed_rows_dev), EYOC_ERR_INVALID, "eyoc_maps_build_needed: %lld needed rows at %p",
+               (long long)n_needed, (const void*)needed_rows_dev);
+  return maps_build_impl(ctx, coords_dev, n, ws, ws_bytes, stream, order, true, needed_rows_dev, n_needed, out);
+}
+
+int eyoc_maps_has_needed_rows(const eyoc_maps* maps) { return maps && maps->need_list ? 1 : 0; }
+
+int eyoc_maps_copy_tile_records(const eyoc_maps* maps, int level, void* out_dev, size_t out_bytes, void* stream) {
+  EYOC_REQUIRE(maps && out_dev && level >= 0 && level < maps->n_levels, EYOC_ERR_INVALID, "eyoc_maps_copy_tile_records: bad argument");
+  EYOC_REQUIRE(maps->local_s1[level], EYOC_ERR_INVALID, "eyoc_maps_copy_tile_records: level %d has no tile records (maps in the caller's order)", level);
+  const size_t bytes = local_rulebook_bytes(maps->rows[level]);
+  EYOC_REQUIRE(out_bytes >= bytes, EYOC_ERR_WORKSPACE, "eyoc_maps_copy_tile_records: %zu < %zu bytes", out_bytes, bytes);
+  EYOC_CHECK_HIP(hipMemcpyAsync(out_dev, maps->local_s1[level], bytes, hipMemcpyDeviceToDevice, (hipStream_t)stream));
+  return EYOC_OK;
+}
+
+}
+
+namespace {
+
+int maps_build_impl(eyoc_ctx* ctx, const int32_t* coords_dev, int n, void* ws, size_t ws_bytes, void* stream, int order, bool has_need,
+                    const int64_t* need_rows, int64_t n_need, eyoc_maps** out) {
   if (ctx) {
     memset(ctx->fault_dup, 0, sizeof(ctx->fault_dup));
     memset(ctx->fault_range, 0, sizeof(ctx->fault_range));
@@ -700,6 +740,18 @@
   const eyoc_ctx::Knobs& kn = ctx->knobs;
   const int order_mode = kn.maps_internal_order >= 0 ? kn.maps_internal_order : order;
   const bool zorder = order_mode > 0 || (order_mode < 0 && n >= ZORDER_MIN_ROWS);
+  unsigned int* need_bits = nullptr;
+  if (has_need) {
+    if (zorder) {
+      need_bits = cv.take<unsigned int>((size_t)(n + 31) / 32);
+      if (need_bits) FAIL_HIP(hipMemsetAsync(need_bits, 0, (size_t)((n + 31) / 32) * 4, st));
+    }
+    if (n_need > 0) {
+      const long long nb = (n_need + 255) / 256;
+      hipLaunchKernelGGL(k_need_scatter, dim3((unsigned)(nb < 4096 ? nb : 4096)), dim3(256), 0, st, (const long long*)need_rows, (long long)n_need, n,
+                         need_bits, counters + 14);
+    }
+  }
   int pre_rows[EYOC_MAX_LEVELS] = {n, 0, 0, 0};
   if (zorder) {
     unsigned long long* zk_in = cv.take<unsigned long long>(n);
@@ -813,6 +865,11 @@
       FAIL_HIP(hipMemcpyAsync(host, counters + 2 + l, sizeof(int), hipMemcpyDeviceToHost, st));
       FAIL_HIP(hipStreamSynchronize(st));
     }
+    if (l == 1 && host[128 + 14] != 0) {
+      set_error("eyoc_maps_build_needed: %d needed rows outside [0, %d)", host[128 + 14], n);
+      delete m;
+      return EYOC_ERR_INVALID;
+    }
     if (l == 1 && host[1] != 0) {
       set_error("eyoc_maps_build: %d coordinate rows outside the supported key range (|c| < 2^17 - 16, 0 <= batch < 1024)", host[1]);
       keep_fault_masks(ctx, host + 128 + 64, EYOC_ERR_RANGE);
@@ -946,8 +1003,9 @@
         DeriveSrc src;
         src.coords = m->coords[0]; src.parent = m->parent[0]; src.children = m->children[0]; src.s1c = m->nbr_s1[1];
         src.nc = m->rows[1]; src.sh = 0; src.up8 = m->up8[0];
-        if (int rc = build_local_rulebook_derived(src, m->rows[0], m->local_s1[0], counters + 8, st, kn.st_group)) { delete m; return rc; }
-      } else if (int rc = build_local_rulebook(m->nbr_s1[l], 27, m->rows[l], m->local_s1[l], counters + 8, st, kn.st_group)) { delete m; return rc; }
+        if (int rc = build_local_rulebook_derived(src, m->rows[0], m->local_s1[0], counters + 8, st, kn.st_group, need_bits, m->row_perm)) { delete m; return rc; }
+      } else if (int rc = build_local_rulebook(m->nbr_s1[l], 27, m->rows[l], m->local_s1[l], counters + 8, st, kn.st_group,
+                                               l == 0 ? need_bits : nullptr, l == 0 ? m->row_perm : nullptr)) { delete m; return rc; }
       if (l + 1 < EYOC_MAX_LEVELS && use_up) {
         m->local_up[l] = cv.take<unsigned char>(local_rulebook_up_bytes(m->rows[l]));
         if (int rc = build_local_rulebook_up(m->nbr_up[l], 27, m->rows[l], m->local_up[l], counters + 9, st)) { delete m; return rc; }
@@ -996,10 +1054,16 @@
         delete m;
         return EYOC_ERR_INVALID;
       }
+    if (host[6] != 0) {
+      set_error("eyoc_maps_build_needed: %d needed rows outside [0, %d)", host[6], n);
+      delete m;
+      return EYOC_ERR_INVALID;
+    }
     if (host[0] != 0) {
       for (int l = 0; l < EYOC_MAX_LEVELS; ++l) m->local_s1[l] = nullptr;
       if (int rc = maps_ensure_table(m, EYOC_MAP_S1, 0, st)) { delete m; return rc; }
     }
+    m->need_records = need_bits != nullptr && m->local_s1[0] != nullptr;
     if (host[1] != 0)
       for (int l = 0; l < EYOC_MAX_LEVELS; ++l) m->local_up[l] = nullptr;
     for (int l = 0; l + 1 < EYOC_MAX_LEVELS; ++l)
@@ -1019,9 +1083,14 @@
     delete m;
     return EYOC_ERR_WORKSPACE;
   }
+  m->need_list = has_need;
   *out = m;
   return EYOC_OK;
 }
+
+}
+
+extern "C" {
 
 size_t eyoc_voxelize_workspace_bytes(int n_points) {
   if (n_points < 0) return 0;
diff --git a/eyoc_amd/csrc/model.hip b/eyoc_amd/csrc/model.hip
--- a/eyoc_amd/csrc/model.hip
+++ b/eyoc_amd/csrc/model.hip
@@ -409,8 +409,8 @@
   return EYOC_OK;
 }
 
-int eyoc_model_forward(eyoc_ctx* ctx, const eyoc_model* mc, const eyoc_maps* maps, const float* feats_dev, float* out_dev,
-                       void* ws, size_t ws_bytes, void* stream) {
+static int model_forward_impl(eyoc_ctx* ctx, const eyoc_model* mc, const eyoc_maps* maps, const float* feats_dev, float* out_dev,
+                              void* ws, size_t ws_bytes, void* stream, bool rows_only) {
   EYOC_REQUIRE(ctx && mc && maps && feats_dev && out_dev && ws, EYOC_ERR_INVALID, "eyoc_model_forward: NULL argument");
   EYOC_REQUIRE(ws_bytes >= eyoc_model_workspace_bytes(mc, maps), EYOC_ERR_WORKSPACE,
                "eyoc_model_forward: workspace %zu < required %zu bytes", ws_bytes, eyoc_model_workspace_bytes(mc, maps));
@@ -528,6 +528,7 @@
           a.tail.w1 = m->blob + q1.w16_off; a.tail.s1 = m->blob + q1.s_off; a.tail.b1 = m->blob + q1.b_off; a.tail.relu1 = q1.relu;
           a.tail.w2 = m->blob + q2.w16_off; a.tail.s2 = m->blob + q2.s_off; a.tail.b2 = m->blob + q2.b_off; a.tail.l2norm = q2.l2norm;
           a.tail.out = buf[q2.out_buf] + q2.out_col; a.tail.ld_out = m->bufs[q2.out_buf].width; a.tail.out_perm = maps->row_perm;
+          a.needed_only = rows_only && p.level == 0 && maps->need_records && a.local == maps->local_s1[0] ? 1 : 0;
           rc = launch_spconv(a, st);
           if (rc) return rc;
           if (m->timing)
@@ -544,6 +545,18 @@
   if (!progress_recorded) EYOC_CHECK_HIP(hipEventRecord(m->progress_event, st));
   if (m->timing) m->events_valid[m->slot] = 1;
   return EYOC_OK;
+}
+
+int eyoc_model_forward(eyoc_ctx* ctx, const eyoc_model* mc, const eyoc_maps* maps, const float* feats_dev, float* out_dev,
+                       void* ws, size_t ws_bytes, void* stream) {
+  return model_forward_impl(ctx, mc, maps, feats_dev, out_dev, ws, ws_bytes, stream, false);
+}
+
+int eyoc_model_forward_rows(eyoc_ctx* ctx, const eyoc_model* mc, const eyoc_maps* maps, const float* feats_dev, float* out_dev,
+                            void* ws, size_t ws_bytes, void* stream) {
+  EYOC_REQUIRE(maps && maps->need_list, EYOC_ERR_INVALID, "eyoc_model_forward_rows: the maps were built without a list of needed rows "
+               "(eyoc_maps_build_needed)");
+  return model_forward_impl(ctx, mc, maps, feats_dev, out_dev, ws, ws_bytes, stream, true);
 }
 
 int eyoc_model_set_progress_event(eyoc_model* m, int layer, void* hip_event) {
diff --git a/eyoc_amd/csrc/spconv.h b/eyoc_amd/csrc/spconv.h
--- a/eyoc_amd/csrc/spconv.h
+++ b/eyoc_amd/csrc/spconv.h
@@ -49,6 +49,7 @@
   float* offset_part = nullptr;
   int cg_local = 0;
   TailFuse tail;
+  int needed_only = 0;
 };
 constexpr int KS_MAX_SLOTS = 1024;
 constexpr size_t KS_PART_BYTES = (size_t)KS_MAX_SLOTS * 256 * 32 * 4;
@@ -127,7 +128,8 @@
 int launch_spconv_upc(const SpconvArgs& a, const unsigned char* ws, hipStream_t st);
 int st_variants();
 size_t local_rulebook_bytes(int n_out);
-int build_local_rulebook(const int32_t* nbr_dev, int K, int n_out, unsigned char* out_dev, int* overflow_dev, hipStream_t st, int group = 1);
+int build_local_rulebook(const int32_t* nbr_dev, int K, int n_out, unsigned char* out_dev, int* overflow_dev, hipStream_t st, int group = 1,
+                         const unsigned int* need = nullptr, const int32_t* need_perm = nullptr);
 struct DeriveSrc {
   const int32_t* coords = nullptr;
   const int32_t* parent = nullptr;
@@ -139,7 +141,8 @@
 size_t local_rulebook128_bytes(int n_out);
 int build_local_rulebook128(const int32_t* nbr_dev, int K, int n_out, unsigned char* out_dev, int* overflow_dev, hipStream_t st, int group = 1);
 int launch_spconv_st128(const SpconvArgs& a, const unsigned char* local_dev, hipStream_t st);
-int build_local_rulebook_derived(const DeriveSrc& src, int n_out, unsigned char* out_dev, int* overflow_dev, hipStream_t st, int group = 1);
+int build_local_rulebook_derived(const DeriveSrc& src, int n_out, unsigned char* out_dev, int* overflow_dev, hipStream_t st, int group = 1,
+                                 const unsigned int* need = nullptr, const int32_t* need_perm = nullptr);
 int launch_spconv_rs(const SpconvArgs& a, hipStream_t st);
 bool tail_fusable(int cin1, int cmid, int cout);
 int launch_tail_fused(const float* in, int ld_in, int n, const float* w1, const float* s1, const float* b1, int relu1, const float* w2,
@@ -172,6 +175,7 @@
   const eyoc_ctx* ctx = nullptr;
 };
 constexpr int ST_TILE = 256, ST_UMAX = 639, ST_UCAP = 1280, ST_NPASS = 2, ST_LOC_OFF = 16 + ST_UCAP * 4, ST_INV_OFF = 33152, ST_LR_BYTES = 33408;
+constexpr int ST_HDR_NEED_MASK = 1, ST_HDR_NEED_UNIQUE = 2;
 int launch_conv1(const Conv1Args& a, hipStream_t st);
 bool conv1_walks_octree(const Conv1Args& a);
 
diff --git a/eyoc_amd/csrc/spconv_st.hip b/eyoc_amd/csrc/spconv_st.hip
--- a/eyoc_amd/csrc/spconv_st.hip
+++ b/eyoc_amd/csrc/spconv_st.hip
@@ -30,6 +30,8 @@
 static_assert(INV_OFF == ST_INV_OFF, "spconv.h mirrors this layout");
 static_assert(TILE == ST_TILE && UMAX == ST_UMAX && UCAP == ST_UCAP && NPASS == ST_NPASS && LR_BYTES == ST_LR_BYTES, "spconv.h mirrors this layout");
 static_assert(LR_BYTES % 128 == 0, "records start on cache lines");
+constexpr int HDR_NEED_MASK = 1, HDR_NEED_UNIQUE = 2;
+static_assert(HDR_NEED_MASK == ST_HDR_NEED_MASK && HDR_NEED_UNIQUE == ST_HDR_NEED_UNIQUE, "spconv.h mirrors this layout");
 #ifndef EYOC_LR_HSLOTS_LOG2
 #define EYOC_LR_HSLOTS_LOG2 11
 #endif
@@ -37,19 +39,23 @@
 
 template <bool DERIVE, int NWB>
 __global__ __launch_bounds__(NWB * 64) void k_local_rulebook(const int32_t* __restrict__ nbr, int K, int n_out, unsigned char* __restrict__ out,
-                                                             int* __restrict__ overflow, int group, DeriveSrc d) {
+                                                             int* __restrict__ overflow, int group, DeriveSrc d,
+                                                             const unsigned int* __restrict__ need, const int32_t* __restrict__ need_perm) {
   constexpr int TR = NWB * 64;
   constexpr int HS = HSLOTS_T, HSHIFT = 32 - HSLOTS_LOG2;
   __shared__ int hk[HS];
   __shared__ unsigned short hid[HS];
   __shared__ unsigned short srow[27][TR];
   __shared__ __attribute__((aligned(16))) unsigned long long key[TR];
-  __shared__ int wave_cnt[NWB];
+  __shared__ int wave_cnt[NWB], wave_cntm[NWB];
+  __shared__ unsigned int nbits[HS / 32];
+  __shared__ unsigned char nchunk[NWB];
   __shared__ int too_many;
   const int lane = threadIdx.x & 63, wave = threadIdx.x >> 6;
   const int tile = blockIdx.x;
   const int row = tile * TR + (int)threadIdx.x;
   for (int i = threadIdx.x; i < HS; i += TR) hk[i] = -1;
+  if (need && threadIdx.x < HS / 32) nbits[threadIdx.x] = 0u;
   if (threadIdx.x == 0) too_many = 0;
   __syncthreads();
   unsigned short slot[27];
@@ -107,7 +113,16 @@
     cb ^= cb >> 1; cb ^= cb >> 2; cb ^= cb >> 4;
     const unsigned long long coarse = cb;
     const unsigned long long pattern = ((unsigned long long)zp << 18) | ((unsigned long long)zm << 9) | z0;
-    key[threadIdx.x] = group ? (coarse << 35) | (pattern << 8) | threadIdx.x : (unsigned long long)threadIdx.x;
+    unsigned long long kk = group ? (coarse << 35) | (pattern << 8) | threadIdx.x : (unsigned long long)threadIdx.x;
+    if (need) {
+      bool nd = false;
+      if (row < n_out) {
+        const int cr = need_perm ? need_perm[row] : row;
+        nd = (need[cr >> 5] >> (cr & 31)) & 1u;
+      }
+      if (!nd) kk |= 1ull << 62;
+    }
+    key[threadIdx.x] = kk;
   }
   __syncthreads();
   if (too_many) {
@@ -117,57 +132,6 @@
     }
     return;
   }
-  constexpr int PER_WAVE = HS / NWB;
-  int cnt = 0;
-  for (int i0 = 0; i0 < PER_WAVE; i0 += 64) cnt += __popcll(__ballot(hk[wave * PER_WAVE + i0 + lane] >= 0));
-  if (lane == 0) wave_cnt[wave] = cnt;
-  __syncthreads();
-  int base = 0, total = 0;
-  for (int w = 0; w < NWB; ++w) { if (w < wave) base += wave_cnt[w]; total += wave_cnt[w]; }
-  unsigned char* lr = out + (size_t)tile * LR_BYTES;
-  int* U = reinterpret_cast<int*>(lr + 16);
-  if (total <= UMAX) {
-    for (int i0 = 0; i0 < PER_WAVE; i0 += 64) {
-      const int s = wave * PER_WAVE + i0 + lane;
-      const int key = hk[s];
-      const unsigned long long m = __ballot(key >= 0);
-      const int id = base + __popcll(m & ((1ull << lane) - 1ull));
-      if (key >= 0) {
-        hid[s] = (unsigned short)id;
-        U[id] = key;
-      }
-      base += __popcll(m);
-    }
-  } else {
-    for (int i0 = 0; i0 < PER_WAVE; i0 += 64) {
-      const int s = wave * PER_WAVE + i0 + lane;
-      const unsigned long long m = __ballot(hk[s] >= 0);
-      if (hk[s] >= 0) hid[s] = (unsigned short)(base + __popcll(m & ((1ull << lane) - 1ull)));
-      base += __popcll(m);
-    }
-    __syncthreads();
-    unsigned short ids[PER_WAVE / 64];
-#pragma unroll
-    for (int q = 0; q < PER_WAVE / 64; ++q) {
-      const int s = wave * PER_WAVE + q * 64 + lane;
-      ids[q] = hk[s] >= 0 ? (unsigned short)canonical_slot_id<HS>(hk, hid, s) : (unsigned short)0;
-    }
-    __syncthreads();
-#pragma unroll
-    for (int q = 0; q < PER_WAVE / 64; ++q) {
-      const int s = wave * PER_WAVE + q * 64 + lane;
-      const int key = hk[s];
-      if (key >= 0) {
-        hid[s] = ids[q];
-        if (ids[q] < NPASS * UMAX) U[ids[q]] = key;
-      }
-    }
-  }
-  if (threadIdx.x == 0) {
-    reinterpret_cast<int*>(lr)[0] = total <= NPASS * UMAX ? total : -1;
-    if (total > NPASS * UMAX) atomicAdd(overflow, 1);
-  }
-  __syncthreads();
   if (group) {
     const unsigned long long mine = key[threadIdx.x];
     int rank = 0;
@@ -181,11 +145,96 @@
     key[rank] = mine;
     __syncthreads();
   }
+  const int r = (int)threadIdx.x, w = r >> 6, c = (r >> 4) & 3, j = r & 15;
+  const unsigned long long skey = key[group ? (c * NWB + ((c & 1) ? NWB - 1 - w : w)) * 16 + j : r];
+  const int src = (int)(skey & 255u);
+  if (need) {
+    const unsigned long long nb = __ballot(((skey >> 62) & 1ull) == 0ull);
+    const unsigned int chunks = ((nb & 0xFFFFull) != 0) | ((((nb >> 16) & 0xFFFFull) != 0) << 1) | ((((nb >> 32) & 0xFFFFull) != 0) << 2) |
+                                ((((nb >> 48) & 0xFFFFull) != 0) << 3);
+    if (lane == 0) nchunk[wave] = (unsigned char)chunks;
+    if ((chunks >> c) & 1u) {
+#pragma unroll
+      for (int k = 0; k < 27; ++k) {
+        const unsigned int hs = srow[k][src];
+        if (hs != 0xFFFFu) atomicOr(&nbits[hs >> 5], 1u << (hs & 31u));
+      }
+    }
+    __syncthreads();
+  }
+  constexpr int PER_WAVE = HS / NWB;
+  int cnt = 0, cntm = 0;
+  for (int i0 = 0; i0 < PER_WAVE; i0 += 64) {
+    const int s = wave * PER_WAVE + i0 + lane;
+    cnt += __popcll(__ballot(hk[s] >= 0));
+    if (need) cntm += __popcll(__ballot((nbits[s >> 5] >> (s & 31)) & 1u));
+  }
+  if (lane == 0) { wave_cnt[wave] = cnt; wave_cntm[wave] = cntm; }
+  __syncthreads();
+  int base = 0, total = 0, basem = 0, totalm = 0;
+  for (int w_ = 0; w_ < NWB; ++w_) {
+    if (w_ < wave) { base += wave_cnt[w_] - wave_cntm[w_]; basem += wave_cntm[w_]; }
+    total += wave_cnt[w_]; totalm += wave_cntm[w_];
+  }
+  base += totalm;
+  unsigned char* lr = out + (size_t)tile * LR_BYTES;
+  int* U = reinterpret_cast<int*>(lr + 16);
+  if (total <= UMAX) {
+    for (int i0 = 0; i0 < PER_WAVE; i0 += 64) {
+      const int s = wave * PER_WAVE + i0 + lane;
+      const int key = hk[s];
+      const bool mk = need && ((nbits[s >> 5] >> (s & 31)) & 1u);
+      const unsigned long long m = __ballot(key >= 0 && !mk), mm = __ballot(mk);
+      const unsigned long long below = (1ull << lane) - 1ull;
+      const int id = mk ? basem + __popcll(mm & below) : base + __popcll(m & below);
+      if (key >= 0) {
+        hid[s] = (unsigned short)id;
+        U[id] = key;
+      }
+      base += __popcll(m);
+      basem += __popcll(mm);
+    }
+  } else {
+    base = 0;
+    for (int w_ = 0; w_ < wave; ++w_) base += wave_cnt[w_];
+    for (int i0 = 0; i0 < PER_WAVE; i0 += 64) {
+      const int s = wave * PER_WAVE + i0 + lane;
+      const unsigned long long m = __ballot(hk[s] >= 0);
+      if (hk[s] >= 0) hid[s] = (unsigned short)(base + __popcll(m & ((1ull << lane) - 1ull)));
+      base += __popcll(m);
+    }
+    __syncthreads();
+    unsigned short ids[PER_WAVE / 64];
+#pragma unroll
+    for (int q = 0; q < PER_WAVE / 64; ++q) {
+      const int s = wave * PER_WAVE + q * 64 + lane;
+      ids[q] = hk[s] >= 0 ? (unsigned short)canonical_slot_id<HS>(hk, hid, s) : (unsigned short)0;
+    }
+    __syncthreads();
+#pragma unroll
+    for (int q = 0; q < PER_WAVE / 64; ++q) {
+      const int s = wave * PER_WAVE + q * 64 + lane;
+      const int key = hk[s];
+      if (key >= 0) {
+        hid[s] = ids[q];
+        if (ids[q] < NPASS * UMAX) U[ids[q]] = key;
+      }
+    }
+  }
+  if (threadIdx.x == 0) {
+    reinterpret_cast<int*>(lr)[0] = total <= NPASS * UMAX ? total : -1;
+    if (total > NPASS * UMAX) atomicAdd(overflow, 1);
+    if (need) {
+      unsigned int nm = 0;
+      for (int w_ = 0; w_ < NWB; ++w_) nm |= (unsigned int)nchunk[w_] << (4 * w_);
+      reinterpret_cast<int*>(lr)[HDR_NEED_MASK] = (int)nm;
+      reinterpret_cast<int*>(lr)[HDR_NEED_UNIQUE] = total <= UMAX ? totalm : total;
+    }
+  }
+  __syncthreads();
   unsigned short* loc = reinterpret_cast<unsigned short*>(lr + 16 + UCAP * 4);
   unsigned char* msk = lr + MASK_OFF;
   __shared__ unsigned char nib[NPASS][27][4];
-  const int r = (int)threadIdx.x, w = r >> 6, c = (r >> 4) & 3, j = r & 15;
-  const int src = (int)(key[group ? (c * NWB + ((c & 1) ? NWB - 1 - w : w)) * 16 + j : r] & 255u);
   lr[RM_OFF + (w * 16 + j) * 4 + c] = (unsigned char)src;
   lr[INV_OFF + src] = (unsigned char)r;
 #pragma unroll
@@ -445,6 +494,17 @@
   ST_STAMP(0);
   const unsigned char* lr = local + (size_t)tile * LR_BYTES;
   const int* __restrict__ U = reinterpret_cast<const int*>(lr + 16);
+  unsigned int nm8 = 0xFFu;
+  int n_un = NPASS * UMAX;
+  if constexpr (TAILF != 0) {
+    if (a.needed_only) {
+      const unsigned int nmask = (unsigned)__builtin_amdgcn_readfirstlane(reinterpret_cast<const int*>(lr)[HDR_NEED_MASK]) & 0xFFFFu;
+      if (nmask == 0u) return;
+      n_un = __builtin_amdgcn_readfirstlane(reinterpret_cast<const int*>(lr)[HDR_NEED_UNIQUE]);
+      nm8 = (nmask >> ((2 * (wave >> 1)) * 4)) & 0xFFu;
+    }
+  }
+  auto chunk_on = [&](int hc) { return TAILF == 0 || ((nm8 >> hc) & 1u) != 0u; };
   if (threadIdx.x < 8)
     *reinterpret_cast<float4*>(xs + (threadIdx.x >> 2) * LO_REGION + UMAX * 64 + (threadIdx.x & 3) * 16) = make_float4(0.f, 0.f, 0.f, 0.f);
 
@@ -496,7 +556,7 @@
   for (int pass = 0; pass < n_pass; ++pass) {
     const int q_lo = max(i0 - pass * nqb, 0), q_hi = min(i1 - pass * nqb, nqb);
     if (q_lo >= q_hi) continue;
-    n_up = min(n_u - pass * UMAX, UMAX);
+    n_up = min(min(n_u, n_un) - pass * UMAX, UMAX);
     if (pass > 0) load_rows(pass);
     const unsigned int* mp = reinterpret_cast<const unsigned int*>(lr + MASK_OFF + pass * MASK_PASS_BYTES);
     u32x8 M0, M1;
@@ -504,6 +564,7 @@
     for (int i = 0; i < 8; ++i) {
       M0[i] = (unsigned)__builtin_amdgcn_readfirstlane((int)mp[i]) >> (w0 * 4);
       M1[i] = i < 6 ? (unsigned)__builtin_amdgcn_readfirstlane((int)mp[8 + i]) >> (w0 * 4) : 0u;
+      if constexpr (TAILF != 0) { M0[i] &= nm8 * 0x10001u; M1[i] &= nm8 * 0x10001u; }
     }
     const unsigned char* lb = lr + 16 + UCAP * 4 + ((size_t)pass * 27 * 64 + w0 * 16) * 8;
 #ifdef EYOC_ST_QBREV
@@ -644,7 +705,7 @@
 #pragma unroll
     for (int hc = 0; hc < NG; ++hc) {
       const int o = orow[hc];
-      if (o < a.n_out) {
+      if (o < a.n_out && chunk_on(hc)) {
         const char* rp = reinterpret_cast<const char*>(a.res + (size_t)o * a.ld_res) + split16_off4(ch);
         rh[hc] = *reinterpret_cast<const uint4*>(rp);
         rl[hc] = *reinterpret_cast<const uint4*>(rp + SPLIT16_LO);
@@ -662,7 +723,7 @@
       v[hc][t] = make_float4(A[ai % 16 + 0] * os + b4[t].x, A[ai % 16 + 1] * os + b4[t].y, A[ai % 16 + 2] * os + b4[t].z,
                              A[ai % 16 + 3] * os + b4[t].w);
     }
-    if (a.res && o < a.n_out) {
+    if (a.res && o < a.n_out && chunk_on(hc)) {
       const float4 q0 = split16_decode4(make_uint2(rh[hc].x, rh[hc].y), make_uint2(rl[hc].x, rl[hc].y));
       const float4 q1 = split16_decode4(make_uint2(rh[hc].z, rh[hc].w), make_uint2(rl[hc].z, rl[hc].w));
       v[hc][0].x += q0.x; v[hc][0].y += q0.y; v[hc][0].z += q0.z; v[hc][0].w += q0.w;
@@ -671,7 +732,7 @@
 #pragma unroll
     for (int t = 0; t < NTW; ++t) {
       if (a.relu) { v[hc][t].x = fmaxf(v[hc][t].x, 0.f); v[hc][t].y = fmaxf(v[hc][t].y, 0.f); v[hc][t].z = fmaxf(v[hc][t].z, 0.f); v[hc][t].w = fmaxf(v[hc][t].w, 0.f); }
-      if (o < a.n_out) split16_track(mx, v[hc][t]);
+      if (o < a.n_out && chunk_on(hc)) split16_track(mx, v[hc][t]);
     }
   }
   if constexpr (TAILF != 0) {
@@ -690,11 +751,14 @@
     constexpr int NK = NG / 2;
     int myrow[NK];
     uint4 Oh[NK], Ol[NK], Sh[NK], Sl[NK];
+    auto my_on = [&](int k) { return ((nm8 >> ((odd ? NK : 0) + k)) & 1u) != 0u; };
+    auto partner_on = [&](int k) { return ((nm8 >> ((odd ? 0 : NK) + k)) & 1u) != 0u; };
 #pragma unroll
     for (int k = 0; k < NK; ++k) {
       myrow[k] = odd ? orow[NK + k] : orow[k];
       Oh[k] = sel4(odd, Xh[NK + k], Xh[k]);
       Ol[k] = sel4(odd, Xl[NK + k], Xl[k]);
+      if (!my_on(k)) continue;
       const int o = myrow[k] < a.n_out ? myrow[k] : a.n_out - 1;
       const char* sp = reinterpret_cast<const char*>(tf.skip + (size_t)o * tf.ld_skip) + g * 16;
       Sh[k] = *reinterpret_cast<const uint4*>(sp);
@@ -732,6 +796,7 @@
     unsigned char* xw = xs + (size_t)(wave * NK) * 2048 + lane * 16;
 #pragma unroll
     for (int k = 0; k < NK; ++k) {
+      if (!partner_on(k)) continue;
       *reinterpret_cast<uint4*>(xw + k * 2048) = sel4(odd, Xh[k], Xh[NK + k]);
       *reinterpret_cast<uint4*>(xw + k * 2048 + 1024) = sel4(odd, Xl[k], Xl[NK + k]);
     }
@@ -740,6 +805,7 @@
     uint4 Ph[NK], Pl[NK];
 #pragma unroll
     for (int k = 0; k < NK; ++k) {
+      if (!my_on(k)) continue;
       Ph[k] = *reinterpret_cast<const uint4*>(xr + k * 2048);
       Pl[k] = *reinterpret_cast<const uint4*>(xr + k * 2048 + 1024);
     }
@@ -769,6 +835,7 @@
     float mx2 = 0.f;
 #pragma unroll
     for (int k = 0; k < NK; ++k) {
+      if (!my_on(k)) continue;
       half8_t Y[2][2];
       float cmx = 0.f;
 #pragma unroll
@@ -873,17 +940,21 @@
 
 size_t local_rulebook_bytes(int n_out) { return (size_t)cdiv(n_out, TILE) * LR_BYTES; }
 
-int build_local_rulebook(const int32_t* nbr_dev, int K, int n_out, unsigned char* out_dev, int* overflow_dev, hipStream_t st, int group) {
+int build_local_rulebook(const int32_t* nbr_dev, int K, int n_out, unsigned char* out_dev, int* overflow_dev, hipStream_t st, int group,
+                         const unsigned int* need, const int32_t* need_perm) {
   if (n_out <= 0) return EYOC_OK;
-  hipLaunchKernelGGL((k_local_rulebook<false, 4>), dim3(cdiv(n_out, TILE)), dim3(256), 0, st, nbr_dev, K, n_out, out_dev, overflow_dev, group, DeriveSrc());
+  hipLaunchKernelGGL((k_local_rulebook<false, 4>), dim3(cdiv(n_out, TILE)), dim3(256), 0, st, nbr_dev, K, n_out, out_dev, overflow_dev, group, DeriveSrc(),
+                     need, need_perm);
   EYOC_CHECK_HIP(hipGetLastError());
   return EYOC_OK;
 }
 
-int build_local_rulebook_derived(const DeriveSrc& src, int n_out, unsigned char* out_dev, int* overflow_dev, hipStream_t st, int group) {
+int build_local_rulebook_derived(const DeriveSrc& src, int n_out, unsigned char* out_dev, int* overflow_dev, hipStream_t st, int group,
+                                 const unsigned int* need, const int32_t* need_perm) {
   if (n_out <= 0) return EYOC_OK;
   EYOC_REQUIRE(src.coords && src.parent && src.children && src.s1c && src.nc > 0, EYOC_ERR_INVALID, "build_local_rulebook_derived: incomplete octree");
-  hipLaunchKernelGGL((k_local_rulebook<true, 4>), dim3(cdiv(n_out, TILE)), dim3(256), 0, st, (const int32_t*)nullptr, 27, n_out, out_dev, overflow_dev, group, src);
+  hipLaunchKernelGGL((k_local_rulebook<true, 4>), dim3(cdiv(n_out, TILE)), dim3(256), 0, st, (const int32_t*)nullptr, 27, n_out, out_dev, overflow_dev, group, src,
+                     need, need_perm);
   EYOC_CHECK_HIP(hipGetLastError());
   return EYOC_OK;
 }
@@ -1053,7 +1124,8 @@
 
 int build_local_rulebook128(const int32_t* nbr_dev, int K, int n_out, unsigned char* out_dev, int* overflow_dev, hipStream_t st, int group) {
   if (n_out <= 0) return EYOC_OK;
-  hipLaunchKernelGGL((k_local_rulebook<false, 2>), dim3(cdiv(n_out, 128)), dim3(128), 0, st, nbr_dev, K, n_out, out_dev, overflow_dev, group, DeriveSrc());
+  hipLaunchKernelGGL((k_local_rulebook<false, 2>), dim3(cdiv(n_out, 128)), dim3(128), 0, st, nbr_dev, K, n_out, out_dev, overflow_dev, group, DeriveSrc(),
+                     (const unsigned int*)nullptr, (const int32_t*)nullptr);
   EYOC_CHECK_HIP(hipGetLastError());
   return EYOC_OK;
 }
diff --git a/eyoc_amd/harness.py b/eyoc_amd/harness.py
--- a/eyoc_amd/harness.py
+++ b/eyoc_amd/harness.py
@@ -38,6 +38,7 @@
         nms_radius=0.6, max_points=8000, k1=30, k2=20))
     fp32_retry_per_step: bool = False
     isolate_failures: bool = False
+    features_at_samples_only: bool = False
     icp_refine: bool = False
     icp_max_correspondence_distance: float | None = None
     icp_max_iteration: int = 30
@@ -330,10 +331,13 @@
     def features(self, batch: DeviceBatch, maps=None) -> SparseTensor:
         return self._features(batch, maps)[0]
 
-    def _features(self, batch, maps):
+    def _features(self, batch, maps, rows_only=False):
         check, self.model.range_check = self.model.range_check, False
+
+        def forward(x):
+            return self.model.forward_rows(x) if rows_only and x.coordinate_manager.has_needed_rows() else self.model(x)
         try:
-            if maps is None and not self.cfg.isolate_failures:
+            if maps is None and not self.cfg.isolate_failures and not (rows_only and self.cfg.features_at_samples_only):
                 return self.model(SparseTensor(batch.feats, coordinates=batch.coords)), batch
             if maps is None:
                 cm, batch = self._build_maps(batch)
@@ -343,13 +347,13 @@
                 if self.cfg.isolate_failures and reduced is not batch:
                     batch = reduced
                     batch.record_stream(torch.cuda.current_stream())
-            return self.model(SparseTensor(batch.feats, coordinate_manager=cm)), batch
+            return forward(SparseTensor(batch.feats, coordinate_manager=cm)), batch
         finally:
             self.model.range_check = check
 
     def _build_maps(self, batch):
         def build(b):
-            cm = CoordinateManager(b.coords)
+            cm = CoordinateManager(b.coords, needed_rows=torch.cat((b.sel0, b.sel1)) if self.cfg.features_at_samples_only else None)
             cm.maps(-1)
             return cm
         if not self.cfg.isolate_failures:
@@ -373,7 +377,7 @@
         step = _Step(slot, self._ev[slot] if timed else None)
         main = torch.cuda.current_stream()
         self._mark(step, 0)
-        F, step.batch = self._features(batch, maps)
+        F, step.batch = self._features(batch, maps, rows_only=self.model.spconv_math != "fp32")
         step.F = F.F
         self._mark(step, 1)
         if read_back:
diff --git a/eyoc_amd/model.py b/eyoc_amd/model.py
--- a/eyoc_amd/model.py
+++ b/eyoc_amd/model.py
@@ -216,6 +216,17 @@
         return self._blob
 
     def forward(self, x: SparseTensor) -> SparseTensor:
+        return self._forward(x, False)
+
+    def forward_rows(self, x: SparseTensor, out: torch.Tensor | None = None) -> SparseTensor:
+        if self.training:
+            raise _lib.EyocError("forward_rows: inference only")
+        if out is not None and (out.shape != (len(x), self.out_channels) or out.dtype != torch.float32 or not out.is_contiguous()
+                                or out.device != x.device):
+            raise ValueError("forward_rows: out must be a contiguous f32 [N, out_channels] tensor on the input's device")
+        return self._forward(x, True, out)
+
+    def _forward(self, x: SparseTensor, rows_only: bool, out=None) -> SparseTensor:
         if not isinstance(x, SparseTensor):
             raise TypeError("expected an eyoc_amd.SparseTensor")
         if x.F.shape[1] != self.in_channels:
@@ -232,14 +243,16 @@
         cm = x.coordinate_manager
         maps = cm.maps(-1)
         cm._reading()
-        out = torch.empty((len(x), self.out_channels), dtype=torch.float32, device=dev)
+        if out is None:
+            out = torch.empty((len(x), self.out_channels), dtype=torch.float32, device=dev)
         with torch.cuda.device(dev):
             ws = _lib.workspace(lib.eyoc_model_workspace_bytes(self._handle, maps), dev)
 
-            def run():
-                _lib.check(lib.eyoc_model_forward(_lib.ctx(dev.index), self._handle, maps, _lib.ptr(x.F), _lib.ptr(out),
-                                                  _lib.ptr(ws), ws.numel(), _lib.stream_ptr()), "eyoc_model_forward")
-            run()
+            def run(rows_only=False):
+                fn, name = (lib.eyoc_model_forward_rows, "eyoc_model_forward_rows") if rows_only else (lib.eyoc_model_forward, "eyoc_model_forward")
+                _lib.check(fn(_lib.ctx(dev.index), self._handle, maps, _lib.ptr(x.F), _lib.ptr(out),
+                              _lib.ptr(ws), ws.numel(), _lib.stream_ptr()), name)
+            run(rows_only)
             if self.range_check and lib.eyoc_model_last_math(self._handle) == 1:
                 try:
                     self.check_range()
diff --git a/eyoc_amd/sparse_tensor.py b/eyoc_amd/sparse_tensor.py
--- a/eyoc_amd/sparse_tensor.py
+++ b/eyoc_amd/sparse_tensor.py
@@ -16,12 +16,17 @@
 
 class CoordinateManager:
 
-    def __init__(self, coordinates: torch.Tensor):
+    def __init__(self, coordinates: torch.Tensor, needed_rows: torch.Tensor | None = None):
         if coordinates.dim() != 2 or coordinates.shape[1] != 4:
             raise ValueError(f"coordinates must be [N,4] (batch,x,y,z), got {tuple(coordinates.shape)}")
         if not coordinates.is_cuda:
             raise _lib.EyocError("SparseTensor coordinates must live on the GPU (no CPU path)")
         self.coordinates = coordinates.to(torch.int32).contiguous()
+        if needed_rows is not None:
+            if not needed_rows.is_cuda or needed_rows.device != coordinates.device or needed_rows.dtype != torch.int64 or needed_rows.dim() != 1:
+                raise ValueError("needed_rows must be a 1-d int64 tensor on the device of the coordinates")
+            needed_rows = needed_rows.contiguous()
+        self.needed_rows = needed_rows
         self._maps = None
         self._ws = None
         self._maps_caller = None
@@ -32,16 +37,26 @@
     def device(self):
         return self.coordinates.device
 
-    def _build(self, order: int):
+    def _build(self, order: int, needed: bool = False):
         lib = _lib.load()
         n = self.coordinates.shape[0]
         with torch.cuda.device(self.device):
             ws = _lib.workspace(lib.eyoc_maps_workspace_bytes(n), self.device)
             h = C.c_void_p()
-            _lib.check(lib.eyoc_maps_build_ordered(_lib.ctx(self.device.index), _lib.ptr(self.coordinates), n,
-                                                   _lib.ptr(ws), ws.numel(), _lib.stream_ptr(), int(order),
-                                                   C.byref(h)), "eyoc_maps_build")
+            if needed and self.needed_rows is not None:
+                rows = self.needed_rows
+                _lib.check(lib.eyoc_maps_build_needed(_lib.ctx(self.device.index), _lib.ptr(self.coordinates), n,
+                                                      _lib.ptr(ws), ws.numel(), _lib.stream_ptr(), int(order),
+                                                      _lib.ptr(rows) if rows.numel() else None, rows.numel(),
+                                                      C.byref(h)), "eyoc_maps_build_needed")
+            else:
+                _lib.check(lib.eyoc_maps_build_ordered(_lib.ctx(self.device.index), _lib.ptr(self.coordinates), n,
+                                                       _lib.ptr(ws), ws.numel(), _lib.stream_ptr(), int(order),
+                                                       C.byref(h)), "eyoc_maps_build")
         return h, ws
+
+    def has_needed_rows(self) -> bool:
+        return bool(_lib.load().eyoc_maps_has_needed_rows(self.maps()))
 
     def _reading(self):
         try:
@@ -58,7 +73,7 @@
 
     def maps(self, order: int = 0):
         if self._maps is None:
-            self._maps, self._ws = self._build(order)
+            self._maps, self._ws = self._build(order, needed=True)
         return self._maps
 
     def _caller_maps(self):
@@ -108,6 +123,16 @@
         with torch.cuda.device(self.device):
             _lib.check(lib.eyoc_maps_copy_row_order(self.maps(), _lib.ptr(out), _lib.stream_ptr()), "eyoc_maps_copy_row_order")
         return out
+
+    def tile_records(self, level: int) -> torch.Tensor:
+        lib = _lib.load()
+        m = self.maps()
+        nbytes = int(lib.eyoc_spconv_local_rulebook_bytes(self.rows(level)))
+        out = torch.empty((nbytes,), dtype=torch.uint8, device=self.device)
+        self._reading()
+        with torch.cuda.device(self.device):
+            _lib.check(lib.eyoc_maps_copy_tile_records(m, level, _lib.ptr(out), nbytes, _lib.stream_ptr()), "eyoc_maps_copy_tile_records")
+        return out.view(-1, 33408)
 
     def up_order(self, level: int, internal: bool = False) -> torch.Tensor:
         m = self.maps() if internal else self._caller_maps()
diff --git a/include/eyoc_hip.h b/include/eyoc_hip.h
--- a/include/eyoc_hip.h
+++ b/include/eyoc_hip.h
@@ -45,6 +45,10 @@
                     size_t workspace_bytes, void* stream, eyoc_maps** out);
 int eyoc_maps_build_ordered(eyoc_ctx* ctx, const int32_t* coords_dev, int n_rows, void* workspace_dev,
                             size_t workspace_bytes, void* stream, int order, eyoc_maps** out);
+int eyoc_maps_build_needed(eyoc_ctx* ctx, const int32_t* coords_dev, int n_rows, void* workspace_dev, size_t workspace_bytes,
+                           void* stream, int order, const int64_t* needed_rows_dev, int64_t n_needed, eyoc_maps** out);
+int eyoc_maps_has_needed_rows(const eyoc_maps* maps);
+int eyoc_maps_copy_tile_records(const eyoc_maps* maps, int level, void* out_dev, size_t out_bytes, void* stream);
 int eyoc_maps_last_fault_batches(const eyoc_ctx* ctx, uint32_t* dup, uint32_t* range);
 int eyoc_maps_free(eyoc_maps* maps);
 int eyoc_maps_copy_up_order(const eyoc_maps* maps, int level, int32_t* out_dev, void* stream);
@@ -161,6 +165,9 @@
 int eyoc_model_forward(eyoc_ctx* ctx, const eyoc_model* model, const eyoc_maps* maps,
                        const float* feats_dev, float* out_dev, void* workspace_dev,
                        size_t workspace_bytes, void* stream);
+int eyoc_model_forward_rows(eyoc_ctx* ctx, const eyoc_model* model, const eyoc_maps* maps,
+                            const float* feats_dev, float* out_dev, void* workspace_dev,
+                            size_t workspace_bytes, void* stream);
 int eyoc_model_num_layers(const eyoc_model* model);
 int eyoc_model_layer_work(eyoc_ctx* ctx, const eyoc_model* model, const eyoc_maps* maps, void* stream,
                           const char** names, int64_t* pairs, double* flops, double* gather_bytes,
```

Result: slower. 3298 pairs/s (-1.2%).
